# SabaPivot/ProjectionTrainer

Measured on AMD Instinct MI355X. Metric: Stage-1 images/sec/node (SigLIP-L-384 + Gemma3-1B, 576+128 tok), higher is better.
Workload: dtype bf16; 1 GPU; cfg2: SigLIP-ViT-L/16-384 frozen fwd + MLP projector fwd/bwd + Gemma3-1B frozen fwd/bwd, 575 vis + 128 text tokens; global_batch=32, per_gpu_batch=32, seq_len=703, parallelism=dp1

## Files before the change

### include/ptk.h

```cpp
#ifndef PTK_H
#define PTK_H

#include <stddef.h>
#include <stdint.h>

#ifdef __cplusplus
extern "C" {
#endif

#define PTK_ABI_VERSION 8

int ptk_abi_version(void);
const char* ptk_last_error(void);


typedef struct {
  int g;
  int skip;
  int64_t gs;
  int64_t off;
} ptk_rowmap;

enum { PTK_ACT_NONE = 0, PTK_ACT_GELU_TANH = 1, PTK_ACT_GELU_ERF = 2, PTK_ACT_GEGLU = 3,
       PTK_ACT_GELU_ERF_BWD = 4, PTK_ACT_GEGLU_BWD = 5 };
enum { PTK_OUT_BF16 = 0, PTK_OUT_F32 = 1, PTK_OUT_F32_BF16ROUND = 2 };

typedef struct {
  const void* A;
  const void* B;
  void* C;
  int M, N, K;
  int64_t lda, ldb, ldc;
  int batch;
  int batch_inner;
  int64_t sA0, sA1, sB0, sB1, sC0, sC1;
  float alpha;
  int act;
  int out;
  const float* bias;
  const float* rowadd;
  int rowadd_period;
  int64_t ld_rowadd;
  const float* resid;
  int64_t ld_resid;
  void* aux;
  void* aux2;
  int64_t ld_aux;
  const void* aux_in;
  const void* aux_in2;
  int64_t ld_aux_in;
  ptk_rowmap amap;
  ptk_rowmap cmap;
  const void* resid16;
  int64_t ld_resid16;
  int bf16_linear;
  void* tail_ws;
} ptk_gemm_desc;
int ptk_gemm(const ptk_gemm_desc* d, void* stream);
#define PTK_GEMM_TAIL_COUNTER_BYTES 16384
size_t ptk_gemm_tail_scratch_bytes(void);
int ptk_gemm_tail_split(const ptk_gemm_desc* d);
int ptk_gemm_plan(const ptk_gemm_desc* d, int ncu, int* path, int* tile_rows, int* tail_split);
int ptk_gemm_split_plan(const ptk_gemm_desc* d, int ncu, int64_t part_floats, int* slices, int* kc, int* rem,
                        int* tail_ws);

int ptk_layernorm(const float* x, const float* w, const float* b, void* y, int rows, int cols, float eps,
                  void* stream);
int ptk_rmsnorm(const float* x, const float* w, void* y, float* rstd, int rows, int cols, float eps,
                void* stream);
int ptk_rmsnorm_bwd(const float* x, const float* w, const float* rstd, const float* dn, const float* dacc,
                    float* dx, int rows, int cols, void* stream);
int ptk_qknorm_rope_fwd(const void* qkv, const float* q_norm_w, const float* k_norm_w, const float* cos_t,
                        const float* sin_t, int batch, int seq, int heads, int kv_heads, int head_dim, float eps,
                        void* Q, void* K, void* V, float* rstd_q, float* rstd_k, void* stream);
int ptk_qknorm_rope_bwd(const void* qkv, const float* q_norm_w, const float* k_norm_w, const float* cos_t,
                        const float* sin_t, int batch, int seq, int heads, int kv_heads, int head_dim,
                        const float* rstd_q, const float* rstd_k, const void* dQ, const void* dK, const void* dV,
                        void* dqkv, void* stream);
int ptk_softmax(const float* S, void* P, int nz, int rows, int cols, int64_t ld, int rows_per_batch, int qdiv,
                int zdiv, int causal, int window, const int32_t* key_valid, int key_len, void* stream);
int ptk_cross_entropy(void* logits, int64_t ld, int rows, int vocab, const int64_t* targets, float* row_loss,
                      const float* gscale, void* stream);
int ptk_transpose_bf16(const void* in, int64_t ld_in, void* out, int64_t ld_out, int nz, int64_t s_in,
                       int64_t s_out, int rows, int cols, int rows_pad, void* stream);
int ptk_transpose_rows_bf16(const void* in, int64_t ld_in, int map_g, int64_t map_gs, int64_t map_off, int rows,
                            int cols, void* out, int64_t ld_out, int rows_pad, void* stream);
int ptk_weight_grad_bf16(const void* dy, int64_t lddy, int y_map_g, int64_t y_map_gs, int64_t y_map_off, int Ny,
                         const void* x, int64_t ldx, int x_map_g, int64_t x_map_gs, int64_t x_map_off, int Nx, int rows,
                         void* grad, void* ta, void* tb, float* part, int64_t part_floats, int mode, void* stream);
int ptk_cast_f32_bf16(const float* in, void* out, int64_t n, void* stream);
int ptk_fill_normal_bf16(void* out, int64_t n, uint64_t seed, float std, float mean, void* stream);
// ... 20 lines not shown
  float scale;
} ptk_flash_desc;
int ptk_flash_attn_fwd(const ptk_flash_desc* d, void* stream);

typedef struct {
  const void* Q; const void* K; const void* V; const void* O; const void* dO;
  const float* lse; float* delta;
  void* dQ; void* dK; void* dV;
  int rows, nkeys, head_dim;
  int batch, batch_inner, zdiv;
  int64_t ldo, sO0, sO1;
  ptk_rowmap omap;
  int qdiv, causal, window;
  const int32_t* key_valid;
  float scale;
  void* workspace;
  int64_t workspace_bytes;
} ptk_flash_bwd_desc;
size_t ptk_flash_bwd_workspace_bytes(const ptk_flash_bwd_desc* d);
int ptk_flash_attn_bwd(const ptk_flash_bwd_desc* d, void* stream);

typedef struct {
  int image_size, patch_size, channels, hidden, heads, intermediate, layers;
  float eps;
} ptk_siglip_config;

typedef struct {
  const void* wqkv;  const float* bqkv;
  const void* wo;    const float* bo;
  const void* w1;    const float* b1;
  const void* w2;    const float* b2;
  const float* ln1_w; const float* ln1_b;
  const float* ln2_w; const float* ln2_b;
} ptk_siglip_layer;

typedef struct {
  const void* patch_w;
  const float* patch_b;
  const float* pos;
  const float* post_w; const float* post_b;
  const ptk_siglip_layer* layers;
} ptk_siglip_weights;

size_t ptk_siglip_workspace_bytes(const ptk_siglip_config* c, int batch);
int ptk_siglip_fwd(const ptk_siglip_config* c, const ptk_siglip_weights* w, int batch, const void* pixels,
                   void* out, void* ws, size_t ws_bytes, void* stream);

typedef struct {
  int vision_dim, inter_dim, llm_dim;
  const void* w1;   const float* b1;
  const void* w2;   const float* b2;
  const void* w2t;
  void* tail_ws;
} ptk_projector;

int ptk_projector_fwd(const ptk_projector* p, int rows, const void* x, void* a, void* h, float* out,
                      ptk_rowmap out_map, int64_t ld_out, int round_bf16, void* stream);
size_t ptk_projector_workspace_bytes(const ptk_projector* p, int rows);
int ptk_projector_bwd(const ptk_projector* p, int rows, const void* x, const void* a, const void* h,
                      const void* dy, float* dw1, float* db1, float* dw2, float* db2, void* ws, size_t ws_bytes,
                      void* stream);
int ptk_gather_vision_grad(const float* dx_llm, int batch, int num_patches, int seq_pad, int llm_dim, void* dy,
                           void* stream);

typedef struct {
  int vocab, hidden, inter, layers, heads, kv_heads, head_dim;
  int sliding_window, sliding_pattern;
  int pad_token_id;
  float query_pre_attn_scalar, eps;
} ptk_gemma3_config;

typedef struct {
  const void* wqkv;  const void* wqkv_t;
  const void* wo;    const void* wo_t;
  const void* wgu;   const void* wgu_t;
  const void* wd;    const void* wd_t;
  const float* ln_in; const float* ln_post_attn; const float* ln_pre_ff; const float* ln_post_ff;
  const float* q_norm; const float* k_norm;
} ptk_gemma3_layer;

typedef struct {
  const void* embed;
  const void* embed_t;
  const float* final_norm;
  const float* rope_cos_local; const float* rope_sin_local;
  const float* rope_cos_global; const float* rope_sin_global;
  int rope_max_pos;
  const ptk_gemma3_layer* layers;
} ptk_gemma3_weights;

typedef struct {
  int batch, text_len, num_vision, seq_pad;
  const int64_t* token_ids;
  const int64_t* labels;
  float* x;
  float* dx;
  float loss_scale;
  float* loss;
  int label_offset;
} ptk_gemma3_batch;

size_t ptk_gemma3_workspace_bytes(const ptk_gemma3_config* c, int batch, int text_len, int seq_pad);
int ptk_gemma3_loss_fwd_bwd(const ptk_gemma3_config* c, const ptk_gemma3_weights* w, const ptk_gemma3_batch* b,
                            void* ws, size_t ws_bytes, void* stream);
int ptk_gemma3_loss_fwd(const ptk_gemma3_config* c, const ptk_gemma3_weights* w, const ptk_gemma3_batch* b,
                        void* ws, size_t ws_bytes, void* stream);

typedef struct {
  void* wqkv; void* wo; void* wgu; void* wd;
  void* ln_in; void* ln_post_attn; void* ln_pre_ff; void* ln_post_ff;
  void* q_norm; void* k_norm;
// ... 96 lines not shown
```

### projectiontrainer_amd/_lib.py

```python
from __future__ import annotations

import ctypes as C
import os

_HERE = os.path.dirname(os.path.abspath(__file__))
LIB_PATH = os.path.join(_HERE, "libptk.so")
if os.environ.get("PTK_LIB"):
    LIB_PATH = os.path.join(os.path.dirname(_HERE), os.environ["PTK_LIB"])

c_void_p, c_int, c_int64, c_float, c_size_t, c_uint64 = C.c_void_p, C.c_int, C.c_int64, C.c_float, C.c_size_t, C.c_uint64
c_float_p = C.POINTER(C.c_float)

ACT_NONE, ACT_GELU_TANH, ACT_GELU_ERF, ACT_GEGLU, ACT_GELU_ERF_BWD, ACT_GEGLU_BWD = range(6)
OUT_BF16, OUT_F32, OUT_F32_BF16ROUND = range(3)


class RowMap(C.Structure):
    _fields_ = [("g", c_int), ("skip", c_int), ("gs", c_int64), ("off", c_int64)]


class GemmDesc(C.Structure):
    _fields_ = [("A", c_void_p), ("B", c_void_p), ("C", c_void_p),
                ("M", c_int), ("N", c_int), ("K", c_int),
                ("lda", c_int64), ("ldb", c_int64), ("ldc", c_int64),
                ("batch", c_int), ("batch_inner", c_int),
                ("sA0", c_int64), ("sA1", c_int64), ("sB0", c_int64), ("sB1", c_int64),
                ("sC0", c_int64), ("sC1", c_int64),
                ("alpha", c_float), ("act", c_int), ("out", c_int),
                ("bias", c_void_p), ("rowadd", c_void_p), ("rowadd_period", c_int),
                ("ld_rowadd", c_int64), ("resid", c_void_p), ("ld_resid", c_int64),
                ("aux", c_void_p), ("aux2", c_void_p), ("ld_aux", c_int64),
                ("aux_in", c_void_p), ("aux_in2", c_void_p), ("ld_aux_in", c_int64),
                ("amap", RowMap), ("cmap", RowMap), ("resid16", c_void_p), ("ld_resid16", c_int64),
                ("bf16_linear", c_int), ("tail_ws", c_void_p)]


class FlashDesc(C.Structure):
    _fields_ = [("Q", c_void_p), ("K", c_void_p), ("V", c_void_p), ("O", c_void_p), ("lse", c_void_p),
                ("rows", c_int), ("nkeys", c_int), ("head_dim", c_int),
                ("ldq", c_int64), ("ldk", c_int64), ("ldo", c_int64),
                ("batch", c_int), ("batch_inner", c_int), ("zdiv", c_int),
                ("sQ0", c_int64), ("sQ1", c_int64), ("sK0", c_int64), ("sK1", c_int64),
                ("sO0", c_int64), ("sO1", c_int64), ("qmap", RowMap), ("omap", RowMap),
                ("qdiv", c_int), ("causal", c_int), ("window", c_int), ("key_valid", c_void_p),
                ("scale", c_float)]


class FlashBwdDesc(C.Structure):
    _fields_ = [("Q", c_void_p), ("K", c_void_p), ("V", c_void_p), ("O", c_void_p), ("dO", c_void_p),
                ("lse", c_void_p), ("delta", c_void_p), ("dQ", c_void_p), ("dK", c_void_p), ("dV", c_void_p),
                ("rows", c_int), ("nkeys", c_int), ("head_dim", c_int),
                ("batch", c_int), ("batch_inner", c_int), ("zdiv", c_int),
                ("ldo", c_int64), ("sO0", c_int64), ("sO1", c_int64), ("omap", RowMap),
                ("qdiv", c_int), ("causal", c_int), ("window", c_int), ("key_valid", c_void_p),
                ("scale", c_float), ("workspace", c_void_p), ("workspace_bytes", c_int64)]


class SiglipConfigC(C.Structure):
    _fields_ = [("image_size", c_int), ("patch_size", c_int), ("channels", c_int), ("hidden", c_int),
                ("heads", c_int), ("intermediate", c_int), ("layers", c_int), ("eps", c_float)]


class SiglipLayerC(C.Structure):
    _fields_ = [("wqkv", c_void_p), ("bqkv", c_void_p), ("wo", c_void_p), ("bo", c_void_p),
                ("w1", c_void_p), ("b1", c_void_p), ("w2", c_void_p), ("b2", c_void_p),
                ("ln1_w", c_void_p), ("ln1_b", c_void_p), ("ln2_w", c_void_p), ("ln2_b", c_void_p)]


class SiglipWeightsC(C.Structure):
    _fields_ = [("patch_w", c_void_p), ("patch_b", c_void_p), ("pos", c_void_p),
                ("post_w", c_void_p), ("post_b", c_void_p), ("layers", C.POINTER(SiglipLayerC))]


class ProjectorC(C.Structure):
    _fields_ = [("vision_dim", c_int), ("inter_dim", c_int), ("llm_dim", c_int),
                ("w1", c_void_p), ("b1", c_void_p), ("w2", c_void_p), ("b2", c_void_p), ("w2t", c_void_p),
                ("tail_ws", c_void_p)]


class Gemma3ConfigC(C.Structure):
    _fields_ = [("vocab", c_int), ("hidden", c_int), ("inter", c_int), ("layers", c_int), ("heads", c_int),
                ("kv_heads", c_int), ("head_dim", c_int), ("sliding_window", c_int),
                ("sliding_pattern", c_int), ("pad_token_id", c_int),
                ("query_pre_attn_scalar", c_float), ("eps", c_float)]


class Gemma3LayerC(C.Structure):
    _fields_ = [("wqkv", c_void_p), ("wqkv_t", c_void_p), ("wo", c_void_p), ("wo_t", c_void_p),
                ("wgu", c_void_p), ("wgu_t", c_void_p), ("wd", c_void_p), ("wd_t", c_void_p),
                ("ln_in", c_void_p), ("ln_post_attn", c_void_p), ("ln_pre_ff", c_void_p),
                ("ln_post_ff", c_void_p), ("q_norm", c_void_p), ("k_norm", c_void_p)]


class Gemma3WeightsC(C.Structure):
    _fields_ = [("embed", c_void_p), ("embed_t", c_void_p), ("final_norm", c_void_p),
                ("rope_cos_local", c_void_p), ("rope_sin_local", c_void_p),
                ("rope_cos_global", c_void_p), ("rope_sin_global", c_void_p),
                ("rope_max_pos", c_int), ("layers", C.POINTER(Gemma3LayerC))]


class Gemma3BatchC(C.Structure):
    _fields_ = [("batch", c_int), ("text_len", c_int), ("num_vision", c_int), ("seq_pad", c_int),
                ("token_ids", c_void_p), ("labels", c_void_p), ("x", c_void_p), ("dx", c_void_p),
                ("loss_scale", c_float), ("loss", c_void_p), ("label_offset", c_int)]


class Gemma3GenerateC(C.Structure):
    _fields_ = [("batch", c_int), ("prompt_len", c_int), ("max_new_tokens", c_int), ("do_sample", c_int),
                ("top_k", c_int), ("temperature", c_float), ("seed", C.c_uint64), ("eos_token_id", c_int64),
                ("pad_token_id", c_int64), ("prompt_batch_stride", c_int64), ("top_p", c_float)]


class Gemma3DecodeC(C.Structure):
    _fields_ = [("rows", c_int), ("prompt_len", c_int), ("max_new_tokens", c_int), ("prompt_repeat", c_int),
                ("prompt_batch_stride", c_int64)]


class Gemma3LayerGradsC(C.Structure):
    _fields_ = [(n, c_void_p) for n in ("wqkv", "wo", "wgu", "wd", "ln_in", "ln_post_attn", "ln_pre_ff",
                                        "ln_post_ff", "q_norm", "k_norm")]


class Gemma3GradsC(C.Structure):
    _fields_ = [("embed", c_void_p), ("final_norm", c_void_p), ("layers", C.POINTER(Gemma3LayerGradsC))]
# ... 1 lines not shown

class ImageDesc(C.Structure):
    _fields_ = [("src_off", c_int64), ("h", C.c_int32), ("w", C.c_int32), ("c", C.c_int32),
                ("kh", C.c_int32), ("kv", C.c_int32), ("pad_", C.c_int32),
                ("coef_off", c_int64), ("tmp_off", c_int64)]


ABI_VERSION = 8

SIGNATURES = {
    "ptk_abi_version": (c_int, []),
    "ptk_last_error": (C.c_char_p, []),
    "ptk_gemm": (c_int, [C.POINTER(GemmDesc), c_void_p]),
    "ptk_gemm_tail_scratch_bytes": (c_size_t, []),
    "ptk_gemm_tail_split": (c_int, [C.POINTER(GemmDesc)]),
    "ptk_gemm_plan": (c_int, [C.POINTER(GemmDesc), c_int] + [C.POINTER(c_int)] * 3),
    "ptk_gemm_split_plan": (c_int, [C.POINTER(GemmDesc), c_int, c_int64] + [C.POINTER(c_int)] * 4),
    "ptk_layernorm": (c_int, [c_void_p, c_void_p, c_void_p, c_void_p, c_int, c_int, c_float, c_void_p]),
    "ptk_rmsnorm": (c_int, [c_void_p, c_void_p, c_void_p, c_void_p, c_int, c_int, c_float, c_void_p]),
    "ptk_rmsnorm_bwd": (c_int, [c_void_p] * 6 + [c_int, c_int, c_void_p]),
    "ptk_qknorm_rope_fwd": (c_int, [c_void_p] * 5 + [c_int] * 5 + [c_float] + [c_void_p] * 6),
    "ptk_qknorm_rope_bwd": (c_int, [c_void_p] * 5 + [c_int] * 5 + [c_void_p] * 7),
    "ptk_softmax": (c_int, [c_void_p, c_void_p, c_int, c_int, c_int, c_int64, c_int, c_int, c_int, c_int,
                            c_int, c_void_p, c_int, c_void_p]),
    "ptk_cross_entropy": (c_int, [c_void_p, c_int64, c_int, c_int, c_void_p, c_void_p, c_void_p, c_void_p]),
    "ptk_transpose_bf16": (c_int, [c_void_p, c_int64, c_void_p, c_int64, c_int, c_int64, c_int64, c_int,
                                   c_int, c_int, c_void_p]),
    "ptk_transpose_rows_bf16": (c_int, [c_void_p, c_int64, c_int, c_int64, c_int64, c_int, c_int, c_void_p, c_int64,
                                        c_int, c_void_p]),
    "ptk_weight_grad_bf16": (c_int, [c_void_p, c_int64, c_int, c_int64, c_int64, c_int,
                                     c_void_p, c_int64, c_int, c_int64, c_int64, c_int, c_int,
                                     c_void_p, c_void_p, c_void_p, c_void_p, c_int64, c_int, c_void_p]),
    "ptk_cast_f32_bf16": (c_int, [c_void_p, c_void_p, c_int64, c_void_p]),
    "ptk_fill_normal_bf16": (c_int, [c_void_p, c_int64, c_uint64, c_float, c_float, c_void_p]),
    "ptk_gemm_timer_enable": (c_int, [c_int]),
    "ptk_gemm_force_small_tiles": (c_int, [c_int]),
    "ptk_gemm_timer_read": (c_int, [c_int, C.POINTER(C.c_double), C.POINTER(c_int)]),
    "ptk_gemm_path_counts": (c_int, [c_void_p, c_int]),
    "ptk_stage_timers_enable": (c_int, [c_int]),
    "ptk_stage_begin": (c_int, [C.c_char_p, c_void_p]),
    "ptk_stage_end": (c_int, [c_void_p]),
    "ptk_stage_timers_read": (c_int64, [C.c_char_p, c_size_t, c_int]),
    "ptk_flash_attn_fwd": (c_int, [C.POINTER(FlashDesc), c_void_p]),
    "ptk_flash_attn_bwd": (c_int, [C.POINTER(FlashBwdDesc), c_void_p]),
    "ptk_flash_bwd_workspace_bytes": (c_size_t, [C.POINTER(FlashBwdDesc)]),
    "ptk_siglip_workspace_bytes": (c_size_t, [C.POINTER(SiglipConfigC), c_int]),
    "ptk_siglip_fwd": (c_int, [C.POINTER(SiglipConfigC), C.POINTER(SiglipWeightsC), c_int, c_void_p, c_void_p,
                               c_void_p, c_size_t, c_void_p]),
    "ptk_projector_fwd": (c_int, [C.POINTER(ProjectorC), c_int, c_void_p, c_void_p, c_void_p, c_void_p, RowMap,
                                  c_int64, c_int, c_void_p]),
    "ptk_projector_workspace_bytes": (c_size_t, [C.POINTER(ProjectorC), c_int]),
    "ptk_projector_bwd": (c_int, [C.POINTER(ProjectorC), c_int] + [c_void_p] * 8 + [c_void_p, c_size_t, c_void_p]),
    "ptk_gather_vision_grad": (c_int, [c_void_p, c_int, c_int, c_int, c_int, c_void_p, c_void_p]),
    "ptk_gemma3_workspace_bytes": (c_size_t, [C.POINTER(Gemma3ConfigC), c_int, c_int, c_int]),
    "ptk_gemma3_loss_fwd_bwd": (c_int, [C.POINTER(Gemma3ConfigC), C.POINTER(Gemma3WeightsC),
                                        C.POINTER(Gemma3BatchC), c_void_p, c_size_t, c_void_p]),
    "ptk_gemma3_loss_fwd": (c_int, [C.POINTER(Gemma3ConfigC), C.POINTER(Gemma3WeightsC),
                                    C.POINTER(Gemma3BatchC), c_void_p, c_size_t, c_void_p]),
    "ptk_gemma3_train_workspace_bytes": (c_size_t, [C.POINTER(Gemma3ConfigC), c_int, c_int, c_int]),
    "ptk_gemma3_train_fwd_bwd": (c_int, [C.POINTER(Gemma3ConfigC), C.POINTER(Gemma3WeightsC),
                                         C.POINTER(Gemma3BatchC), C.POINTER(Gemma3GradsC), c_void_p, c_size_t,
                                         c_void_p]),
    "ptk_gemma3_generate_workspace_bytes": (c_size_t, [C.POINTER(Gemma3ConfigC), c_int, c_int, c_int]),
    "ptk_gemma3_generate": (c_int, [C.POINTER(Gemma3ConfigC), C.POINTER(Gemma3WeightsC), C.POINTER(Gemma3GenerateC),
                                    c_void_p, c_void_p, c_void_p, c_void_p, c_void_p, c_size_t, c_void_p]),
    "ptk_gemma3_decode_workspace_bytes": (c_size_t, [C.POINTER(Gemma3ConfigC), C.POINTER(Gemma3DecodeC)]),
# ... 121 lines not shown
```

### projectiontrainer_amd/csrc/capi.cpp

```cpp
#include <stdarg.h>
#include <stdio.h>

#include "../../include/ptk.h"
#include "ptk_internal.h"

namespace ptk {

static thread_local char g_err[512] = "";

int set_error(const char* fmt, ...) {
  va_list ap;
  va_start(ap, fmt);
  vsnprintf(g_err, sizeof(g_err), fmt, ap);
  va_end(ap);
  return -1;
}

RowMap to_map(ptk_rowmap m) { return RowMap{m.g, m.skip, (long)m.gs, (long)m.off}; }

GemmArgs to_args(const ptk_gemm_desc* d) {
  GemmArgs a;
  a.A = (const bf16_t*)d->A; a.B = (const bf16_t*)d->B; a.C = d->C;
  a.M = d->M; a.N = d->N; a.K = d->K;
  a.lda = d->lda; a.ldb = d->ldb; a.ldc = d->ldc;
  a.zin = d->batch_inner > 0 ? d->batch_inner : 1;
  a.sA0 = d->sA0; a.sA1 = d->sA1; a.sB0 = d->sB0; a.sB1 = d->sB1; a.sC0 = d->sC0; a.sC1 = d->sC1;
  a.alpha = d->alpha;
  a.bias = d->bias; a.rowadd = d->rowadd; a.rowadd_period = d->rowadd_period > 0 ? d->rowadd_period : 1;
  a.ld_rowadd = d->ld_rowadd; a.resid = d->resid; a.ld_resid = d->ld_resid;
  a.aux = (bf16_t*)d->aux; a.aux2 = (bf16_t*)d->aux2; a.ld_aux = d->ld_aux;
  a.aux_in = (const bf16_t*)d->aux_in; a.aux_in2 = (const bf16_t*)d->aux_in2; a.ld_aux_in = d->ld_aux_in;
  a.amap = to_map(d->amap); a.cmap = to_map(d->cmap);
  a.resid16 = (const bf16_t*)d->resid16; a.ld_resid16 = d->ld_resid16; a.bf16_linear = d->bf16_linear;
  a.tail_ws = d->tail_ws;
  return a;
}

int device_cus() {
  static int n = 0;
  if (n == 0) {
    int dev = 0, v = 0;
    if (hipGetDevice(&dev) == hipSuccess &&
        hipDeviceGetAttribute(&v, hipDeviceAttributeMultiprocessorCount, dev) == hipSuccess && v > 0)
      n = v;
    else
      n = 256;
  }
  return n;
}

}

using namespace ptk;
#define ST ((hipStream_t)stream)

extern "C" {

int ptk_abi_version(void) { return PTK_ABI_VERSION; }
const char* ptk_last_error(void) { return g_err; }

int ptk_gemm(const ptk_gemm_desc* d, void* stream) {
  if (!d) return set_error("ptk_gemm: null desc");
  if (d->act == PTK_ACT_GEGLU && (d->N % 32)) return set_error("ptk_gemm: GEGLU needs N %% 32 == 0");
  return launch_gemm(to_args(d), d->act, d->out, d->batch > 0 ? d->batch : 1, ST);
}

size_t ptk_gemm_tail_scratch_bytes(void) { return p8_tail_scratch_bytes(); }
// ... 57 lines not shown
}
int ptk_qknorm_rope_bwd(const void* qkv, const float* q_norm_w, const float* k_norm_w, const float* cos_t,
                        const float* sin_t, int batch, int seq, int heads, int kv_heads, int head_dim,
                        const float* rstd_q, const float* rstd_k, const void* dQ, const void* dK, const void* dV,
                        void* dqkv, void* stream) {
  const AttnShape sh{batch, seq, heads, kv_heads, head_dim};
  return launch_qknorm_rope_bwd((const bf16_t*)qkv, q_norm_w, k_norm_w, cos_t, sin_t, sh, rstd_q, rstd_k,
                                (const bf16_t*)dQ, (const bf16_t*)dK, (const bf16_t*)dV, (bf16_t*)dqkv, ST);
}
int ptk_softmax(const float* S, void* P, int nz, int rows, int cols, int64_t ld, int rows_per_batch, int qdiv,
                int zdiv, int causal, int window, const int32_t* key_valid, int key_len, void* stream) {
  MaskSpec m{rows_per_batch > 0 ? rows_per_batch : rows, qdiv > 0 ? qdiv : 1, zdiv > 0 ? zdiv : 1, causal, window,
             key_valid, key_len};
  return launch_softmax_fwd(S, (bf16_t*)P, nz, rows, cols, ld, m, ST);
}

int ptk_cross_entropy(void* logits, int64_t ld, int rows, int vocab, const int64_t* targets, float* row_loss,
                      const float* gscale, void* stream) {
  return launch_ce_fwd_bwd((bf16_t*)logits, ld, rows, vocab, targets, row_loss, gscale, ST);
}

int ptk_transpose_bf16(const void* in, int64_t ld_in, void* out, int64_t ld_out, int nz, int64_t s_in, int64_t s_out,
                       int rows, int cols, int rows_pad, void* stream) {
  return launch_transpose((const bf16_t*)in, ld_in, s_in, 0, 1, (bf16_t*)out, ld_out, s_out, 0, nz, rows, cols,
                          rows_pad, ST);
}

int ptk_transpose_rows_bf16(const void* in, int64_t ld_in, int map_g, int64_t map_gs, int64_t map_off, int rows,
                            int cols, void* out, int64_t ld_out, int rows_pad, void* stream) {
  const RowMap m{map_g, 0, map_gs, map_off};
  return launch_transpose_rows((const bf16_t*)in, ld_in, m, rows, cols, (bf16_t*)out, ld_out, rows_pad, ST);
}

int ptk_cast_f32_bf16(const float* in, void* out, int64_t n, void* stream) {
  return launch_cast_f32_bf16(in, (bf16_t*)out, n, ST);
}

int ptk_gemm_force_small_tiles(int mode) {
  if (mode != 0 && mode != 1 && mode != 2 && mode != 4 && mode != 8 && mode != 32 && mode != 512 && mode != 1024 &&
      mode != 4096)
    return set_error("gemm tile mode %d not in {0, 1, 2, 4, 8, 32, 512, 1024, 4096}", mode);
  force_small_tiles(mode);
  return 0;
}
int ptk_gemm_timer_enable(int on) {
  timer_enable(on);
  return 0;
}
int ptk_gemm_timer_read(int act_class, double* total_ms, int* count) { return timer_read(act_class, total_ms, count); }
int ptk_gemm_path_counts(int64_t* counts, int reset) { return path_counts(counts, reset); }

int ptk_fill_normal_bf16(void* out, int64_t n, uint64_t seed, float std, float mean, void* stream) {
  return launch_fill_normal_bf16((bf16_t*)out, n, seed, std, mean, ST);
}

int ptk_flash_attn_fwd(const ptk_flash_desc* d, void* stream) {
  if (!d) return set_error("flash: null desc");
  FlashArgs a;
  a.Q = (const bf16_t*)d->Q; a.K = (const bf16_t*)d->K; a.V = (const bf16_t*)d->V; a.O = (bf16_t*)d->O;
  a.lse = d->lse; a.rows = d->rows; a.nkeys = d->nkeys; a.D = d->head_dim;
  a.ldq = d->ldq; a.ldk = d->ldk; a.ldo = d->ldo;
  a.zin = d->batch_inner > 0 ? d->batch_inner : 1; a.zdiv = d->zdiv > 0 ? d->zdiv : 1;
  a.sQ0 = d->sQ0; a.sQ1 = d->sQ1; a.sK0 = d->sK0; a.sK1 = d->sK1; a.sO0 = d->sO0; a.sO1 = d->sO1;
  a.qmap = to_map(d->qmap); a.omap = to_map(d->omap);
  a.qdiv = d->qdiv > 0 ? d->qdiv : 1; a.causal = d->causal; a.window = d->window;
  a.key_valid = d->key_valid; a.scale = d->scale;
// ... 137 lines not shown
```

### projectiontrainer_amd/csrc/gemm.hip

```cpp
#include <stdlib.h>

#include "common.h"
#include "ptk_internal.h"
#include "gemm_epi.h"

#include <algorithm>
#include <vector>

namespace ptk {

constexpr int BM = 128, BN = 128, BK = 64, GROUP_M = 8;
constexpr int STAGE_BYTES = (BM + BN) * BK * 2;
static_assert(4 * 64 * 68 * 4 >= 2 * STAGE_BYTES, "epilogue staging must cover the pipeline buffers");

typedef const __attribute__((address_space(1))) void* gptr_t;
typedef __attribute__((address_space(3))) void* lptr_t;

#ifdef PTK_NO_SRC_SWZ
#define PTK_SRC_SWZ(c, r) (c)
#else
#define PTK_SRC_SWZ(c, r) ((c) ^ (((r) >> 1) & 7))
#endif

#ifndef PTK_GLDS_AUX
// ... 651 lines not shown
    ++g_path_count[path][act & 7];
    if (g_timing && ((g_timing_mask >> act) & 1)) { e0 = next_event(act); e1 = next_event(act); }
    if (e0) (void)hipEventRecord(e0, st);
  }
  ~GemmLaunchScope() { if (e1) (void)hipEventRecord(e1, st); }
};

GemmPlanEnv gemm_plan_env() {
  GemmPlanEnv e;
  e.ncu = device_cus();
  e.force_tiles = g_force_tiles;
  e.p8_all = PTK_AB("PTK_P8", 0) == 1;
  e.tm_short = PTK_AB("PTK_TM224", 1) != 0;
  e.lean_epi = lean_epilogue_enabled();
  e.streamk = streamk_enabled();
  e.tail_scope = tail_scope();
  return e;
}

int launch_gemm(const GemmArgs& a, int act, int out, int batch, hipStream_t st, const GemmPlan* planned) {
  if (a.M <= 0 || a.N <= 0 || batch <= 0) return 0;
  if (a.K <= 0 || a.K % BK) return set_error("gemm: K=%d must be a positive multiple of 64", a.K);
  if ((a.lda % 8) || (a.ldb % 8)) return set_error("gemm: lda/ldb must be multiples of 8 (16-B rows)");
  if (((uintptr_t)a.A | (uintptr_t)a.B) & 15) return set_error("gemm: A/B must be 16-B aligned");
  if (a.zin <= 0) return set_error("gemm: zin must be >= 1");
  const long ntile = (long)((a.M + BM - 1) / BM) * ((a.N + BN - 1) / BN);
  if (ntile > 0x7fffffffL) return set_error("gemm: too many tiles");
  if (!gemm_act_out(act, out, [](auto, auto) {})) return set_error("gemm: unsupported (act=%d, out=%d)", act, out);
  const GemmPlan plan = planned ? *planned : gemm_plan(a, act, out, batch, gemm_plan_env());
  GemmLaunchScope scope(plan.path, act, st);
  const dim3 grid_big((unsigned)((long)((a.M + BIG - 1) / BIG) * ((a.N + BIG - 1) / BIG)), 1, 1);
  switch (plan.path) {
    case GEMM_PATH_P8:
    case GEMM_PATH_P8SK: return launch_gemm_p8(a, act, out, st, plan.tail, plan.tm);
    case GEMM_PATH_W4: return launch_gemm_w4(a, act, out, st, 0);
    case GEMM_PATH_BIG2:
      gemm_act_out(act, out, [&](auto A, auto O) {
        hipLaunchKernelGGL((gemm_big2_kernel<A(), O()>), grid_big, dim3(512), 0, st, a);
      });
      break;
    case GEMM_PATH_BIG:
      gemm_act_out(act, out, [&](auto A, auto O) {
        hipLaunchKernelGGL((gemm_big_kernel<A(), O()>), grid_big, dim3(512), 0, st, a);
      });
      break;
    default:
      gemm_act_out(act, out, [&](auto A, auto O) {
        hipLaunchKernelGGL((gemm_nt_kernel<A(), O()>), dim3((unsigned)ntile, 1, (unsigned)batch), dim3(256), 0, st, a);
      });
      break;
  }
  return hipGetLastError() == hipSuccess ? 0 : set_error("gemm launch failed");
}

int gemm_p8_kslices(const GemmArgs& a, int slices, hipStream_t st) {
  if (a.M <= 0 || a.N <= 0) return 0;
  GemmLaunchScope scope(GEMM_PATH_P8, ACT_NONE, st);
  return launch_gemm_p8_kslices(a, slices, st);
}

int gemm_tn(const GemmArgs& a, int out, int slices, void* slab, hipStream_t st, long k_rows) {
  if (a.M <= 0 || a.N <= 0) return 0;
  GemmLaunchScope scope(GEMM_PATH_TN, ACT_NONE, st);
  return launch_gemm_tn(a, out, slices, slab, st, k_rows);
}

}

// ... 9 lines not shown
```

### projectiontrainer_amd/csrc/gemm_plan.cpp

```cpp
#include <algorithm>

#include "ptk_internal.h"

namespace ptk {

bool w4_supported(const GemmArgs& a, int act, int out) {
  if (a.N % 8 || a.K % W4_KT) return false;
  if (a.alpha != 1.f) return false;
  if (a.row_stats) return false;
  if (a.resid16 && (out != OUT_BF16 || a.ld_resid16 % 8)) return false;
  if ((a.ldc % 8) || (a.resid && a.ld_resid % 4) || (a.rowadd && a.ld_rowadd % 4)) return false;
  if ((a.aux || a.aux2) && a.ld_aux % 8) return false;
  if ((a.aux_in || a.aux_in2) && a.ld_aux_in % 8) return false;
  if (((uintptr_t)a.C | (uintptr_t)a.bias | (uintptr_t)a.resid | (uintptr_t)a.resid16 | (uintptr_t)a.rowadd | (uintptr_t)a.aux |
       (uintptr_t)a.aux2 | (uintptr_t)a.aux_in | (uintptr_t)a.aux_in2) & 15)
    return false;
  if (act == ACT_GEGLU && (a.N % 32)) return false;
  if (act == ACT_GEGLU_BWD && (!a.aux_in || !a.aux_in2 || (a.N % 16) || (a.ldc % 8))) return false;
  if (act == ACT_GELU_ERF_BWD && !a.aux_in) return false;
  if (out != OUT_BF16 && (act != ACT_NONE)) return false;
  if (a.amap.g != 0) return false;
  const double abytes = (double)(a.M + a.amap.off) * a.lda * 2, bbytes = (double)a.N * a.ldb * 2;
  return abytes < 2147483000.0 && bbytes < 2147483000.0;
}
// ... 137 lines not shown
  return a.M >= 1024 && a.N >= 512 && (a.K >= 6144 || (a.N >= 6144 && a.K >= 1152));
}
bool staggered_big(const GemmArgs& a, const GemmPlanEnv& e) {
  return e.force_tiles == 4 || (e.force_tiles == 0 && big_shape(a) && a.K >= 4096);
}
bool big(const GemmArgs& a, const GemmPlanEnv& e) {
  return e.force_tiles != 1 && (e.force_tiles == 2 || big_shape(a));
}

}

GemmPlan gemm_plan(const GemmArgs& a, int act, int out, int batch, const GemmPlanEnv& e) {
  GemmPlan p;
  if (batch != 1) {
    p.path = GEMM_PATH_NTB;
    return p;
  }
  if (p8_supported(a, act, out)) {
    const P8Tail tl = tail(a, act, out, e);
    const int tm = tl.units ? 256 : short_tile(a, act, out, e);
    const bool single = single_round(a, act, out, e);
    if (e.force_tiles == 32 || single || tl.units || tm != 256 || p8_over_w4(a, act, out, e)) {
      p.path = tl.units ? GEMM_PATH_P8SK : GEMM_PATH_P8;
      p.tm = tm;
      p.tail = tl;
      p.single_round = single;
      return p;
    }
  }
  if ((e.force_tiles == 8 || w4_shape(a, act, out, e)) && w4_supported(a, act, out)) p.path = GEMM_PATH_W4;
  else if (staggered_big(a, e)) p.path = GEMM_PATH_BIG2;
  else if (big(a, e)) p.path = GEMM_PATH_BIG;
  return p;
}

GemmSplitPlan gemm_split_plan(const GemmArgs& a, int out, long part_floats, const GemmPlanEnv& env) {
  GemmSplitPlan sp;
  GemmPlanEnv e = env;
  e.force_tiles = 0;
  sp.direct = gemm_plan(a, ACT_NONE, out, 1, e);
  const GemmPlan& direct = sp.direct;
  if (direct.path == GEMM_PATH_P8SK) return sp;
  if (e.streamk && a.K >= 4096 && (size_t)part_floats * sizeof(float) >= P8_CNT_BYTES + p8_slab_bytes(e.ncu)) {
    GemmArgs b = a;
    b.tail_ws = reinterpret_cast<void*>((uintptr_t)256);
    const GemmPlan lent = gemm_plan(b, ACT_NONE, out, 1, e);
    if (lent.path == GEMM_PATH_P8SK) {
      sp.tail_ws = true;
      sp.direct = lent;
      return sp;
    }
  }
  if (direct.single_round) return sp;
  const long nbig = tiles256(a);
  int S = 1, kmin = 1024;
  if (a.K >= 4096 && nbig <= 64) S = 4;
  else if (a.K >= 4096 && nbig <= 300) S = 2;
  const long n128 = (long)((a.M + 127) / 128) * ((a.N + 127) / 128), cus = e.ncu;
  if (n128 * 2 <= cus) {
    kmin = 256;
    while (n128 * S * 2 <= 2 * cus && a.K / (S * 2) >= kmin) S *= 2;
  }
  while (S > 1 && ((long)S * a.M * a.N > part_floats || a.K / S < kmin || a.N % 4 || a.ldc % 4)) S /= 2;
  const bool plain = !a.rowadd && !a.resid && !a.aux && !a.aux_in && a.amap.g == 0 && a.amap.off == 0 &&
                     a.cmap.g == 0 && a.cmap.off == 0 && a.bias == nullptr && a.alpha == 1.f;
  if (S == 1 || !plain) return sp;
// ... 54 lines not shown
```

### projectiontrainer_amd/csrc/gemm_w4.hip

```cpp
#include "common.h"
#include "ptk_internal.h"
#include "gemm_epi.h"
#include "gemm_persist.h"

#include <algorithm>
#include <cstdlib>
#include <type_traits>

#ifndef PTK_W4_RDS
#define PTK_W4_RDS 0
#endif
#ifndef PTK_W4_DMS
#define PTK_W4_DMS 0
#endif
#ifndef PTK_P8_PRIO
#define PTK_P8_PRIO 1
#endif
#ifndef PTK_P8_MPRIO
#define PTK_P8_MPRIO 0
#endif

namespace ptk {

template <int ACT, int OUT, bool LEAN = false>
__global__ void __launch_bounds__(256, 1) gemm_w4_kernel(GemmArgs p, uint32_t a_bytes, uint32_t b_bytes,
                                                         uint32_t c_bytes) {
  __shared__ __attribute__((aligned(16))) char smem[W4_NSLOT * W4_SLOT];
  const int lane = threadIdx.x & 63;
  const int wave = __builtin_amdgcn_readfirstlane(threadIdx.x >> 6);
  const int wr = wave >> 1, wc = wave & 1;
  const int nbm = (p.M + W4 - 1) / W4, nbn = (p.N + W4 - 1) / W4;
  const int ntile = nbm * nbn;
  const int G = gridDim.x;
  int loc;
  {
    const int b = blockIdx.x, q = G >> 3, rr = G & 7, x = b & 7;
    loc = (x < rr ? x * (q + 1) : rr * (q + 1) + (x - rr) * q) + (b >> 3);
  }
  if (loc >= ntile) return;
  const int nt = p.K / W4_KT;
  const int nks = 2 * nt;
  const int total_ks = ((ntile - loc + G - 1) / G) * nks;

  const u32x4_t rsa = w4_rsrc(p.A, a_bytes), rsb = w4_rsrc(p.B, b_bytes);

  uint32_t offa[4], offb[4];
#pragma unroll
  for (int j = 0; j < 4; ++j) {
    const int lr = wave * 64 + 16 * j + (lane >> 2);
    const int lc = (lane & 3) ^ ((lane >> 3) & 2);
    offa[j] = (uint32_t)lr * (uint32_t)p.lda * 2u + lc * 16;
    offb[j] = (uint32_t)lr * (uint32_t)p.ldb * 2u + lc * 16;
  }
  const uint32_t lds_base = __builtin_amdgcn_readfirstlane(lds_addr(smem));
  const uint32_t lds_dma = lds_base + wave * 64 * 64;
  int dt = loc, dks = 0, dcount = 0;
  uint32_t dsa = 0, dsb = 0;
  auto dma_tile = [&](int t) {
    int bm, bn;
    w4_tile_coords(t, nbm, nbn, bm, bn);
    dsa = __builtin_amdgcn_readfirstlane((uint32_t)(bm * W4 + (int)p.amap.off) * (uint32_t)p.lda * 2u);
    dsb = __builtin_amdgcn_readfirstlane((uint32_t)(bn * W4) * (uint32_t)p.ldb * 2u);
  };
  auto dma_advance = [&]() {
    if (++dcount < total_ks) {
      if (++dks == nks) {
        dks = 0;
        dt += G;
        dma_tile(dt);
      }
    }
  };
  auto slot_next = [](uint32_t s) { s += W4_SLOT; return s == W4_NSLOT * W4_SLOT ? 0u : s; };

  const int frag_off = (lane & 15) * 64 + (((lane >> 4) ^ ((lane >> 1) & 2)) << 4);
  const uint32_t frag_a = lds_addr(smem) + wr * 128 * 64 + frag_off;
  const uint32_t frag_b = lds_addr(smem) + W4_SOPB + wc * 128 * 64 + frag_off;
  bf16x8_t fa0[8], fb0[8], fa1[8], fb1[8];
  f32x4_t acc[8][8];

#define W4_GROUP(FA, FB, Q, FIRST)                                                  \
  do {                                                                              \
    _Pragma("unroll") for (int jj = 0; jj < 4; ++jj) {                              \
      if (FIRST) W4_MFMA0(acc[(Q) >> 1][4 * ((Q) & 1) + jj], FB[4 * ((Q) & 1) + jj], FA[(Q) >> 1]); \
      else W4_MFMA(acc[(Q) >> 1][4 * ((Q) & 1) + jj], FB[4 * ((Q) & 1) + jj], FA[(Q) >> 1]);       \
    }                                                                               \
  } while (0)
#define W4_READ(FA, FB, BA, BB, Q)                                                  \
  do {                                                                              \
    if ((Q) < 8) W4_DSREAD(FA[(Q) & 7], BA, ((Q) & 7) * 1024);                      \
    else W4_DSREAD(FB[(Q) & 7], BB, ((Q) & 7) * 1024);                              \
  } while (0)
#define W4_PIN(FA, FB)                                                                              \
  do {                                                                                              \
    asm volatile("s_waitcnt lgkmcnt(0)" ::: "memory");                                              \
    asm volatile("" : "+v"(FA[0]), "+v"(FA[1]), "+v"(FA[2]), "+v"(FA[3]), "+v"(FA[4]), "+v"(FA[5]),  \
                 "+v"(FA[6]), "+v"(FA[7]));                                                         \
    asm volatile("" : "+v"(FB[0]), "+v"(FB[1]), "+v"(FB[2]), "+v"(FB[3]), "+v"(FB[4]), "+v"(FB[5]),  \
                 "+v"(FB[6]), "+v"(FB[7]));                                                         \
  } while (0)

  auto kstep = [&](auto first_c, const bf16x8_t (&FA)[8], const bf16x8_t (&FB)[8], bf16x8_t (&NA)[8],
                   bf16x8_t (&NB)[8], uint32_t rs, uint32_t ws) {
    constexpr bool first = decltype(first_c)::value;
    const uint32_t ba = frag_a + rs, bb = frag_b + rs;
    const uint32_t da = lds_dma + ws, db = da + W4_SOPB;
    const uint32_t sa = dsa + dks * (W4_KS * 2), sb = dsb + dks * (W4_KS * 2);
#pragma unroll
    for (int q = 0; q < 16; ++q) {
#if PTK_W4_RDS == 1
      if (q < 8) {
        W4_READ(NA, NB, ba, bb, 2 * q);
        W4_READ(NA, NB, ba, bb, 2 * q + 1);
      }
#else
      if (q < 8) {
        W4_READ(NA, NB, ba, bb, q);
      } else if (q < 12) {
        W4_READ(NA, NB, ba, bb, 8 + 2 * (q - 8));
        W4_READ(NA, NB, ba, bb, 9 + 2 * (q - 8));
      }
#endif
#if PTK_W4_DMS == 1
      if (q >= 8) {
        const int pc = q - 8;
#elif PTK_W4_DMS == 2
      if (q < 8) {
        const int pc = q;
#elif PTK_W4_DMS == 3
      if (q & 1) {
        const int pc = q >> 1;
#else
      if (!(q & 1)) {
        const int pc = q >> 1;
#endif
        if (pc & 1) W4_DMA(rsb, offb[pc >> 1], sb, db + (pc >> 1) * 1024);
        else W4_DMA(rsa, offa[pc >> 1], sa, da + (pc >> 1) * 1024);
      }
      W4_GROUP(FA, FB, q, first);
    }
  };

  dma_tile(dt);
#pragma unroll
  for (int b = 0; b < 4; ++b) {
    const uint32_t da = lds_dma + b * W4_SLOT, db = da + W4_SOPB;
    const uint32_t sa = dsa + dks * (W4_KS * 2), sb = dsb + dks * (W4_KS * 2);
#pragma unroll
    for (int j = 0; j < 4; ++j) {
      W4_DMA(rsa, offa[j], sa, da + j * 1024);
      W4_DMA(rsb, offb[j], sb, db + j * 1024);
    }
    dma_advance();
  }
  asm volatile("s_waitcnt vmcnt(8)" ::: "memory");
  __builtin_amdgcn_s_barrier();
#pragma unroll
  for (int q = 0; q < 16; ++q) W4_READ(fa0, fb0, frag_a, frag_b, q);
  W4_PIN(fa0, fb0);
  __builtin_amdgcn_s_barrier();

  uint32_t rs = W4_SLOT, ws = 4 * W4_SLOT;
  int t = loc, kt = 0;
#ifdef PTK_P8_STAMPS
  unsigned int stv_[4] = {0u, 0u, 0u, 0u};
  const int em_ = g_p8_epi_mode;
#endif
  for (int g = 0; g < total_ks; g += 2) {
    if (kt == 0) P8_STAMP(0, (t - loc) / G);
    if (kt == 0) kstep(std::true_type{}, fa0, fb0, fa1, fb1, rs, ws);
    else kstep(std::false_type{}, fa0, fb0, fa1, fb1, rs, ws);
    W4_PIN(fa1, fb1);
    dma_advance();
    rs = slot_next(rs);
    ws = slot_next(ws);
    kstep(std::false_type{}, fa1, fb1, fa0, fb0, rs, ws);
    W4_PIN(fa0, fb0);
    dma_advance();
    rs = slot_next(rs);
    ws = slot_next(ws);
// ... 5 lines not shown
      asm volatile("s_nop 7\n\ts_nop 7" ::: "memory");
      int bm, bn;
      w4_tile_coords(t, nbm, nbn, bm, bn);
#ifdef PTK_P8_STAMPS
      if (em_ != 1)
#endif
      {
        const long row0 = (long)bm * W4 + wr * 128, col0 = (long)bn * W4 + wc * 128;
        if constexpr (LEAN && ACT == ACT_GEGLU_BWD)
          w4_epilogue_lean_glu<ACT, 8>(kernarg_args(), acc, row0, col0, lane, c_bytes);
        else if constexpr (LEAN) w4_epilogue_lean<ACT, 8>(kernarg_args(), acc, row0, col0, lane, c_bytes);
        else w4_epilogue<ACT, OUT>(kernarg_args(), acc, row0, col0, lane);
      }
      P8_STAMP(3, (t - loc) / G);
      t += G;
      kt = 0;
    } else {
      ++kt;
    }
  }
  asm volatile("s_waitcnt vmcnt(0)" ::: "memory");
#ifdef PTK_P8_STAMPS
  if (wave == 0 && blockIdx.x < 1024)
#pragma unroll
    for (int k = 0; k < 4; ++k) g_p8_stamps[blockIdx.x][k][lane] = stv_[k];
#endif
#undef W4_GROUP
#undef W4_READ
#undef W4_PIN
}

bool lean_epilogue_enabled() { return PTK_AB("PTK_LEAN_EPI", 1) != 0; }

int launch_gemm_w4(const GemmArgs& a, int act, int out, hipStream_t st, int max_grid) {
  const long ntile = (long)((a.M + W4 - 1) / W4) * ((a.N + W4 - 1) / W4);
  long grid = std::min<long>(ntile, max_grid > 0 ? max_grid : device_cus());
#ifdef PTK_P8_STAMPS
  if (const char* e = getenv("PTK_GEMM_GRID")) grid = std::min<long>(grid, atol(e));
#endif
  const long arows = a.M + a.amap.off;
  const uint32_t ab = (uint32_t)std::min<double>((double)arows * a.lda * 2, 2147483000.0);
  const uint32_t bb = (uint32_t)std::min<double>((double)a.N * a.ldb * 2, 2147483000.0);
  uint32_t cb = 0;
  if (lean_epilogue_ok(a, act, out, cb, lean_epilogue_enabled())) {
#define PTK_W4L_CASE(ACT_)                                                                                   \
    if (act == ACT_)                                                                                         \
      hipLaunchKernelGGL((gemm_w4_kernel<ACT_, OUT_BF16, true>), dim3((unsigned)grid), dim3(256), 0, st, a, ab, bb, cb);
    PTK_W4L_CASE(ACT_NONE)
    PTK_W4L_CASE(ACT_GELU_TANH)
    PTK_W4L_CASE(ACT_GEGLU_BWD)
#undef PTK_W4L_CASE
    return hipGetLastError() == hipSuccess ? 0 : set_error("gemm_w4 launch failed");
  }
  if (!gemm_act_out(act, out, [&](auto A, auto O) {
        hipLaunchKernelGGL((gemm_w4_kernel<A(), O()>), dim3((unsigned)grid), dim3(256), 0, st, a, ab, bb, 0u);
      }))
    return set_error("gemm_w4: unsupported (act=%d, out=%d)", act, out);
  return hipGetLastError() == hipSuccess ? 0 : set_error("gemm_w4 launch failed");
}


namespace {
constexpr int P8_PIECES = 4;

}



#ifdef PTK_P8_CREAD
#define P8_DSREAD(DST, ADDR, OFF) \
  (DST) = *reinterpret_cast<const __attribute__((address_space(3))) bf16x8_t*>((uintptr_t)((ADDR) + (OFF)))
#define P8_LGKM(N) do { } while (0)
#define P8_BARRIER() do { __builtin_amdgcn_s_barrier(); asm volatile("" ::: "memory"); } while (0)
#else
#define P8_BARRIER() __builtin_amdgcn_s_barrier()
#define P8_DSREAD(DST, ADDR, OFF) W4_DSREAD(DST, ADDR, OFF)
#define P8_LGKM(N) asm volatile("s_waitcnt lgkmcnt(" #N ")" ::: "memory")
#endif
template <int ACT, int OUT, bool SK, bool LEAN = false, int TM = 256>
__global__ void __launch_bounds__(512, 1) gemm_p8_kernel(GemmArgs p, uint32_t a_bytes, uint32_t b_bytes, P8Tail tl,
                                                         uint32_t c_bytes) {
  static_assert(TM == 256 || ((TM == 224 || TM == 192 || TM == 160) && !SK), "shorter tiles: whole tiles only");
  constexpr int RB = TM / 32;
  __shared__ __attribute__((aligned(16))) char smem[W4_NSLOT * W4_SLOT];
  const int lane = threadIdx.x & 63;
  const int wave = __builtin_amdgcn_readfirstlane(threadIdx.x >> 6);
  const int hf = wave >> 2, wq = wave & 3, wr = wq >> 1, wc = wq & 1;
  const bool a_dma = TM == 256 || wave < RB;
  const int nbm = (p.M + TM - 1) / TM, nbn = (p.N + W4 - 1) / W4;
  const int ntile = nbm * nbn;
  const int G = gridDim.x;
  int loc;
  {
    const int b = blockIdx.x, q = G >> 3, rr = G & 7, x = b & 7;
    loc = (x < rr ? x * (q + 1) : rr * (q + 1) + (x - rr) * q) + (b >> 3);
  }
  const int nt = p.K / W4_KT;
  const int dp_tiles = SK ? tl.dp_tiles : ntile;
  const int n_dp = loc < dp_tiles ? (dp_tiles - loc + G - 1) / G : 0;
  const int U = SK ? tl.units : 0, Gs = SK ? tl.gsplit : 1, nu = nt >> 1;
  const int u0 = SK && loc < Gs ? p8_start(loc, Gs, U) : 0, u1 = SK && loc < Gs ? p8_start(loc + 1, Gs, U) : 0;
  const int n_tail = u1 > u0 ? (u1 - 1) / nu - u0 / nu + 1 : 0;
  const int nseg = n_dp + n_tail;
  if (nseg == 0) return;
  const int total_ks = 2 * n_dp * nt + 4 * (u1 - u0);
  uint32_t segA = 0, segB = 0, segC = 0;
  if constexpr (SK) {
    const int i = lane;
    int t, k0, k1, tt;
    if (i < n_dp) {
      t = loc + i * G; k0 = 0; k1 = nt; tt = -1;
    } else {
      tt = u0 / nu + (i - n_dp);
      k0 = 2 * (max(u0, tt * nu) - tt * nu);
      k1 = 2 * (min(u1, (tt + 1) * nu) - tt * nu);
      t = dp_tiles + tt;
    }
    int g0 = 0, np = 1, s0 = 0, myslot = 0;
    if (tt >= 0 && i < nseg) {
      g0 = p8_owner((long)tt * nu, Gs, U);
      np = p8_owner((long)(tt + 1) * nu - 1, Gs, U) - g0 + 1;
      s0 = p8_start(g0, Gs, U) < tt * nu ? 1 : 0;
      myslot = u0 < tt * nu ? 1 : 0;
      if (np == 1) tt = -1;
    }
    segA = (uint32_t)t | ((uint32_t)(tt + 1) << 16);
    segB = (uint32_t)k0 | ((uint32_t)k1 << 16);
    segC = (uint32_t)g0 | ((uint32_t)np << 10) | ((uint32_t)s0 << 20) | ((uint32_t)myslot << 21);
  }
  auto segment = [&](int s, int& t, int& k0, int& k1, int& tt) __attribute__((always_inline)) {
    if constexpr (!SK) {
      t = loc + s * G; k0 = 0; k1 = nt; tt = -1;
    } else {
      const uint32_t a = __builtin_amdgcn_readlane(segA, s), b = __builtin_amdgcn_readlane(segB, s);
      t = (int)(a & 0xffffu); tt = (int)(a >> 16) - 1;
      k0 = (int)(b & 0xffffu); k1 = (int)(b >> 16);
    }
  };
  const u32x4_t rsa = w4_rsrc(p.A, a_bytes), rsb = w4_rsrc(p.B, b_bytes);

  uint32_t offa[2], offb[2];
#pragma unroll
  for (int j = 0; j < 2; ++j) {
    const int lr = wave * 32 + 16 * j + (lane >> 2);
    const int lc = (lane & 3) ^ ((lane >> 3) & 2);
    offa[j] = (uint32_t)lr * (uint32_t)p.lda * 2u + lc * 16;
    offb[j] = (uint32_t)lr * (uint32_t)p.ldb * 2u + lc * 16;
  }
  const uint32_t lds_base = __builtin_amdgcn_readfirstlane(lds_addr(smem));
  const uint32_t lds_dma = lds_base + wave * 32 * 64;
  int dseg = 0, dks = 0, dlen = 0, dcount = 0;
  uint32_t dsa = 0, dsb = 0;
  auto dma_seg = [&](int s) {
    int t, k0, k1, tt;
    segment(s, t, k0, k1, tt);
    int bm, bn;
    w4_tile_coords(t, nbm, nbn, bm, bn);
    uint32_t kz = 0;
    if (!SK && tl.zslices > 1) {
      const int nbz = nbm / tl.zslices, z = bm / nbz;
      bm -= z * nbz;
      kz = (uint32_t)z * (uint32_t)p.K * 2u;
    }
    dsa = __builtin_amdgcn_readfirstlane((uint32_t)(bm * TM + (int)p.amap.off) * (uint32_t)p.lda * 2u + kz +
                                         (uint32_t)k0 * (W4_KT * 2));
    dsb = __builtin_amdgcn_readfirstlane((uint32_t)(bn * W4) * (uint32_t)p.ldb * 2u + kz + (uint32_t)k0 * (W4_KT * 2));
    dlen = 2 * (k1 - k0);
  };
  auto dma_advance = [&]() {
    if (++dcount < total_ks) {
      if (++dks == dlen) {
        dks = 0;
        dma_seg(++dseg);
      }
    }
  };
  auto slot_next = [](uint32_t s) { s += W4_SLOT; return s == W4_NSLOT * W4_SLOT ? 0u : s; };

  const int frag_off = (lane & 15) * 64 + (((lane >> 4) ^ ((lane >> 1) & 2)) << 4);
  const uint32_t frag_a = lds_addr(smem) + wr * (TM / 2) * 64 + frag_off;
  const uint32_t frag_b = lds_addr(smem) + W4_SOPB + (wc * 128 + hf * 64) * 64 + frag_off;
  bf16x8_t fa[8], fb0[4], fb1[4];
  f32x4_t acc[8][4];

  auto read_frags = [&](uint32_t rs) __attribute__((always_inline)) {
    const uint32_t ba = frag_a + rs, bb = frag_b + rs;
#pragma unroll
    for (int r = 0; r < RB; ++r) P8_DSREAD(fa[r], ba, r * 1024);
#pragma unroll
    for (int r = 0; r < 4; ++r) P8_DSREAD(fb0[r], bb, r * 1024);
    P8_LGKM(0);
    asm volatile("" : "+v"(fa[0]), "+v"(fa[1]), "+v"(fa[2]), "+v"(fa[3]), "+v"(fa[4]), "+v"(fa[5]),
                 "+v"(fa[6]), "+v"(fa[7]));
    asm volatile("" : "+v"(fb0[0]), "+v"(fb0[1]), "+v"(fb0[2]), "+v"(fb0[3]));
  };

  auto kstep = [&](auto first_c, auto read_c, auto half_c, bf16x8_t (&FB)[4], bf16x8_t (&NB)[4], uint32_t rs,
                   uint32_t ws) __attribute__((always_inline)) {
    constexpr bool first = decltype(first_c)::value, rd = decltype(read_c)::value;
    constexpr int half = decltype(half_c)::value;
    const uint32_t ba = frag_a + rs, bb = frag_b + rs;
    const uint32_t da = lds_dma + ws, db = da + W4_SOPB;
    const uint32_t sa = dsa + dks * (W4_KS * 2), sb = dsb + dks * (W4_KS * 2);
#pragma unroll
    for (int q = 0; q < RB; ++q) {
      if constexpr (RB == 8) {
        if (q == 0) P8_LGKM(6);
        else if (q < 3) P8_LGKM(8);
        else if (q == 3) P8_LGKM(9);
        else P8_LGKM(10);
      } else if constexpr (RB == 7) {
        if (q == 0) P8_LGKM(5);
        else if (q < 3) P8_LGKM(7);
        else if (q == 3) P8_LGKM(8);
        else P8_LGKM(9);
      } else if constexpr (RB == 6) {
        if (q == 0) P8_LGKM(4);
        else if (q < 3) P8_LGKM(6);
        else if (q == 3) P8_LGKM(7);
        else P8_LGKM(8);
      } else {
        static_assert(RB == 5, "tile heights 256, 224, 192, 160");
        if (q == 0) P8_LGKM(3);
        else if (q < 3) P8_LGKM(5);
        else if (q == 3) P8_LGKM(6);
        else P8_LGKM(7);
      }
      asm volatile("" : "+v"(fa[q]));
      if (q == 0) asm volatile("" : "+v"(FB[0]), "+v"(FB[1]), "+v"(FB[2]), "+v"(FB[3]));
      if (rd && q < 4) P8_DSREAD(NB[q], bb, q * 1024);
#pragma unroll
      for (int pc = 0; pc < 4; ++pc) {
        if (q == (2 * pc + half < RB - 1 ? 2 * pc + half : RB - 1)) {
          if (pc & 1) W4_DMA(rsb, offb[pc >> 1], sb, db + (pc >> 1) * 1024);
          else if (a_dma) W4_DMA(rsa, offa[pc >> 1], sa, da + (pc >> 1) * 1024);
        }
// ... 4 lines not shown
        if (first) W4_MFMA0(acc[q][jj], FB[jj], fa[q]);
        else W4_MFMA(acc[q][jj], FB[jj], fa[q]);
      }
      if (PTK_P8_MPRIO) asm volatile("s_setprio 0" ::: "memory");
      if (rd && q >= 1) P8_DSREAD(fa[q - 1], ba, (q - 1) * 1024);
    }
    if (rd) P8_DSREAD(fa[RB - 1], ba, (RB - 1) * 1024);
  };

  auto tail_store = [&](int slot) __attribute__((always_inline)) {
    float* mine = tl.slab + (((size_t)loc * 2 + slot) * 8 + wave) * P8_WAVE_FLOATS + lane * 4;
#pragma unroll
    for (int q = 0; q < 8; ++q)
#pragma unroll
      for (int jj = 0; jj < 4; ++jj)
        asm volatile("global_store_dwordx4 %0, %1, off" :: "v"(mine + (4 * q + jj) * 256), "a"(acc[q][jj])
                     : "memory");
  };

#ifdef PTK_P8_STAMPS
  unsigned int stv_[4] = {0u, 0u, 0u, 0u};
  const int em_ = g_p8_epi_mode;
#endif
  auto vm_wait = [&]() __attribute__((always_inline)) {
    if (TM != 256 && !a_dma) asm volatile("s_waitcnt vmcnt(2)" ::: "memory");
    else asm volatile("s_waitcnt vmcnt(4)" ::: "memory");
  };
  auto run = [&](auto half_c) __attribute__((always_inline)) {
    if (PTK_P8_PRIO && decltype(half_c)::value) __builtin_amdgcn_s_setprio(PTK_P8_PRIO);
    dma_seg(0);
#pragma unroll
    for (int b = 0; b < 4; ++b) {
      const uint32_t da = lds_dma + b * W4_SLOT, db = da + W4_SOPB;
      const uint32_t sa = dsa + dks * (W4_KS * 2), sb = dsb + dks * (W4_KS * 2);
#pragma unroll
      for (int j = 0; j < 2; ++j) {
        if (a_dma) W4_DMA(rsa, offa[j], sa, da + j * 1024);
        W4_DMA(rsb, offb[j], sb, db + j * 1024);
      }
      dma_advance();
    }
    vm_wait();
    P8_BARRIER();
    read_frags(0);
    P8_BARRIER();
    uint32_t rs = W4_SLOT, ws = 4 * W4_SLOT;
    auto pair = [&](auto first_c, auto last_c) __attribute__((always_inline)) {
      constexpr bool lst = decltype(last_c)::value;
      kstep(first_c, std::true_type{}, half_c, fb0, fb1, rs, ws);
      dma_advance();
      rs = slot_next(rs);
      ws = slot_next(ws);
      kstep(std::false_type{}, std::integral_constant<bool, !lst>{}, half_c, fb1, fb0, rs, ws);
      dma_advance();
      if (!lst) rs = slot_next(rs);
      ws = slot_next(ws);
      vm_wait();
      P8_BARRIER();
    };
    for (int s = 0; s < nseg; ++s) {
      int t, k0, k1, tt;
      segment(s, t, k0, k1, tt);
      P8_STAMP(0, s);
      pair(std::true_type{}, std::false_type{});
      P8_STAMP(1, s);
      for (int kt = k0 + 1; kt < k1 - 1; ++kt) pair(std::false_type{}, std::false_type{});
      pair(std::false_type{}, std::true_type{});
// ... 101 lines not shown
  const dim3 grid((unsigned)(ntile - tl.dp_tiles), 8);
  const int nu = a.K / W4_KT / 2;
  if (act != ACT_NONE) return set_error("p8 fixup: ACT_NONE only");
  if (out == OUT_BF16) hipLaunchKernelGGL((p8_fixup_kernel<ACT_NONE, OUT_BF16>), grid, dim3(512), 0, st, a, tl, nu);
  else if (out == OUT_F32) hipLaunchKernelGGL((p8_fixup_kernel<ACT_NONE, OUT_F32>), grid, dim3(512), 0, st, a, tl, nu);
  else hipLaunchKernelGGL((p8_fixup_kernel<ACT_NONE, OUT_F32_BFR>), grid, dim3(512), 0, st, a, tl, nu);
  return hipGetLastError() == hipSuccess ? 0 : set_error("p8 fixup launch failed");
}

size_t p8_tail_scratch_bytes() { return P8_CNT_BYTES + p8_slab_bytes(device_cus()); }

static bool streamk_models() { return PTK_AB("PTK_STREAMK", 1) != 0; }
bool streamk_enabled() { return streamk_models(); }
static thread_local void* g_tail_scope = nullptr;
void* tail_scope() { return g_tail_scope; }
TailScratchScope::TailScratchScope(void* ws, hipStream_t st) : prev(g_tail_scope) {
  if (!streamk_models()) ws = nullptr;
  g_tail_scope = ws;
  (void)st;
}
TailScratchScope::~TailScratchScope() { g_tail_scope = prev; }

size_t p8_tail_scratch_bytes_models() { return streamk_models() ? p8_tail_scratch_bytes() : 0; }

int launch_gemm_p8_kslices(const GemmArgs& a, int slices, hipStream_t st) {
  if (slices < 1 || a.M % W4 || a.K < 128 || a.K % W4_KT || a.cmap.g || a.cmap.off || a.amap.g || a.amap.off ||
      a.bias || a.rowadd || a.resid || a.resid16 || a.aux || a.row_stats)
    return set_error("gemm_p8_kslices: unsupported operands");
  if ((double)a.M * a.lda * 2 + (double)slices * a.K * 2 >= 4293918720.0 ||
      (double)a.N * a.ldb * 2 + (double)slices * a.K * 2 >= 4293918720.0)
    return set_error("gemm_p8_kslices: operands past 4 GiB");
  GemmArgs g = a;
  g.M = a.M * slices;
  P8Tail tl;
  tl.zslices = slices;
  const long ntile = (long)(g.M / W4) * ((g.N + W4 - 1) / W4);
  const long grid = std::min<long>(ntile, device_cus());
  const uint32_t ab = (uint32_t)std::min<double>((double)a.M * a.lda * 2, 4294967040.0);
  const uint32_t bb = (uint32_t)std::min<double>((double)a.N * a.ldb * 2, 4294967040.0);
  hipLaunchKernelGGL((gemm_p8_kernel<ACT_NONE, OUT_F32, false>), dim3((unsigned)grid), dim3(512), 0, st, g, ab, bb, tl,
                     0u);
  return hipGetLastError() == hipSuccess ? 0 : set_error("gemm_p8_kslices launch failed");
}

template <int TM>
static int launch_p8_short(const GemmArgs& a, int act, int out, hipStream_t st, long grid, bool lean_epi) {
  const uint32_t ab = (uint32_t)std::min<double>((double)(a.M + a.amap.off) * a.lda * 2, 2147483000.0);
  const uint32_t bb = (uint32_t)std::min<double>((double)a.N * a.ldb * 2, 2147483000.0);
  const P8Tail tl{};
  uint32_t cb = 0;
  if (lean_epilogue_ok(a, act, out, cb, lean_epi)) {
    if (act == ACT_NONE)
      hipLaunchKernelGGL((gemm_p8_kernel<ACT_NONE, OUT_BF16, false, true, TM>), dim3((unsigned)grid), dim3(512), 0,
                         st, a, ab, bb, tl, cb);
    else
      hipLaunchKernelGGL((gemm_p8_kernel<ACT_GELU_TANH, OUT_BF16, false, true, TM>), dim3((unsigned)grid),
                         dim3(512), 0, st, a, ab, bb, tl, cb);
  } else if (act == ACT_GELU_TANH) {
    hipLaunchKernelGGL((gemm_p8_kernel<ACT_GELU_TANH, OUT_BF16, false, false, TM>), dim3((unsigned)grid), dim3(512),
                       0, st, a, ab, bb, tl, 0u);
  } else if (out == OUT_BF16) {
    hipLaunchKernelGGL((gemm_p8_kernel<ACT_NONE, OUT_BF16, false, false, TM>), dim3((unsigned)grid), dim3(512), 0,
                       st, a, ab, bb, tl, 0u);
  } else if (out == OUT_F32) {
    hipLaunchKernelGGL((gemm_p8_kernel<ACT_NONE, OUT_F32, false, false, TM>), dim3((unsigned)grid), dim3(512), 0,
                       st, a, ab, bb, tl, 0u);
  } else {
    hipLaunchKernelGGL((gemm_p8_kernel<ACT_NONE, OUT_F32_BFR, false, false, TM>), dim3((unsigned)grid), dim3(512),
                       0, st, a, ab, bb, tl, 0u);
  }
  return hipGetLastError() == hipSuccess ? 0 : set_error("gemm_p8 launch failed");
}

int launch_gemm_p8(const GemmArgs& a, int act, int out, hipStream_t st, const P8Tail& tl, int tm) {
  const long ncu = device_cus();
  const bool lean_epi = lean_epilogue_enabled();
  if (tm != 256 && !tl.units) {
    if (!(act == ACT_NONE || (act == ACT_GELU_TANH && out == OUT_BF16)))
      return set_error("gemm_p8: %d-row tiles take the plain / GELU-tanh epilogues only", tm);
    if (tm != 224 && tm != 192 && tm != 160) return set_error("gemm_p8: tile height %d (256, 224, 192, 160)", tm);
    const long ntm = (long)((a.M + tm - 1) / tm) * ((a.N + W4 - 1) / W4);
    const long grid = std::min<long>(ntm, ncu);
    if (tm == 224) return launch_p8_short<224>(a, act, out, st, grid, lean_epi);
    if (tm == 192) return launch_p8_short<192>(a, act, out, st, grid, lean_epi);
    return launch_p8_short<160>(a, act, out, st, grid, lean_epi);
  }
  const long ntile = (long)((a.M + W4 - 1) / W4) * ((a.N + W4 - 1) / W4);
  long grid = tl.units ? ncu : std::min<long>(ntile, ncu);
#ifdef PTK_P8_STAMPS
  if (const char* e = getenv("PTK_GEMM_GRID")) grid = std::min<long>(grid, atol(e));
#endif
  const long arows = a.M + a.amap.off;
  const uint32_t ab = (uint32_t)std::min<double>((double)arows * a.lda * 2, 2147483000.0);
  const uint32_t bb = (uint32_t)std::min<double>((double)a.N * a.ldb * 2, 2147483000.0);
  uint32_t cb = 0;
  if (tl.units) {
    if (act != ACT_NONE) return set_error("gemm_p8: the stream-K tail takes ACT_NONE only (act=%d)", act);
    if (lean_epilogue_ok(a, act, out, cb, lean_epi)) {
      hipLaunchKernelGGL((gemm_p8_kernel<ACT_NONE, OUT_BF16, true, true>), dim3((unsigned)grid), dim3(512), 0, st, a,
                         ab, bb, tl, cb);
    } else if (!gemm_act_out(act, out, [&](auto A, auto O) {
                 if constexpr (A() == ACT_NONE)
                   hipLaunchKernelGGL((gemm_p8_kernel<ACT_NONE, O(), true>), dim3((unsigned)grid), dim3(512), 0, st, a,
                                      ab, bb, tl, 0u);
               })) {
      return set_error("gemm_p8: unsupported (act=%d, out=%d)", act, out);
    }
    if (hipGetLastError() != hipSuccess) return set_error("gemm_p8 launch failed");
    return launch_p8_fixup(a, act, out, tl, st);
  }
  if (lean_epilogue_ok(a, act, out, cb, lean_epi)) {
#define PTK_P8L_CASE(ACT_)                                                                                   \
    if (act == ACT_)                                                                                         \
      hipLaunchKernelGGL((gemm_p8_kernel<ACT_, OUT_BF16, false, true>), dim3((unsigned)grid), dim3(512), 0, st, a, ab, \
                         bb, tl, cb);
    PTK_P8L_CASE(ACT_NONE)
    PTK_P8L_CASE(ACT_GELU_TANH)
    PTK_P8L_CASE(ACT_GEGLU_BWD)
#undef PTK_P8L_CASE
    return hipGetLastError() == hipSuccess ? 0 : set_error("gemm_p8 launch failed");
  }
  if (!gemm_act_out(act, out, [&](auto A, auto O) {
        hipLaunchKernelGGL((gemm_p8_kernel<A(), O(), false>), dim3((unsigned)grid), dim3(512), 0, st, a, ab, bb, tl, 0u);
      }))
    return set_error("gemm_p8: unsupported (act=%d, out=%d)", act, out);
  return hipGetLastError() == hipSuccess ? 0 : set_error("gemm_p8 launch failed");
}

}
```

### projectiontrainer_amd/csrc/misc.hip

```cpp
#include "common.h"

#include <algorithm>
#include <cstdlib>
#include "ptk_internal.h"

namespace ptk {

#define RET_OK(name) return hipGetLastError() == hipSuccess ? 0 : set_error(name " launch failed")

__global__ void __launch_bounds__(256) transpose_kernel(const bf16_t* __restrict__ in, long ld_in, long sin0, long sin1,
                                                        int zin, bf16_t* __restrict__ out, long ld_out, long sout0,
                                                        long sout1, int rows, int cols, int rows_pad) {
  __shared__ bf16_t tile[64][66];
  const int z = blockIdx.z, z0 = z / zin, z1 = z - z0 * zin;
  const bf16_t* src = in + z0 * sin0 + z1 * sin1;
  bf16_t* dst = out + z0 * sout0 + z1 * sout1;
  const int r0 = blockIdx.y * 64, c0 = blockIdx.x * 64;
  const int tx = threadIdx.x & 15, ty = threadIdx.x >> 4;
#pragma unroll
  for (int k = 0; k < 4; ++k) {
    const int r = r0 + ty + 16 * k;
    const int c = c0 + tx * 4;
    u16x4_t v = {0, 0, 0, 0};
    if (r < rows) {
// ... 34 lines not shown
  hipLaunchKernelGGL(transpose_kernel, grid, dim3(256), 0, st, in, ld_in, sin0, sin1, zin, out, ld_out, sout0,
                     sout1, rows, cols, rows_pad);
  RET_OK("transpose");
}

__global__ void __launch_bounds__(256) im2col_kernel(const bf16_t* __restrict__ px, bf16_t* __restrict__ out, int B,
                                                     int C, int H, int W, int P) {
  const int gx = W / P, gy = H / P;
  const int oct = P / 8;
  const long total = (long)B * gy * gx * C * P * oct;
  const long i = (long)blockIdx.x * 256 + threadIdx.x;
  if (i >= total) return;
  long t = i;
  const int o = t % oct; t /= oct;
  const int ky = t % P; t /= P;
  const int c = t % C; t /= C;
  const int px_ = t % gx; t /= gx;
  const int py = t % gy; t /= gy;
  const int b = (int)t;
  const bf16_t* s = px + (((long)b * C + c) * H + (py * P + ky)) * W + px_ * P + o * 8;
  const long row = ((long)b * gy + py) * gx + px_;
  bf16_t* d = out + row * (C * P * P) + (long)c * P * P + ky * P + o * 8;
  *reinterpret_cast<u16x8_t*>(d) = *reinterpret_cast<const u16x8_t*>(s);
}

int launch_im2col(const bf16_t* px, bf16_t* out, int B, int C, int H, int W, int P, hipStream_t st) {
  if (P % 8 || H % P || W % P) return set_error("im2col: patch %d must be a multiple of 8 dividing %dx%d", P, H, W);
  const long total = (long)B * (H / P) * (W / P) * C * P * (P / 8);
  if (total <= 0) return 0;
  hipLaunchKernelGGL(im2col_kernel, dim3((unsigned)((total + 255) / 256)), dim3(256), 0, st, px, out, B, C, H, W, P);
  RET_OK("im2col");
}

__global__ void cast_f32_bf16_kernel(const float* __restrict__ in, bf16_t* __restrict__ out, long n) {
  const long i = ((long)blockIdx.x * 256 + threadIdx.x) * 4;
  if (i + 3 < n) {
    float4 v = *reinterpret_cast<const float4*>(in + i);
    u16x4_t o;
    o[0] = f2bf(v.x); o[1] = f2bf(v.y); o[2] = f2bf(v.z); o[3] = f2bf(v.w);
    *reinterpret_cast<u16x4_t*>(out + i) = o;
  } else {
    for (long j = i; j < n; ++j) out[j] = f2bf(in[j]);
  }
}
int launch_cast_f32_bf16(const float* in, bf16_t* out, long n, hipStream_t st) {
  if (n <= 0) return 0;
  hipLaunchKernelGGL(cast_f32_bf16_kernel, dim3((unsigned)((n / 4 + 256) / 256)), dim3(256), 0, st, in, out, n);
  RET_OK("cast");
}

__global__ void __launch_bounds__(256) build_llm_inputs_kernel(const bf16_t* __restrict__ E,
                                                               const int64_t* __restrict__ ids, int T, int Nv,
                                                               int S, int Spad, int H, float scale, int pad_id,
                                                               float* __restrict__ x, int32_t* __restrict__ kv) {
  const long row = blockIdx.x;
  const int b = (int)(row / Spad), s = (int)(row - (long)b * Spad);
  if (threadIdx.x == 0) {
    int valid = 0;
    if (s < Nv) valid = 1;
    else if (s < S) valid = ids[(long)b * T + (s - Nv)] != pad_id;
    kv[row] = valid;
  }
  if (s < Nv) return;
  float* xr = x + row * H;
  if (s >= S) {
    for (int c = threadIdx.x * 4; c < H; c += 1024) *reinterpret_cast<float4*>(xr + c) = make_float4(0, 0, 0, 0);
// ... 381 lines not shown
```

### projectiontrainer_amd/csrc/models.cpp

```cpp
#include <cstdlib>
#include <algorithm>
#include <math.h>
#include <string.h>

#include <vector>

#include "../../include/ptk.h"
#include "ptk_internal.h"

using namespace ptk;

namespace {

struct Bump {
  char* base;
  size_t off = 0;
  explicit Bump(void* b) : base((char*)b) {}
  template <class T>
  T* take(size_t n) {
    off = (off + 255) & ~(size_t)255;
    T* p = base ? reinterpret_cast<T*>(base + off) : nullptr;
    off += n * sizeof(T);
    return p;
  }
// ... 32 lines not shown
                                   int M, int H, bf16_t* g_pre, bf16_t* g_post, float* wpart, hipStream_t st) {
  const RowMap ident{0, 0, 0, 0};
  if (g_pre && norm_wg_fused()) {
    const int nb = residual_norm_bwd_wg_blocks(M);
    float* pq = wpart + rms_wgrad_finish_floats(nb, H);
    CK(launch_residual_norm_bwd_wg(x2, w_pre, rstd_pre, dn, dR, t, w_post, rstd_t, dt, M, H, wpart, pq, st));
    CK(launch_rms_wgrad_finish(wpart, nb, H, g_pre, st));
    return launch_rms_wgrad_finish(pq, nb, H, g_post, st);
  }
  if (g_pre) CK(launch_rms_wgrad_bdy(x2, H, ident, rstd_pre, dn, H, M, H, g_pre, wpart, st));
  CK(launch_residual_norm_bwd_bdn(x2, w_pre, rstd_pre, dn, dR, t, w_post, rstd_t, dt, M, H, st));
  if (g_pre) CK(launch_rms_wgrad_bx(t, H, ident, rstd_t, dR, H, 1, M, H, g_post, wpart, st));
  return 0;
}
static bool dkv_reduce_split() {
  static const int v = [] { const char* e = getenv("PTK_DKV_REDUCE_SPLIT"); return e && e[0] == '1' ? 1 : 0; }();
  return v != 0;
}

static bool lm_stats_only() {
#ifdef PTK_DIAG
  static const int v = [] { const char* e = getenv("PTK_LM_STATS_ONLY"); return e && e[0] == '1' ? 1 : 0; }();
  return v != 0;
#else
  return false;
#endif
}

static bool ce_two_pass() {
  static const int v = [] { const char* e = getenv("PTK_CE_TWO_PASS"); return e && e[0] == '1' ? 1 : 0; }();
  return v != 0;
}

GemmArgs gemm(const void* A, long lda, const void* B, long ldb, void* C, long ldc, int M, int N, int K) {
  GemmArgs g;
  g.A = (const bf16_t*)A; g.B = (const bf16_t*)B; g.C = C;
  g.lda = lda; g.ldb = ldb; g.ldc = ldc;
  g.M = M; g.N = N; g.K = K;
  return g;
}

struct SiglipWs {
  bf16_t *patches, *h, *a, *qkv, *o, *mlp;
  void* tail;
};

SiglipWs siglip_layout(Bump& bp, const ptk_siglip_config* c, int B) {
  const long D = c->hidden, I = c->intermediate, P = c->patch_size, Nn = (c->image_size / P) * (c->image_size / P);
  const long Np = (Nn + 63) / 64 * 64, M = B * Nn, H = c->heads, hd = D / H, Kp = (long)c->channels * P * P;
  SiglipWs w;
  w.patches = bp.take<bf16_t>(M * Kp);
  w.h = bp.take<bf16_t>(M * D);
  w.a = bp.take<bf16_t>(M * D);
  w.qkv = bp.take<bf16_t>(M * 3 * D);
  w.o = bp.take<bf16_t>(M * D);
  w.mlp = bp.take<bf16_t>(M * I);
  w.tail = bp.take<char>(p8_tail_scratch_bytes_models());
  return w;
}

struct GemmaLayerSave {
  float *x2, *rstd_in, *rstd_ao, *rstd_pre, *rstd_dn, *rstd_q, *rstd_k;
  bf16_t *qkv, *Q, *K, *V, *O, *ao, *glu_a, *glu_b, *dn;
  float* lse;
  bf16_t *xn_in = nullptr, *xn_ff = nullptr, *h = nullptr;
};
struct GemmaWs {
  std::vector<float*> x;
// ... 90 lines not shown
    const long Rp = (R + 63) / 64 * 64;
    w.TA = bp.take<bf16_t>(std::max(std::max(2 * I, Dqkv), H) * M);
    w.TB = bp.take<bf16_t>(std::max(std::max(H, Dq), I) * M);
    w.TL = bp.take<bf16_t>(V * Rp);
    w.TX = bp.take<bf16_t>(H * Rp);
    w.eg_keys = bp.take<char>((long)embed_grad_ws_bytes(B, T));
    w.wpart = bp.take<float>(std::max(std::max((long)rms_wgrad_partial_floats((int)M, (int)H),
                                               2L * rms_wgrad_finish_floats(residual_norm_bwd_wg_blocks((int)M), (int)H)),
                                      (long)qknorm_wgrad_partial_floats(M, (int)D)));
  }
  w.sk_floats = std::max(std::max(2 * M * H, 2 * 2 * I * H), 4 * std::max(Dqkv, H) * H);
  if (train) w.sk_floats = std::max(w.sk_floats, V * H);
  w.sk_floats = std::max(w.sk_floats, (long)(p8_tail_scratch_bytes() / sizeof(float)) + 64);
  if (train) w.sk_floats = std::max(w.sk_floats, (long)(tn_slab_bytes() / sizeof(float)));
  w.skpart = bp.take<float>(w.sk_floats);
  w.tail = bp.take<char>(p8_tail_scratch_bytes_models());
  return w;
}

int gemm_split(const GemmArgs& a, int out, float* part, long part_floats, hipStream_t st) {
  const GemmPlanEnv env = gemm_plan_env();
  const GemmSplitPlan sp = gemm_split_plan(a, out, part ? part_floats : 0, env);
  if (sp.kc == 0) {
    GemmArgs b = a;
    GemmPlan plan = sp.direct;
    if (sp.tail_ws) {
      b.tail_ws = part;
      plan.tail.slab = reinterpret_cast<float*>(reinterpret_cast<char*>(part) + P8_CNT_BYTES);
    }
    return launch_gemm(b, ACT_NONE, out, 1, st, env.force_tiles == 0 ? &plan : nullptr);
  }
  const int kc = sp.kc, nfull = sp.slices, rem = sp.rem;
  GemmArgs b = a;
  b.C = part; b.ldc = a.N; b.K = kc;
  b.sA0 = kc; b.sB0 = kc; b.sC0 = (long)a.M * a.N;
  b.bf16_linear = 0; b.resid16 = nullptr; b.ld_resid16 = 0;
  CK(launch_gemm(b, ACT_NONE, OUT_F32, nfull, st));
  if (rem) {
    GemmArgs r = b;
    r.A = a.A + (long)nfull * kc; r.B = a.B + (long)nfull * kc; r.K = rem;
    r.C = part + (long)nfull * a.M * a.N;
    CK(launch_gemm(r, ACT_NONE, OUT_F32, 1, st));
  }
  const bool bf = out == OUT_BF16;
  return launch_splitk_reduce(part, nfull + (rem ? 1 : 0), a.M, a.N, a.C, a.ldc, bf ? 1 : 0,
                              bf ? a.resid16 : nullptr, a.ld_resid16, st);
}

static int wgrad_tn_mode() { return PTK_AB("PTK_WGRAD_TN", 1); }
}
namespace ptk {
int wgrad_tn_enabled() { return wgrad_tn_mode() != 0; }
}
namespace {
int weight_grad(const bf16_t* dy, long lddy, RowMap ymap, int Ny, const bf16_t* x, long ldx, RowMap xmap, int Nx,
                int rows, bf16_t* TA, bf16_t* TB, void* grad, float* skpart, long sk_floats, hipStream_t st,
                int tn = -1) {
  if (!grad) return 0;
  if (tn < 0) tn = wgrad_tn_mode();
  if (tn && ymap.g == 0 && ymap.off == 0 && xmap.g == 0 && xmap.off == 0 && rows > 0) {
    const int Kp = (rows + 63) / 64 * 64;
    GemmArgs g = gemm(dy, lddy, x, ldx, grad, Nx, Ny, Nx, Kp);
    g.bf16_linear = 1;
    g.resid16 = (const bf16_t*)grad;
    g.ld_resid16 = Nx;
    const GemmPlanEnv env = gemm_plan_env();
// ... 48 lines not shown
  return bp.off + 256;
}

int ptk_siglip_fwd(const ptk_siglip_config* c, const ptk_siglip_weights* wt, int B, const void* pixels, void* out,
                   void* ws, size_t ws_bytes, void* stream) {
  hipStream_t st = (hipStream_t)stream;
  if (ws_bytes < ptk_siglip_workspace_bytes(c, B)) return set_error("siglip_fwd: workspace too small");
  if (c->hidden % c->heads) return set_error("siglip_fwd: hidden %% heads");
  const int D = c->hidden, I = c->intermediate, P = c->patch_size, Hh = c->heads, hd = D / Hh;
  const int Nn = (c->image_size / P) * (c->image_size / P), Np = (Nn + 63) / 64 * 64, M = B * Nn;
  const int Kp = c->channels * P * P;
  if (Kp % 64 || hd % 64) return set_error("siglip_fwd: patch dim %d and head dim %d must be multiples of 64", Kp, hd);
  Bump bp(ws);
  SiglipWs w = siglip_layout(bp, c, B);
  TailScratchScope tail(w.tail, st);
  CK(tail.status);
  StageScope stage_all("siglip.fwd", st);
  StageSeq sq(st);
  sq.next("siglip.embed");

  CK(launch_im2col((const bf16_t*)pixels, w.patches, B, c->channels, c->image_size, c->image_size, P, st));
  {
    GemmArgs g = gemm(w.patches, Kp, wt->patch_w, Kp, w.h, D, M, D, Kp);
    g.bias = wt->patch_b;
    g.bf16_linear = 1;
    g.rowadd = wt->pos; g.rowadd_period = Nn; g.ld_rowadd = D;
    CK(launch_gemm(g, ACT_NONE, OUT_BF16, 1, st));
  }
  for (int l = 0; l < c->layers; ++l) {
    const ptk_siglip_layer& L = wt->layers[l];
    sq.next("siglip.attn");
    CK(launch_layernorm_bf16(w.h, L.ln1_w, L.ln1_b, w.a, M, D, c->eps, st));
    {
      GemmArgs g = gemm(w.a, D, L.wqkv, D, w.qkv, 3 * D, M, 3 * D, D);
      g.bias = L.bqkv;
      CK(launch_gemm(g, ACT_NONE, OUT_BF16, 1, st));
    }
    {
      FlashArgs fa;
      fa.Q = w.qkv; fa.K = w.qkv + D; fa.V = w.qkv + 2 * D; fa.O = w.o;
      fa.rows = Nn; fa.nkeys = Nn; fa.D = hd;
      fa.ldq = fa.ldk = 3 * D; fa.ldo = D;
      fa.zin = Hh; fa.zdiv = Hh;
      fa.sQ0 = fa.sK0 = (long)Nn * 3 * D; fa.sQ1 = fa.sK1 = hd;
      fa.sO0 = (long)Nn * D; fa.sO1 = hd;
      fa.scale = 1.0f / sqrtf((float)hd);
      StageScope sf("siglip.flash", st);
      CK(launch_attn_fwd(fa, B * Hh, st));
    }
    {
      GemmArgs g = gemm(w.o, D, L.wo, D, w.h, D, M, D, D);
      g.bias = L.bo; g.bf16_linear = 1; g.resid16 = w.h; g.ld_resid16 = D;
      CK(launch_gemm(g, ACT_NONE, OUT_BF16, 1, st));
    }
    sq.next("siglip.mlp");
    CK(launch_layernorm_bf16(w.h, L.ln2_w, L.ln2_b, w.a, M, D, c->eps, st));
    {
      GemmArgs g = gemm(w.a, D, L.w1, D, w.mlp, I, M, I, D);
      g.bias = L.b1;
      CK(launch_gemm(g, ACT_GELU_TANH, OUT_BF16, 1, st));
    }
    {
      GemmArgs g = gemm(w.mlp, I, L.w2, I, w.h, D, M, D, I);
      g.bias = L.b2; g.bf16_linear = 1; g.resid16 = w.h; g.ld_resid16 = D;
      CK(launch_gemm(g, ACT_NONE, OUT_BF16, 1, st));
    }
  }
  sq.next("siglip.post_norm");
  CK(launch_layernorm_bf16(w.h, wt->post_w, wt->post_b, (bf16_t*)out, M, D, c->eps, st));
  return 0;
}

size_t ptk_gemma3_workspace_bytes(const ptk_gemma3_config* c, int batch, int text_len, int seq_pad) {
  Bump bp(nullptr);
  gemma_layout(bp, c, batch, text_len, seq_pad);
  return bp.off + 256;
}

size_t ptk_gemma3_train_workspace_bytes(const ptk_gemma3_config* c, int batch, int text_len, int seq_pad) {
  Bump bp(nullptr);
  gemma_layout(bp, c, batch, text_len, seq_pad, true);
  return bp.off + 256;
}

}

namespace {

int gemma_run(const ptk_gemma3_config* c, const ptk_gemma3_weights* wt, const ptk_gemma3_batch* bt,
              const ptk_gemma3_grads* gr, void* ws, size_t ws_bytes, hipStream_t st, bool fwd_only = false) {
  const bool train = gr != nullptr;
  const int B = bt->batch, T = bt->text_len, Nv = bt->num_vision, Sp = bt->seq_pad, S = Nv + T;
  const int lo = bt->label_offset;
  if (Sp % 64 || S > Sp) return set_error("gemma3: seq_pad %d must be a multiple of 64 and >= %d", Sp, S);
  if (Sp > wt->rope_max_pos) return set_error("gemma3: seq_pad %d exceeds rope table (%d)", Sp, wt->rope_max_pos);
  if (c->heads % c->kv_heads) return set_error("gemma3: heads %% kv_heads");
// ... 6 lines not shown
  const int H = c->hidden, I = c->inter, D = c->head_dim, Hq = c->heads, Hkv = c->kv_heads, G = Hq / Hkv;
  const int M = B * Sp, Dq = Hq * D, Dqkv = (Hq + 2 * Hkv) * D, Tl = T - lo, R = B * Tl, V = c->vocab;
  const int Z = B * Hkv, SG = Sp * G, nl = c->layers;
  const float eps = c->eps, scale = 1.0f / sqrtf(c->query_pre_attn_scalar);
  Bump bp(ws);
  GemmaWs w = gemma_layout(bp, c, B, T, Sp, train);
  TailScratchScope tail(w.tail, st);
  CK(tail.status);
  AttnShape ash{B, Sp, Hq, Hkv, D};
  const RowMap ident{0, 0, 0, 0};
  const int Rp = (R + 63) / 64 * 64;
  StageSeq sq(st);
  sq.next("gemma.embed");

  const float escale = bfround_host(sqrtf((float)H));
  CK(launch_build_llm_inputs((const bf16_t*)wt->embed, bt->token_ids, B, T, Nv, S, Sp, H, escale, c->pad_token_id,
                             bt->x, w.key_valid, st));
  w.x[0] = bt->x;
  CK(launch_rmsnorm_fwd(w.x[0], H, ident, wt->layers[0].ln_in, train ? w.L[0].xn_in : w.xn, w.L[0].rstd_in, M, H,
                        eps, st));

  const RowMap lossmap{Tl, 0, Sp, Nv - 1 + lo};

  for (int l = 0; l < nl; ++l) {
    const ptk_gemma3_layer& L = wt->layers[l];
    GemmaLayerSave& sv = w.L[l];
    const bool sliding = (l + 1) % c->sliding_pattern != 0;
    const float* cs = sliding ? wt->rope_cos_local : wt->rope_cos_global;
    const float* sn = sliding ? wt->rope_sin_local : wt->rope_sin_global;
    bf16_t* xin = train ? sv.xn_in : w.xn;
    bf16_t* xff = train ? sv.xn_ff : w.xn;
    bf16_t* hh = train ? sv.h : w.h;
    sq.next("gemma.fwd.attn");
    CK(gemm_split(gemm(xin, H, L.wqkv, H, sv.qkv, Dqkv, M, Dqkv, H), OUT_BF16, w.skpart, w.sk_floats, st));
    CK(launch_qknorm_rope_fwd(sv.qkv, L.q_norm, L.k_norm, cs, sn, ash, eps, sv.Q, sv.K, sv.V, sv.rstd_q, sv.rstd_k,
                              st));
    {
      FlashArgs fa;
      fa.Q = sv.Q; fa.K = sv.K; fa.V = sv.V; fa.O = sv.O; fa.lse = sv.lse;
      fa.rows = SG; fa.nkeys = Sp; fa.D = D;
      fa.ldq = D; fa.ldk = D; fa.ldo = D;
      fa.zin = Hkv; fa.zdiv = Hkv;
      fa.sQ0 = (long)Hkv * SG * D; fa.sQ1 = (long)SG * D;
      fa.sK0 = (long)Hkv * Sp * D; fa.sK1 = (long)Sp * D;
      fa.sO0 = (long)Sp * Hq * D; fa.sO1 = (long)G * D;
      fa.omap = RowMap{G, 0, Hq, 0};
      fa.qdiv = G; fa.causal = 1; fa.window = sliding ? c->sliding_window : 0;
      fa.key_valid = w.key_valid;
      fa.scale = scale;
      StageScope sf("gemma.fwd.flash", st);
      CK(launch_attn_fwd(fa, Z, st));
    }
    CK(gemm_split(gemm(sv.O, Dq, L.wo, Dq, sv.ao, H, M, H, Dq), OUT_BF16, w.skpart, w.sk_floats, st));
    CK(launch_residual_norm_fwd(sv.ao, w.x[l], L.ln_post_attn, L.ln_pre_ff, sv.x2, xff, sv.rstd_ao, sv.rstd_pre, M,
                                H, eps, st));
    sq.next("gemma.fwd.mlp");
    if (l + 1 < nl) {
      GemmArgs g = gemm(xff, H, L.wgu, H, hh, I, M, 2 * I, H);
      g.aux = sv.glu_a; g.aux2 = sv.glu_b; g.ld_aux = I;
      CK(launch_gemm(g, ACT_GEGLU, OUT_BF16, 1, st));
      CK(gemm_split(gemm(hh, I, L.wd, I, sv.dn, H, M, H, I), OUT_BF16, w.skpart, w.sk_floats, st));
    } else {
      GemmArgs g = gemm(xff, H, L.wgu, H, hh, I, R, 2 * I, H);
      g.amap = lossmap;
      g.aux = sv.glu_a; g.aux2 = sv.glu_b; g.ld_aux = I;
      CK(launch_gemm(g, ACT_GEGLU, OUT_BF16, 1, st));
      CK(launch_zero(sv.dn, (size_t)M * H * sizeof(bf16_t), st));
      GemmArgs g2 = gemm(hh, I, L.wd, I, sv.dn, H, R, H, I);
      g2.cmap = lossmap;
      CK(launch_gemm(g2, ACT_NONE, OUT_BF16, 1, st));
    }
    const float* wnext = (l + 1 < nl) ? wt->layers[l + 1].ln_in : nullptr;
    float* rnext = (l + 1 < nl) ? w.L[l + 1].rstd_in : nullptr;
    bf16_t* xnext = (train && l + 1 < nl) ? w.L[l + 1].xn_in : w.xn;
    CK(launch_residual_norm_fwd(sv.dn, sv.x2, L.ln_post_ff, wnext, w.x[l + 1], xnext, sv.rstd_dn, rnext, M, H, eps,
                                st));
  }

  sq.next("gemma.lm_head_ce");
  CK(launch_rmsnorm_fwd(w.x[nl], H, lossmap, wt->final_norm, w.xf, w.rstd_f, R, H, eps, st));
  {
    GemmArgs g = gemm(w.xf, H, wt->embed, H, w.logits, V, R, V, H);
    if (w.ce_stats && !ce_two_pass()) {
      g.row_stats = w.ce_stats;
      g.ld_stats = (V / 64) * 2;
      g.stats_only = lm_stats_only() ? 1 : 0;
    }
    CK(launch_gemm(g, ACT_NONE, OUT_BF16, 1, st));
    CK(launch_count_valid(bt->labels, R, bt->loss_scale, w.gscale, w.count, st));
    if (g.row_stats)
      CK(launch_ce_stats_fwd_bwd(w.logits, V, R, V, w.ce_stats, g.ld_stats, bt->labels, w.row_loss, w.gscale, st));
    else
      CK(launch_ce_fwd_bwd(w.logits, V, R, V, bt->labels, w.row_loss, w.gscale, st));
  }
  CK(launch_loss_reduce(w.row_loss, R, w.count, bt->loss, st));
  if (fwd_only) return 0;
  sq.next("gemma.lm_head_bwd");
  if (train) CK(weight_grad(w.logits, V, ident, V, w.xf, H, ident, H, R, w.TL, w.TX, gr->embed, w.skpart, w.sk_floats, st));
  const bool ks_fits = (double)R * V * 2 + (double)LM_KSLICES * (V / LM_KSLICES) * 2 < 4293918720.0;
  if (R % 256 == 0 && V % (64 * LM_KSLICES) == 0 && ks_fits) {
    GemmArgs g = gemm(w.logits, V, wt->embed_t, V, w.dxf_part, H, R, H, V / LM_KSLICES);
// ... 6 lines not shown
    CK(launch_gemm(g, ACT_NONE, OUT_F32, LM_SPLITK, st));
    if (rem) {
      const long o = (long)LM_SPLITK * kc;
      CK(launch_gemm(gemm(w.logits + o, V, (const bf16_t*)wt->embed_t + o, V, w.dxf_part + (long)LM_SPLITK * R * H, H, R, H, rem),
                     ACT_NONE, OUT_F32, 1, st));
    }
    CK(launch_sum_partials(w.dxf_part, LM_SPLITK + (rem ? 1 : 0), (long)R * H, w.dxf, st));
  }
  float* dR = bt->dx;
  CK(launch_zero(dR, (size_t)M * H * 4, st));
  CK(launch_rmsnorm_bwd_scatter(w.x[nl], lossmap, wt->final_norm, w.rstd_f, w.dxf, dR, R, H, st));
  if (train)
    CK(launch_rms_wgrad(w.x[nl], H, lossmap, w.rstd_f, w.dxf, H, 1, R, H, (bf16_t*)gr->final_norm, w.wpart, st));

  for (int l = nl - 1; l >= 0; --l) {
    const ptk_gemma3_layer& L = wt->layers[l];
    const ptk_gemma3_layer_grads* GL = train ? &gr->layers[l] : nullptr;
    GemmaLayerSave& sv = w.L[l];
    const bool sliding = (l + 1) % c->sliding_pattern != 0;
    const float* cs = sliding ? wt->rope_cos_local : wt->rope_cos_global;
    const float* sn = sliding ? wt->rope_sin_local : wt->rope_sin_global;
    const bool last = l == nl - 1;
    sq.next("gemma.bwd.mlp");
    if (last) {
      CK(launch_post_norm_bwd(dR, sv.dn, L.ln_post_ff, sv.rstd_dn, w.dao, M, H, st));
      if (train)
        CK(launch_rms_wgrad_bx(sv.dn, H, ident, sv.rstd_dn, dR, H, 1, M, H, (bf16_t*)GL->ln_post_ff, w.wpart, st));
    }
    if (train)
      CK(last ? weight_grad(w.dao, H, lossmap, H, sv.h, I, ident, I, R, w.TA, w.TB, GL->wd, w.skpart, w.sk_floats, st)
              : weight_grad(w.dao, H, ident, H, sv.h, I, ident, I, M, w.TA, w.TB, GL->wd, w.skpart, w.sk_floats, st));
    if (!last) {
      if (geglu_split()) {
        CK(launch_gemm(gemm(w.dao, H, L.wd_t, H, w.h, I, M, I, H), ACT_NONE, OUT_BF16, 1, st));
        CK(launch_geglu_bwd(w.h, sv.glu_a, sv.glu_b, w.dgu, M, I, st));
      } else {
        GemmArgs g = gemm(w.dao, H, L.wd_t, H, w.dgu, 2 * I, M, I, H);
        g.aux_in = sv.glu_a;
        g.aux_in2 = sv.glu_b;
        g.ld_aux_in = I;
        CK(launch_gemm(g, ACT_GEGLU_BWD, OUT_BF16, 1, st));
      }
      if (train) CK(weight_grad(w.dgu, 2 * I, ident, 2 * I, sv.xn_ff, H, ident, H, M, w.TA, w.TB, GL->wgu, w.skpart, w.sk_floats, st));
      CK(gemm_split(gemm(w.dgu, 2 * I, L.wgu_t, 2 * I, w.dtmp, H, M, H, 2 * I), OUT_BF16, w.skpart, w.sk_floats, st));
    } else {
      GemmArgs g = gemm(w.dao, H, L.wd_t, H, w.h, I, R, I, H);
      g.amap = lossmap;
      CK(launch_gemm(g, ACT_NONE, OUT_BF16, 1, st));
      CK(launch_geglu_bwd(w.h, sv.glu_a, sv.glu_b, w.dgu, R, I, st));
      if (train) CK(weight_grad(w.dgu, 2 * I, ident, 2 * I, sv.xn_ff, H, lossmap, H, R, w.TA, w.TB, GL->wgu, w.skpart, w.sk_floats, st));
      CK(launch_zero(w.dtmp, (size_t)M * H * sizeof(bf16_t), st));
      GemmArgs g2 = gemm(w.dgu, 2 * I, L.wgu_t, 2 * I, w.dtmp, H, R, H, 2 * I);
      g2.cmap = lossmap;
      CK(launch_gemm(g2, ACT_NONE, OUT_BF16, 1, st));
    }
    sq.next("gemma.bwd.attn");
    CK(residual_norm_bwd_grads(sv.x2, L.ln_pre_ff, sv.rstd_pre, w.dtmp, dR, sv.ao, L.ln_post_attn, sv.rstd_ao, w.dao,
                               M, H, train ? (bf16_t*)GL->ln_pre_ff : nullptr,
                               train ? (bf16_t*)GL->ln_post_attn : nullptr, w.wpart, st));
    if (train)
      CK(weight_grad(w.dao, H, ident, H, sv.O, Dq, ident, Dq, M, w.TA, w.TB, GL->wo, w.skpart, w.sk_floats, st));
    {
      GemmArgs g = gemm(w.dao, H, L.wo_t, H, w.dO, (long)G * D, M, G * D, H);
      g.sB0 = (long)G * D * H; g.sC0 = (long)Sp * G * D;
      g.cmap = RowMap{Sp, 0, (long)Hkv * Sp, 0};
      CK(launch_gemm(g, ACT_NONE, OUT_BF16, Hkv, st));
    }
    FlashBwdArgs dkv_plan;
    dkv_plan.dkv_deferred = 0;
    {
      FlashBwdArgs fb;
      fb.Q = sv.Q; fb.K = sv.K; fb.V = sv.V; fb.O = sv.O; fb.dO = w.dO; fb.lse = sv.lse; fb.delta = w.delta;
      fb.dQ = w.dQ; fb.dK = w.dK; fb.dV = w.dV;
      fb.rows = SG; fb.nkeys = Sp; fb.D = D;
      fb.zin = Hkv; fb.zdiv = Hkv;
      fb.ldo = D; fb.sO0 = (long)Sp * Hq * D; fb.sO1 = (long)G * D;
      fb.omap = RowMap{G, 0, Hq, 0};
      fb.qdiv = G; fb.causal = 1; fb.window = sliding ? c->sliding_window : 0;
      fb.key_valid = w.key_valid;
      fb.scale = scale;
      fb.dkv_part = w.dkv_part; fb.dkv_part_bytes = w.dkv_part_bytes;
      StageScope sf("gemma.bwd.flash", st);
      CK(launch_attn_bwd(fb, Z, st, (dkv_reduce_split() || train) ? nullptr : &dkv_plan));
    }
    CK(launch_qknorm_rope_bwd(sv.qkv, L.q_norm, L.k_norm, cs, sn, ash, sv.rstd_q, sv.rstd_k, w.dQ, w.dK, w.dV, w.dqkv,
                              st, &dkv_plan));
    if (train) {
      CK(launch_qknorm_wgrad(sv.qkv, cs, sn, ash, sv.rstd_q, sv.rstd_k, w.dQ, w.dK, (bf16_t*)GL->q_norm,
                             (bf16_t*)GL->k_norm, w.wpart, st));
      CK(weight_grad(w.dqkv, Dqkv, ident, Dqkv, sv.xn_in, H, ident, H, M, w.TA, w.TB, GL->wqkv, w.skpart, w.sk_floats, st));
    }
    CK(gemm_split(gemm(w.dqkv, Dqkv, L.wqkv_t, Dqkv, w.dtmp, H, M, H, Dqkv), OUT_BF16, w.skpart, w.sk_floats, st));
    if (l > 0) {
      const ptk_gemma3_layer& Lp = wt->layers[l - 1];
      const GemmaLayerSave& sp = w.L[l - 1];
      CK(residual_norm_bwd_grads(w.x[l], L.ln_in, sv.rstd_in, w.dtmp, dR, sp.dn, Lp.ln_post_ff, sp.rstd_dn, w.dao,
                                 M, H, train ? (bf16_t*)GL->ln_in : nullptr,
                                 train ? (bf16_t*)gr->layers[l - 1].ln_post_ff : nullptr, w.wpart, st));
    } else {
      if (train)
        CK(launch_rms_wgrad_bdy(w.x[l], H, ident, sv.rstd_in, w.dtmp, H, M, H, (bf16_t*)GL->ln_in, w.wpart, st));
      CK(launch_rmsnorm_bwd_bdn(w.x[l], L.ln_in, sv.rstd_in, w.dtmp, dR, dR, M, H, st));
    }
  }
  if (train) sq.next("gemma.embed_grad");
  if (train) CK(launch_embed_grad(bt->token_ids, B, T, Nv, Sp, H, escale, dR, (bf16_t*)gr->embed, w.eg_keys, st));
  return 0;
}

}

namespace {

struct GenPass {
  float *xa, *xb, *x2, *rs1, *rs2, *rq, *rk;
  bf16_t *xn, *qkv, *Q, *K, *V, *O, *ao, *h, *dn;
  int32_t* kv;
  float* skp = nullptr;
  size_t skp_bytes = 0;
};
size_t gen_skinny_bytes(const ptk_gemma3_config* c, long rows) {
  if (rows > 256) return 0;
  rows = std::min<long>(rows, 64);
  const int H = c->hidden, I = c->inter, D = c->head_dim, Dq = c->heads * D, Dqkv = (c->heads + 2 * c->kv_heads) * D;
  const int M = (int)rows;
// ... 411 lines not shown
```

### projectiontrainer_amd/csrc/ptk_internal.h

```cpp
#pragma once
#include <hip/hip_runtime.h>
#include <stddef.h>
#include <stdint.h>

#include <type_traits>

#include "common.h"

namespace ptk {

int set_error(const char* fmt, ...);

#ifdef PTK_AB_ENV
}
#include <cstdlib>
namespace ptk {
inline int ab_env(const char* name, int dflt) { const char* e = getenv(name); return e && *e ? atoi(e) : dflt; }
#define PTK_AB(NAME, DFLT) ([] { static const int v_ = ::ptk::ab_env(NAME, DFLT); return v_; }())
#else
#define PTK_AB(NAME, DFLT) (DFLT)
#endif

enum Act { ACT_NONE = 0, ACT_GELU_TANH = 1, ACT_GELU_ERF = 2, ACT_GEGLU = 3,
           ACT_GELU_ERF_BWD = 4, ACT_GEGLU_BWD = 5 };
enum Out { OUT_BF16 = 0, OUT_F32 = 1, OUT_F32_BFR = 2 };

struct GemmArgs {
  const bf16_t* A = nullptr;
  const bf16_t* B = nullptr;
  void* C = nullptr;
  int M = 0, N = 0, K = 0;
  long lda = 0, ldb = 0, ldc = 0;
  int zin = 1;
  long sA0 = 0, sA1 = 0, sB0 = 0, sB1 = 0, sC0 = 0, sC1 = 0;
  float alpha = 1.f;
  const float* bias = nullptr;
  const float* rowadd = nullptr;
  int rowadd_period = 1;
  long ld_rowadd = 0;
  const float* resid = nullptr;
  long ld_resid = 0;
  const bf16_t* resid16 = nullptr;
  long ld_resid16 = 0;
  int bf16_linear = 0;
  bf16_t* aux = nullptr;
  bf16_t* aux2 = nullptr;
  long ld_aux = 0;
  const bf16_t* aux_in = nullptr;
  const bf16_t* aux_in2 = nullptr;
  long ld_aux_in = 0;
  RowMap amap{0, 0, 0, 0};
  RowMap cmap{0, 0, 0, 0};
  float* row_stats = nullptr;
  long ld_stats = 0;
  int stats_only = 0;
  void* tail_ws = nullptr;
};

enum GemmPath { GEMM_PATH_NT = 0, GEMM_PATH_BIG = 1, GEMM_PATH_BIG2 = 2, GEMM_PATH_W4 = 3, GEMM_PATH_NTB = 4,
                GEMM_PATH_P8SK = 5, GEMM_PATH_P8 = 6, GEMM_PATH_TN = 7, GEMM_NPATH = 9 };
int path_counts(int64_t* out, int reset);
int device_cus();

template <class F>
inline bool gemm_act_out(int act, int out, F&& f) {
#define PTK_ACT_OUT(ACT_, OUT_)                                                          \
  if (act == ACT_ && out == OUT_) {                                                      \
    f(std::integral_constant<int, ACT_>{}, std::integral_constant<int, OUT_>{});         \
    return true;                                                                         \
  }
  PTK_ACT_OUT(ACT_NONE, OUT_BF16)
  PTK_ACT_OUT(ACT_NONE, OUT_F32)
  PTK_ACT_OUT(ACT_NONE, OUT_F32_BFR)
  PTK_ACT_OUT(ACT_GELU_TANH, OUT_BF16)
  PTK_ACT_OUT(ACT_GELU_ERF, OUT_BF16)
  PTK_ACT_OUT(ACT_GEGLU, OUT_BF16)
  PTK_ACT_OUT(ACT_GELU_ERF_BWD, OUT_BF16)
  PTK_ACT_OUT(ACT_GEGLU_BWD, OUT_BF16)
#undef PTK_ACT_OUT
  return false;
}

constexpr int W4 = 256;
constexpr int W4_KT = 64;
struct P8Tail {
  int dp_tiles = 0;
  int units = 0;
  int gsplit = 0;
  float* slab = nullptr;
  int zslices = 1;
};
constexpr size_t P8_WAVE_FLOATS = 128 * 64;
constexpr size_t P8_CNT_BYTES = 16384;
struct GemmPlanEnv {
  int ncu = 256;
  int force_tiles = 0;
  bool p8_all = false;
  bool tm_short = true;
  bool lean_epi = true;
  bool streamk = true;
  void* tail_scope = nullptr;
};
GemmPlanEnv gemm_plan_env();
struct GemmPlan {
  int path = GEMM_PATH_NT;
  int tm = 256;
  P8Tail tail;
  bool single_round = false;
};
GemmPlan gemm_plan(const GemmArgs& a, int act, int out, int batch, const GemmPlanEnv& env);
int launch_gemm(const GemmArgs& a, int act, int out, int batch, hipStream_t st, const GemmPlan* planned = nullptr);
struct GemmSplitPlan {
  int slices = 1, kc = 0, rem = 0;
  bool tail_ws = false;
  GemmPlan direct;
};
GemmSplitPlan gemm_split_plan(const GemmArgs& a, int out, long part_floats, const GemmPlanEnv& env);
bool w4_supported(const GemmArgs& a, int act, int out);
int launch_gemm_w4(const GemmArgs& a, int act, int out, hipStream_t st, int max_grid);
double w4_round_fill(long M, long N, int ncu);
bool p8_supported(const GemmArgs& a, int act, int out);
int launch_gemm_p8(const GemmArgs& a, int act, int out, hipStream_t st, const P8Tail& tail, int tm = 256);
int p8_tile_height(const GemmArgs& a, int act, int out, int ncu);
int launch_gemm_p8_kslices(const GemmArgs& a, int slices, hipStream_t st);
int gemm_p8_kslices(const GemmArgs& a, int slices, hipStream_t st);
bool lean_epilogue_candidate(const GemmArgs& a, bool lean_epi);
bool lean_epilogue_ok(const GemmArgs& a, int act, int out, uint32_t& c_bytes, bool lean_epi);
bool lean_epilogue_enabled();
bool tn_supported(const GemmArgs& a, int out, int slices, bool lean_epi);
int tn_slices(const GemmArgs& a, long part_floats, const GemmPlanEnv& env);
P8Tail tn_tail_plan(const GemmArgs& a, void* slab, int ncu);
size_t tn_slab_bytes();
int launch_gemm_tn(const GemmArgs& a, int out, int slices, void* slab, hipStream_t st, long k_rows = -1);
int gemm_tn(const GemmArgs& a, int out, int slices, void* slab, hipStream_t st, long k_rows = -1);
int wgrad_tn_enabled();
size_t p8_tail_scratch_bytes();
size_t p8_tail_scratch_bytes_models();
size_t p8_slab_bytes(long G);
bool streamk_enabled();
P8Tail p8_tail_plan_ws(const GemmArgs& a, long ntile, long G, void* slab, long max_t0, long max_t1);
P8Tail p8_tail_plan(const GemmArgs& a, int act, int out, const GemmPlanEnv& env);
void* tail_scope();
struct TailScratchScope {
// ... 123 lines not shown
  int dkv_deferred = 0;
};

constexpr int DKV_KEYS = 128, DKV_CH = 32;
__host__ __device__ inline void dkv_slab_chunks(const FlashBwdArgs& a, int s, int& c_lo, int& c_hi) {
  int r_lo = 0, r_hi = a.rows;
  if (a.causal) {
    r_lo = min(a.rows, s * DKV_KEYS * a.qdiv);
    if (a.window > 0) r_hi = min(a.rows, (s * DKV_KEYS + DKV_KEYS + a.window - 1) * a.qdiv);
  }
  c_lo = r_lo / DKV_CH;
  c_hi = max(c_lo, (r_hi + DKV_CH - 1) / DKV_CH);
}
__host__ __device__ inline int dkv_pieces(const FlashBwdArgs& a, int s) {
  int lo, hi;
  dkv_slab_chunks(a, s, lo, hi);
  const int n = hi - lo;
  return (a.dkv_target <= 0 || n <= a.dkv_target) ? 1 : (n + a.dkv_target - 1) / a.dkv_target;
}
__host__ __device__ inline int dkv_part_base(const FlashBwdArgs& a, int s) {
  int base = 0;
  for (int t = 0; t < s; ++t) {
    const int pt = dkv_pieces(a, t);
    if (pt > 1) base += pt;
  }
  return base;
}

int launch_attn_bwd(const FlashBwdArgs& a, int nz, hipStream_t st, FlashBwdArgs* defer = nullptr);
size_t attn_bwd_workspace_bytes(const FlashBwdArgs& a, int nz);

int launch_transpose(const bf16_t* in, long ld_in, long sin0, long sin1, int zin, bf16_t* out, long ld_out,
                     long sout0, long sout1, int nz, int rows, int cols, int rows_pad, hipStream_t st);
int launch_im2col(const bf16_t* px, bf16_t* out, int B, int C, int H, int W, int P, hipStream_t st);
int launch_cast_f32_bf16(const float* in, bf16_t* out, long n, hipStream_t st);
int launch_build_llm_inputs(const bf16_t* embed, const int64_t* ids, int B, int T, int Nv, int S, int Spad,
                            int H, float scale_bf16, int pad_id, float* x, int32_t* key_valid,
                            hipStream_t st);
int launch_ce_fwd_bwd(bf16_t* logits, long ld, int R, int V, const int64_t* targets, float* row_loss,
                      const float* gscale, hipStream_t st);
int launch_ce_stats_fwd_bwd(bf16_t* logits, long ld, int R, int V, const float* stats, long ld_stats,
                            const int64_t* targets, float* row_loss, const float* gscale, hipStream_t st);
int launch_count_valid(const int64_t* labels, int n, float loss_scale, float* gscale, float* count,
                       hipStream_t st);
int launch_loss_reduce(const float* row_loss, int R, const float* count, float* loss, hipStream_t st);
int launch_gather_dy(const float* dx, int B, int N, int Spad, int H, bf16_t* dy, hipStream_t st);
int launch_colsum_bf16(const bf16_t* x, int rows, int cols, float* out, float* partial, long part_floats,
                       hipStream_t st);
int launch_sumsq_partial(const float* x, long n, float* partial, int nparts, hipStream_t st);
int launch_clip_adamw(float* p, const float* g, float* m, float* v, long n, const float* partial,
                      int nparts, float grad_scale, float max_norm, float lr, float b1, float b2,
                      float eps, float wd, int step, float* norm_out, hipStream_t st);
int launch_sum_partials(const float* part, int nsplit, long n, float* out, hipStream_t st);
int launch_zero(void* p, size_t bytes, hipStream_t st);
int launch_geglu_bwd(const bf16_t* dh, const bf16_t* g, const bf16_t* u, bf16_t* dgu, long M, int I, hipStream_t st);
int launch_fill_normal_bf16(bf16_t* out, long n, uint64_t seed, float std, float mean, hipStream_t st);

int launch_gen_prompt(const float* src, long ld_b, int B, int P, int Pp, int H, float* x, int32_t* kv, hipStream_t st);
int launch_kv_append(const bf16_t* src, long src_z, bf16_t* dst, long dst_z, int Z, int p0, int n, int D,
                     hipStream_t st);
int launch_gen_sample(const bf16_t* logits, long ld, int B, int V, int do_sample, int top_k, float temperature,
                      float top_p, uint64_t seed, int step, long eos_id, long pad_id, int32_t* finished, int64_t* out,
                      long ld_out, int64_t* next, hipStream_t st);
bool skinny_supported(int M, int N, int K, long lda, long ldb, long ldc, int act);
size_t skinny_part_bytes(int M, int N, int K);
int launch_gemm_skinny(const bf16_t* A, long lda, const bf16_t* B, long ldb, bf16_t* C, long ldc, int M, int N,
// ... 50 lines not shown
```

### projectiontrainer_amd/gemma3.py

```python
from __future__ import annotations

import ctypes as C

import numpy as np
import torch

from . import _lib as L
from . import kernels as K
from .config import Gemma3TextConfig


def _dev(a, dtype, device):
    t = torch.from_numpy(a) if isinstance(a, np.ndarray) else a
    return t.to(device=device, dtype=dtype).contiguous()


def interleave_gate_up(gate, up):
    I, H = gate.shape
    return torch.stack([gate.view(I // 16, 16, H), up.view(I // 16, 16, H)], dim=1).reshape(2 * I, H).contiguous()


def rope_tables(cfg: Gemma3TextConfig, max_pos: int, sliding: bool):
    d = cfg.head_dim
    theta = cfg.rope_local_base_freq if sliding else cfg.rope_theta
    inv = 1.0 / (theta ** (torch.arange(0, d, 2, dtype=torch.int64).float() / d))
    if not sliding and cfg.rope_linear_factor != 1.0:
        inv = inv / cfg.rope_linear_factor
    f = torch.arange(max_pos, dtype=torch.float32)[:, None] * inv[None, :]
    return f.cos().contiguous(), f.sin().contiguous()


class Gemma3CausalLM:
    def __init__(self, cfg: Gemma3TextConfig, params: dict | None, device="cuda", max_pos: int = 2048):
        self.cfg, self.device, self.max_pos = cfg, torch.device(device), max_pos
        self._ws = None
        if params is not None:
            self._load(params)
            self._build_c()

    def _load(self, params):
        cfg, dev = self.cfg, self.device
        bf, f32 = torch.bfloat16, torch.float32
        g = lambda n, dt: _dev(params[n], dt, dev)
        self.embed = g("model.embed_tokens.weight", bf)
        self.final_norm = g("model.norm.weight", f32)
        self.layers = []
        for i in range(cfg.num_hidden_layers):
            p = f"model.layers.{i}."
            wqkv = torch.cat([g(p + f"self_attn.{n}_proj.weight", bf) for n in "qkv"]).contiguous()
            wgu = interleave_gate_up(g(p + "mlp.gate_proj.weight", bf), g(p + "mlp.up_proj.weight", bf))
            lay = dict(wqkv=wqkv, wo=g(p + "self_attn.o_proj.weight", bf), wgu=wgu,
                       wd=g(p + "mlp.down_proj.weight", bf),
                       ln_in=g(p + "input_layernorm.weight", f32),
                       ln_post_attn=g(p + "post_attention_layernorm.weight", f32),
                       ln_pre_ff=g(p + "pre_feedforward_layernorm.weight", f32),
                       ln_post_ff=g(p + "post_feedforward_layernorm.weight", f32),
                       q_norm=g(p + "self_attn.q_norm.weight", f32), k_norm=g(p + "self_attn.k_norm.weight", f32))
            self.layers.append(lay)
        self._derive()

    def _derive(self):
        for lay in self.layers:
            for k in ("wqkv", "wo", "wgu", "wd"):
                lay[k + "_t"] = K.transpose(lay[k])
        self.embed_t = K.transpose(self.embed)
        tabs = [rope_tables(self.cfg, self.max_pos, s) for s in (True, False)]
        (self.cos_l, self.sin_l), (self.cos_g, self.sin_g) = [(c.to(self.device), s.to(self.device))
                                                              for c, s in tabs]

    @staticmethod
    def config_from_hf(c) -> Gemma3TextConfig:
        lt = getattr(c, "layer_types", None)
        rp = getattr(c, "rope_parameters", None)
        if lt is not None and isinstance(rp, dict) and "full_attention" in rp:
            lt = list(lt)
            pattern = lt.index("full_attention") + 1 if "full_attention" in lt else len(lt) + 1
            want = ["sliding_attention" if (i + 1) % pattern else "full_attention" for i in range(len(lt))]
            if lt != want:
                raise ValueError(f"Gemma3 layer_types {lt} are not a periodic sliding/full pattern")
            theta, local = rp["full_attention"]["rope_theta"], rp["sliding_attention"]["rope_theta"]
            factor = float(rp["full_attention"].get("factor", 1.0))
        else:
            pattern = int(c.sliding_window_pattern)
            theta, local = float(c.rope_theta), float(c.rope_local_base_freq)
            rs = getattr(c, "rope_scaling", None) or {}
            kind = rs.get("rope_type", rs.get("type", "default"))
            if kind not in ("default", "linear"):
                raise ValueError(f"Gemma3 rope_scaling type {kind!r} is not supported (default / linear only)")
            factor = float(rs.get("factor", 1.0)) if kind == "linear" else 1.0
        return Gemma3TextConfig(vocab_size=c.vocab_size, hidden_size=c.hidden_size,
                                intermediate_size=c.intermediate_size, num_hidden_layers=c.num_hidden_layers,
                                num_attention_heads=c.num_attention_heads, num_key_value_heads=c.num_key_value_heads,
                                head_dim=c.head_dim, sliding_window=c.sliding_window, sliding_window_pattern=pattern,
                                rope_theta=theta, rope_local_base_freq=local, rope_linear_factor=factor,
                                query_pre_attn_scalar=c.query_pre_attn_scalar, rms_norm_eps=c.rms_norm_eps,
                                pad_token_id=c.pad_token_id if c.pad_token_id is not None else 0)

    @staticmethod
    def check_not_quantized(model):
        qc = getattr(getattr(model, "config", None), "quantization_config", None)
        if (getattr(model, "is_loaded_in_4bit", False) or getattr(model, "is_loaded_in_8bit", False)
                or getattr(model, "is_quantized", False) or qc is not None or hasattr(model, "peft_config")):
            raise ValueError("Gemma3CausalLM.from_hf: quantised / QLoRA (peft) language models are not supported "
                             "by the HIP Stage-1 path; pass the dense bf16 or fp32 Gemma3ForCausalLM "
                             "(run without --enable_qlora)")

    @classmethod
    def from_hf(cls, model, device="cuda", max_pos=2048):
        cls.check_not_quantized(model)
        cfg = cls.config_from_hf(model.config)
        sd = {k: v.detach().float() for k, v in model.state_dict().items()}
        lm = cls(cfg, sd, device, max_pos)
        gc = getattr(model, "generation_config", None)
        if gc is not None:
            lm.generation_defaults = {k: getattr(gc, k) for k in ("top_k", "top_p", "temperature")
                                      if getattr(gc, k, None) is not None}
        return lm

    @classmethod
    def random_init(cls, cfg: Gemma3TextConfig, device="cuda", seed=1, max_pos=2048):
        self = cls(cfg, None, device, max_pos)
        dev = self.device
        H, I = cfg.hidden_size, cfg.intermediate_size
        s = [seed * 100000]

        def nb(*shape, std=0.02):
            s[0] += 1
            return K.fill_normal_(torch.empty(shape, dtype=torch.bfloat16, device=dev), s[0], std)
        z = lambda n: torch.zeros(n, dtype=torch.float32, device=dev)
        self.embed = nb(cfg.vocab_size, H)
        self.final_norm = z(H)
        self.layers = [dict(wqkv=nb(cfg.q_dim + 2 * cfg.kv_dim, H), wo=nb(H, cfg.q_dim), wgu=nb(2 * I, H),
                            wd=nb(H, I), ln_in=z(H), ln_post_attn=z(H), ln_pre_ff=z(H), ln_post_ff=z(H),
                            q_norm=z(cfg.head_dim), k_norm=z(cfg.head_dim))
                       for _ in range(cfg.num_hidden_layers)]
        self._derive()
        self._build_c()
        return self

    def _build_c(self):
        c = self.cfg
        self.c_cfg = L.Gemma3ConfigC(c.vocab_size, c.hidden_size, c.intermediate_size, c.num_hidden_layers,
                                     c.num_attention_heads, c.num_key_value_heads, c.head_dim, c.sliding_window,
                                     c.sliding_window_pattern, c.pad_token_id, float(c.query_pre_attn_scalar),
                                     c.rms_norm_eps)
        keys = ("wqkv", "wqkv_t", "wo", "wo_t", "wgu", "wgu_t", "wd", "wd_t", "ln_in", "ln_post_attn", "ln_pre_ff",
                "ln_post_ff", "q_norm", "k_norm")
        arr = (L.Gemma3LayerC * len(self.layers))()
        for i, lay in enumerate(self.layers):
            arr[i] = L.Gemma3LayerC(*[lay[k].data_ptr() for k in keys])
        self._c_layers = arr
        self.c_w = L.Gemma3WeightsC(self.embed.data_ptr(), self.embed_t.data_ptr(), self.final_norm.data_ptr(),
                                    self.cos_l.data_ptr(), self.sin_l.data_ptr(), self.cos_g.data_ptr(),
                                    self.sin_g.data_ptr(), self.max_pos, C.cast(arr, C.POINTER(L.Gemma3LayerC)))

    @staticmethod
    def seq_pad(seq_len: int) -> int:
        return (seq_len + 63) // 64 * 64

    def workspace(self, batch, text_len, seq_pad):
        n = L.lib().ptk_gemma3_workspace_bytes(self.c_cfg, batch, text_len, seq_pad)
        if self._ws is None or self._ws.numel() < n:
            self._ws = None
            self._ws = torch.empty(n, dtype=torch.uint8, device=self.device)
        return self._ws

    def loss_and_input_grad(self, x, dx, token_ids, labels, num_vision, loss_scale, loss, pad_token_id=None):
        B, T = token_ids.shape
        Sp = x.shape[0] // B
        ws = self.workspace(B, T, Sp)
        bt = L.Gemma3BatchC(B, T, num_vision, Sp, token_ids.data_ptr(), labels.data_ptr(), x.data_ptr(),
                            0 if dx is None else dx.data_ptr(), loss_scale, loss.data_ptr())
        cfg = self.c_cfg
        if pad_token_id is not None and pad_token_id != cfg.pad_token_id:
            cfg = L.Gemma3ConfigC.from_buffer_copy(cfg)
            cfg.pad_token_id = int(pad_token_id)
        fn = "ptk_gemma3_loss_fwd" if dx is None else "ptk_gemma3_loss_fwd_bwd"
        L.check(getattr(L.lib(), fn)(cfg, self.c_w, bt, ws.data_ptr(), ws.numel(), L.stream_ptr(self.device)), fn)

    def get_input_embeddings(self):
        return self.embed

    generation_defaults: dict = {}
# ... 128 lines not shown
```

### projectiontrainer_amd/kernels.py

```python
from __future__ import annotations

import torch

from . import _lib as L
from ._lib import check, ptr


def _require_cuda(*ts):
    for t in ts:
        if t is not None and not t.is_cuda:
            raise L.PtkError("libptk ops need HIP device tensors (no CPU fallback)")


def _bits(t):
    return ptr(t)


def gemm(A, B, *, C=None, out_dtype=torch.bfloat16, act=L.ACT_NONE, alpha=1.0, bias=None, rowadd=None,
         resid=None, aux=None, aux2=None, aux_in=None, aux_in2=None, M=None, N=None, K=None,
         lda=None, ldb=None, ldc=None, batch=1, batch_inner=1, strides=(0, 0, 0, 0, 0, 0),
         amap=(0, 0, 0, 0), cmap=(0, 0, 0, 0), out_mode=None, resid16=None, bf16_linear=False, tail_ws=None):
    _require_cuda(A, B)
    M = A.shape[-2] if M is None else M
    K = A.shape[-1] if K is None else K
    N = B.shape[-2] if N is None else N
    n_out = N // 2 if act == L.ACT_GEGLU else (2 * N if act == L.ACT_GEGLU_BWD else N)
    if C is None:
        C = torch.empty((M, n_out), dtype=out_dtype, device=A.device)
    if out_mode is None:
        out_mode = L.OUT_BF16 if C.dtype == torch.bfloat16 else L.OUT_F32
    d = L.GemmDesc()
    d.A, d.B, d.C = ptr(A), ptr(B), ptr(C)
    d.M, d.N, d.K = M, N, K
    d.lda = A.stride(-2) if lda is None else lda
    d.ldb = B.stride(-2) if ldb is None else ldb
    d.ldc = C.stride(-2) if ldc is None else ldc
    d.batch, d.batch_inner = batch, batch_inner
    d.sA0, d.sA1, d.sB0, d.sB1, d.sC0, d.sC1 = strides
    d.alpha, d.act, d.out = alpha, act, out_mode
    d.bias = ptr(bias)
    if rowadd is not None:
        d.rowadd, d.rowadd_period, d.ld_rowadd = ptr(rowadd), rowadd.shape[0], rowadd.stride(0)
    if resid is not None:
        d.resid, d.ld_resid = ptr(resid), resid.stride(-2)
    if aux is not None:
        d.aux, d.ld_aux = ptr(aux), aux.stride(-2)
    d.aux2 = ptr(aux2)
    if aux_in is not None:
        d.aux_in, d.ld_aux_in = ptr(aux_in), aux_in.stride(-2)
    d.aux_in2 = ptr(aux_in2)
    d.amap = L.RowMap(*amap)
    d.cmap = L.RowMap(*cmap)
    if resid16 is not None:
        d.resid16, d.ld_resid16 = ptr(resid16), resid16.stride(-2)
    d.bf16_linear = int(bool(bf16_linear))
    d.tail_ws = ptr(tail_ws)
    check(L.lib().ptk_gemm(d, L.stream_ptr(A.device)), "ptk_gemm")
    return C


def layernorm(x, w, b, eps):
    _require_cuda(x)
    y = torch.empty(x.shape, dtype=torch.bfloat16, device=x.device)
    rows, cols = x.numel() // x.shape[-1], x.shape[-1]
    check(L.lib().ptk_layernorm(ptr(x), ptr(w), ptr(b), ptr(y), rows, cols, eps, L.stream_ptr(x.device)), "layernorm")
    return y


def rmsnorm(x, w, eps):
    _require_cuda(x)
    rows, cols = x.numel() // x.shape[-1], x.shape[-1]
    y = torch.empty(x.shape, dtype=torch.bfloat16, device=x.device)
    rstd = torch.empty(rows, dtype=torch.float32, device=x.device)
    check(L.lib().ptk_rmsnorm(ptr(x), ptr(w), ptr(y), ptr(rstd), rows, cols, eps, L.stream_ptr(x.device)), "rmsnorm")
    return y, rstd


def rmsnorm_bwd(x, w, rstd, dn, dacc=None):
    rows, cols = x.numel() // x.shape[-1], x.shape[-1]
    dx = torch.empty_like(x)
    check(L.lib().ptk_rmsnorm_bwd(ptr(x), ptr(w), ptr(rstd), ptr(dn), ptr(dacc), ptr(dx), rows, cols,
                                  L.stream_ptr(x.device)), "rmsnorm_bwd")
    return dx


def qknorm_rope(qkv, q_w, k_w, cos_t, sin_t, *, batch, seq, heads, kv_heads, head_dim, eps):
    _require_cuda(qkv)
    dev, G = qkv.device, heads // kv_heads
    Q = torch.empty(batch, kv_heads, seq, G, head_dim, dtype=torch.bfloat16, device=dev)
# ... 48 lines not shown
    for t in (dy, x, grad):
        if t.dtype != torch.bfloat16 or t.dim() != 2 or t.stride(1) != 1:
            raise L.PtkError("weight_grad: dy, x, grad must be 2-D bf16 tensors with unit column stride")
    Ny, Nx = dy.shape[1], x.shape[1]
    if tuple(grad.shape) != (Ny, Nx) or grad.stride(0) != Nx:
        raise L.PtkError("weight_grad: grad must be a contiguous [Ny, Nx] tensor")
    rows = dy.shape[0] if rows is None else rows
    kp = (rows + 63) // 64 * 64
    ta = tb = None
    if mode != 2:
        ta = torch.empty((Ny, kp), dtype=torch.bfloat16, device=dy.device)
        tb = torch.empty((Nx, kp), dtype=torch.bfloat16, device=dy.device)
    pf = 0 if part is None else part.numel()
    check(L.lib().ptk_weight_grad_bf16(ptr(dy), dy.stride(0), ymap[0], ymap[1], ymap[2], Ny, ptr(x), x.stride(0),
                                       xmap[0], xmap[1], xmap[2], Nx, rows, ptr(grad), ptr(ta), ptr(tb), ptr(part),
                                       pf, mode, L.stream_ptr(dy.device)), "weight_grad")
    return grad


def transpose(x, rows_pad=None, out=None):
    squeeze = x.dim() == 2
    x3 = x.unsqueeze(0) if squeeze else x
    Z, rows, cols = x3.shape
    rp = rows if rows_pad is None else rows_pad
    if out is None:
        out = torch.empty((Z, cols, rp), dtype=x.dtype, device=x.device)
    else:
        if tuple(out.shape[-2:]) != (cols, rp) or out.numel() != Z * cols * rp or not out.is_contiguous():
            raise L.PtkError(f"transpose: out {tuple(out.shape)} does not hold [{Z}, {cols}, {rp}]")
        out = out.view(Z, cols, rp)
    check(L.lib().ptk_transpose_bf16(ptr(x3), x3.stride(1), ptr(out), rp, Z, x3.stride(0), cols * rp, rows, cols, rp,
                                     L.stream_ptr(x.device)), "transpose")
    return out[0] if squeeze else out


def cast_bf16(x, out=None):
    out = torch.empty(x.shape, dtype=torch.bfloat16, device=x.device) if out is None else out
    check(L.lib().ptk_cast_f32_bf16(ptr(x), ptr(out), x.numel(), L.stream_ptr(x.device)), "cast")
    return out


def fill_normal_(t, seed, std=0.02, mean=0.0):
    assert t.dtype == torch.bfloat16 and t.is_contiguous()
    check(L.lib().ptk_fill_normal_bf16(ptr(t), t.numel(), seed & (2**64 - 1), std, mean, L.stream_ptr(t.device)),
          "fill_normal")
    return t


def flash_attn(Q, K, V, O, *, rows, nkeys, head_dim, ldq, ldk, ldo, batch, batch_inner=1, zdiv=1,
               strides=(0, 0, 0, 0, 0, 0), qmap=(0, 0, 0, 0), omap=(0, 0, 0, 0), qdiv=1, causal=False,
               window=0, key_valid=None, scale=1.0, lse=None):
    _require_cuda(Q, K, V, O)
    d = L.FlashDesc()
    d.Q, d.K, d.V, d.O, d.lse = ptr(Q), ptr(K), ptr(V), ptr(O), ptr(lse)
    d.rows, d.nkeys, d.head_dim = rows, nkeys, head_dim
    d.ldq, d.ldk, d.ldo = ldq, ldk, ldo
    d.batch, d.batch_inner, d.zdiv = batch, batch_inner, zdiv
    d.sQ0, d.sQ1, d.sK0, d.sK1, d.sO0, d.sO1 = strides
    d.qmap, d.omap = L.RowMap(*qmap), L.RowMap(*omap)
    d.qdiv, d.causal, d.window = qdiv, int(causal), window
    d.key_valid, d.scale = ptr(key_valid), scale
    check(L.lib().ptk_flash_attn_fwd(d, L.stream_ptr(Q.device)), "flash_attn_fwd")
    return O


def flash_attn_bwd(Q, K, V, O, dO, lse, *, rows, nkeys, head_dim, batch, batch_inner=1, zdiv=1, ldo=None,
# ... 24 lines not shown
```

### projectiontrainer_amd/siglip.py

```python
from __future__ import annotations

import ctypes as C

import numpy as np
import torch

from . import _lib as L
from . import kernels as K
from .config import SiglipVisionConfig


def _dev(a, dtype, device):
    t = torch.from_numpy(a) if isinstance(a, np.ndarray) else a
    return t.to(device=device, dtype=dtype).contiguous()


class SiglipVisionTower:
    def __init__(self, cfg: SiglipVisionConfig, params: dict, device="cuda", prefix="vision_model."):
        self.cfg, self.device = cfg, torch.device(device)
        bf, f32 = torch.bfloat16, torch.float32
        g = lambda n, dt: _dev(params[prefix + n], dt, self.device)
        D = cfg.hidden_size
        self.patch_w = g("embeddings.patch_embedding.weight", bf).reshape(D, -1).contiguous()
        self.patch_b = g("embeddings.patch_embedding.bias", f32)
# ... 24 lines not shown
                                 layer_norm_eps=vc.layer_norm_eps)
        sd = {"vision_model." + k: v.detach().float() for k, v in vm.state_dict().items()}
        return cls(cfg, sd, device)

    @classmethod
    def random_init(cls, cfg: SiglipVisionConfig, device="cuda", seed=0):
        dev = torch.device(device)
        self = cls.__new__(cls)
        self.cfg, self.device = cfg, dev
        D, I = cfg.hidden_size, cfg.intermediate_size
        s = [seed * 1000]

        def nb(*shape, std=0.02):
            s[0] += 1
            return K.fill_normal_(torch.empty(shape, dtype=torch.bfloat16, device=dev), s[0], std)
        f = lambda n, v=0.0: torch.full((n,), v, dtype=torch.float32, device=dev)
        self.patch_w = nb(D, cfg.patch_dim)
        self.patch_b = f(D)
        self.pos = nb(cfg.num_patches, D).float()
        self.post_w, self.post_b = f(D, 1.0), f(D)
        self.layers = [dict(wqkv=nb(3 * D, D), bqkv=f(3 * D), wo=nb(D, D), bo=f(D), w1=nb(I, D), b1=f(I),
                            w2=nb(D, I), b2=f(D), ln1_w=f(D, 1.0), ln1_b=f(D), ln2_w=f(D, 1.0), ln2_b=f(D))
                       for _ in range(cfg.num_hidden_layers)]
        self._build_c()
        self._ws = None
        return self

    def _build_c(self):
        c = self.cfg
        self.c_cfg = L.SiglipConfigC(c.image_size, c.patch_size, c.num_channels, c.hidden_size,
                                     c.num_attention_heads, c.intermediate_size, c.num_hidden_layers,
                                     c.layer_norm_eps)
        arr = (L.SiglipLayerC * len(self.layers))()
        for i, lay in enumerate(self.layers):
            arr[i] = L.SiglipLayerC(*[lay[k].data_ptr() for k in ("wqkv", "bqkv", "wo", "bo", "w1", "b1", "w2", "b2",
                                                                   "ln1_w", "ln1_b", "ln2_w", "ln2_b")])
        self._c_layers = arr
        self.c_w = L.SiglipWeightsC(self.patch_w.data_ptr(), self.patch_b.data_ptr(), self.pos.data_ptr(),
                                    self.post_w.data_ptr(), self.post_b.data_ptr(),
                                    C.cast(arr, C.POINTER(L.SiglipLayerC)))

    def workspace(self, batch):
        n = L.lib().ptk_siglip_workspace_bytes(self.c_cfg, batch)
        if self._ws is None or self._ws.numel() < n:
            self._ws = torch.empty(n, dtype=torch.uint8, device=self.device)
        return self._ws

    def forward_into(self, pixels_bf16, out):
        B = pixels_bf16.shape[0]
        ws = self.workspace(B)
        L.check(L.lib().ptk_siglip_fwd(self.c_cfg, self.c_w, B, pixels_bf16.data_ptr(), out.data_ptr(),
                                       ws.data_ptr(), ws.numel(), L.stream_ptr(self.device)), "ptk_siglip_fwd")
        return out

    def __call__(self, pixel_values):
        if not pixel_values.is_cuda:
            raise L.PtkError("SiglipVisionTower runs on the HIP device only")
        px = pixel_values.to(torch.bfloat16).contiguous()
        B = px.shape[0]
        out = torch.empty((B * self.cfg.num_patches, self.cfg.hidden_size), dtype=torch.bfloat16, device=self.device)
        self.forward_into(px, out)
        return out.view(B, self.cfg.num_patches, self.cfg.hidden_size)
```

### projectiontrainer_amd/stage2.py

```python
from __future__ import annotations

import math

import torch
import torch.distributed as dist

from . import _lib as L
from . import kernels as K
from .gemma3 import Gemma3CausalLM
from .projectors import MLPProjector
from .siglip import SiglipVisionTower
from .stage1 import cosine_lambda

LAYER_KEYS = ("wqkv", "wo", "wgu", "wd", "ln_in", "ln_post_attn", "ln_pre_ff", "ln_post_ff", "q_norm", "k_norm")
NORM_KEYS = ("ln_in", "ln_post_attn", "ln_pre_ff", "ln_post_ff", "q_norm", "k_norm")
HF_NORM = {"ln_in": "input_layernorm", "ln_post_attn": "post_attention_layernorm",
           "ln_pre_ff": "pre_feedforward_layernorm", "ln_post_ff": "post_feedforward_layernorm",
           "q_norm": "self_attn.q_norm", "k_norm": "self_attn.k_norm"}


def deinterleave_gate_up(wgu):
    I2, H = wgu.shape
    v = wgu.view(I2 // 32, 2, 16, H)
    return v[:, 0].reshape(I2 // 2, H), v[:, 1].reshape(I2 // 2, H)
# ... 8 lines not shown
        cfg, dev = llm.cfg, llm.device
        segs = [("embed", tuple(llm.embed.shape))]
        for i, lay in enumerate(llm.layers):
            segs += [(f"{i}.{k}", tuple(lay[k].shape)) for k in ("wqkv", "wo", "wgu", "wd")]
        norm_segs = [("final_norm", (cfg.hidden_size,))]
        for i, lay in enumerate(llm.layers):
            norm_segs += [(f"{i}.{k}", tuple(lay[k].shape)) for k in NORM_KEYS]
        off, self.offsets = 0, {}
        for j, (name, shape) in enumerate(segs + norm_segs):
            if j == len(segs):
                self.norm_lo = off
            self.offsets[name] = (off, shape)
            n = math.prod(shape)
            off += (n + self.ALIGN - 1) // self.ALIGN * self.ALIGN
        self.norm_hi = off
        unit = self.ALIGN * world_size
        self.numel = (off + unit - 1) // unit * unit
        self.flat = torch.zeros(self.numel, dtype=torch.bfloat16, device=dev)
        self.grad = torch.zeros(self.numel, dtype=torch.bfloat16, device=dev)
        self.view("embed").copy_(llm.embed)
        self.view("final_norm").copy_(llm.final_norm)
        for i, lay in enumerate(llm.layers):
            for k in LAYER_KEYS:
                self.view(f"{i}.{k}").copy_(lay[k])
        llm.embed = self.view("embed")
        self.norm32 = torch.zeros(self.norm_hi - self.norm_lo, dtype=torch.float32, device=dev)
        n32 = lambda name: self.norm32[self.offsets[name][0] - self.norm_lo:][:math.prod(self.offsets[name][1])]
        llm.final_norm = n32("final_norm")
        for i, lay in enumerate(llm.layers):
            for k in ("wqkv", "wo", "wgu", "wd"):
                lay[k] = self.view(f"{i}.{k}")
            for k in NORM_KEYS:
                lay[k] = n32(f"{i}.{k}").view(self.offsets[f"{i}.{k}"][1])
        self.refresh()
        llm._build_c()
        self._build_grads_c()

    def view(self, name, buf=None):
        off, shape = self.offsets[name]
        return (self.flat if buf is None else buf)[off:off + math.prod(shape)].view(shape)

    def grad_view(self, name):
        return self.view(name, self.grad)

    def _build_grads_c(self):
        arr = (L.Gemma3LayerGradsC * len(self.llm.layers))()
        for i in range(len(self.llm.layers)):
            arr[i] = L.Gemma3LayerGradsC(*[self.grad_view(f"{i}.{k}").data_ptr() for k in LAYER_KEYS])
        self._c_layer_grads = arr
        self.c_grads = L.Gemma3GradsC(self.grad_view("embed").data_ptr(), self.grad_view("final_norm").data_ptr(),
                                      arr)

    def refresh(self):
        llm = self.llm
        self.norm32.copy_(self.flat[self.norm_lo:self.norm_hi])
        for lay in llm.layers:
            for k in ("wqkv", "wo", "wgu", "wd"):
                K.transpose(lay[k], out=lay[k + "_t"])
        K.transpose(llm.embed, out=llm.embed_t)

    def zero_grad(self):
        self.grad.zero_()

    def shard(self, rank):
        n = self.numel // self.world
        return rank * n, n
# ... 128 lines not shown
        L.check(L.lib().ptk_adamw_bf16(p.data_ptr(), g.data_ptr(), self.exp_avg.data_ptr(),
                                       self.exp_avg_sq.data_ptr(), n, self.sumsq.data_ptr(), self.max_norm, lr, b1,
                                       b2, self.eps, self.wd, self.opt_step, self.grad_norm.data_ptr(), stream),
                "adamw_bf16")
        if self.zero1:
            self._shard_param.copy_(p)
            all_gather_(st.flat, self._shard_param, self.world, self.pg)
        st.refresh()
        st.zero_grad()
        self.sched_step += self.world
        self.last_lr = lr
        return lr

    @property
    def scheduler_lr(self):
        return self.lr0 * cosine_lambda(self.sched_step, self.warmup, self.total)

    def optimizer_state(self):
        return {"exp_avg": self.exp_avg.cpu(), "exp_avg_sq": self.exp_avg_sq.cpu(), "step": self.opt_step,
                "sched_step": self.sched_step, "shard": (self.shard_lo, self.shard_n), "world": self.world,
                "rank": self.rank, "numel": self.state.numel}

    def load_optimizer_state(self, sd):
        if (sd["world"], sd["rank"], sd["numel"]) != (self.world, self.rank, self.state.numel):
            raise ValueError(f"optimizer shard of world {sd['world']} rank {sd['rank']} (store {sd['numel']}) does "
                             f"not match this engine (world {self.world} rank {self.rank} store {self.state.numel})")
        self.exp_avg.copy_(sd["exp_avg"])
        self.exp_avg_sq.copy_(sd["exp_avg_sq"])
        self.opt_step, self.sched_step = int(sd["step"]), int(sd["sched_step"])


def synthetic_engine(cfg, device="cuda", seed=0, **kw):
    vision = SiglipVisionTower.random_init(cfg.vision, device, seed)
    llm = Gemma3CausalLM.random_init(cfg.text, device, seed + 1, max_pos=Gemma3CausalLM.seq_pad(cfg.seq_len))
    torch.manual_seed(seed + 2)
    proj = MLPProjector(cfg.vision.hidden_size, cfg.text.hidden_size, cfg.expansion_factor, device=device)
    return Stage2Engine(vision, llm, proj, **kw)


def reduce_scatter_(out_shard, flat, world, rank, group=None):
    if dist.get_backend(group) == "gloo":
        t = flat.float()
        dist.all_reduce(t, op=dist.ReduceOp.SUM, group=group)
        n = out_shard.numel()
        out_shard.copy_(t[rank * n:(rank + 1) * n])
    else:
        dist.reduce_scatter_tensor(out_shard, flat, op=dist.ReduceOp.SUM, group=group)
    return out_shard


def all_gather_(flat, shard, world, group=None):
    if dist.get_backend(group) == "gloo":
        parts = [torch.empty(shard.shape, dtype=torch.float32, device=shard.device) for _ in range(world)]
        dist.all_gather(parts, shard.float(), group=group)
        flat.copy_(torch.cat(parts))
    else:
        dist.all_gather_into_tensor(flat, shard, group=group)
    return flat
```

### projectiontrainer_amd/vqa_trainer.py

```python
from __future__ import annotations

import logging
import math
import os

import torch

from . import dist as D
from .gemma3 import Gemma3CausalLM
from .projectors import MLPProjector
from .siglip import SiglipVisionTower
from .stage2 import Stage2Engine

logger = logging.getLogger(__name__)


def vqa_collate_fn(batch, tokenizer):
    pad_id, side = tokenizer.pad_token_id, getattr(tokenizer, "padding_side", "right")

    def pad(seqs):
        n = max(s.shape[0] for s in seqs)
        out = []
        for s in seqs:
            p = torch.full((n - s.shape[0],), pad_id, dtype=s.dtype)
# ... 9 lines not shown
                 val_dataset, output_dir: str, batch_size: int, learning_rate: float, weight_decay: float,
                 num_epochs: int, gradient_accumulation_steps: int, warmup_ratio: float, freeze_vision_encoder: bool,
                 freeze_projection_layer: bool, freeze_llm: bool, enable_qlora: bool, train_ve_first_epoch: bool,
                 wandb_project: str, log_fn=None, seed: int = 0, generate_max_new_tokens: int = 512,
                 generate_num_beams: int = 3, generate_do_sample: bool = True, generate_top_k: int = 50,
                 generate_top_p: float = 0.9, generate_seed: int = 0):
        if enable_qlora:
            raise NotImplementedError("VQATrainerStage2 (HIP): QLoRA / 4-bit LLMs are not supported; run with the "
                                      "dense bf16 LLM and --unfreeze_llm")
        if freeze_llm or not freeze_projection_layer or not freeze_vision_encoder or train_ve_first_epoch:
            raise NotImplementedError("VQATrainerStage2 (HIP) supports the BASELINE cfg4 setting: LLM unfrozen, "
                                      "projector and vision encoder frozen")
        if accelerator is None:
            accelerator = D.DistState(gradient_accumulation_steps)
        elif not isinstance(accelerator, D.DistState):
            accelerator = D.from_accelerator(accelerator)
        self.accelerator = acc = accelerator
        self.device = acc.device
        self.tokenizer = tokenizer
        self.output_dir, self.num_epochs, self.batch_size = output_dir, num_epochs, batch_size
        self.train_dataset, self.val_dataset = train_dataset, val_dataset
        self.wandb_project, self.log_fn, self.seed = wandb_project, log_fn, seed
        self.gas = gradient_accumulation_steps
        self.gen_kwargs = dict(max_new_tokens=generate_max_new_tokens, num_beams=generate_num_beams,
                               do_sample=generate_do_sample, top_k=generate_top_k, top_p=generate_top_p)
        self.generate_seed = generate_seed
        self.validation_dir = os.path.join(output_dir, "validation_examples")
        if acc.is_main_process:
            os.makedirs(self.validation_dir, exist_ok=True)

        self.vision_encoder = vision_encoder if isinstance(vision_encoder, SiglipVisionTower) \
            else SiglipVisionTower.from_hf(vision_encoder, self.device)
        self.language_model = language_model if isinstance(language_model, Gemma3CausalLM) \
            else Gemma3CausalLM.from_hf(language_model, self.device, max_pos=4096)
        if not isinstance(projection_layer, MLPProjector):
            sd = projection_layer.state_dict()
            p = MLPProjector(sd["model.0.weight"].shape[1], sd["model.2.weight"].shape[0])
            p.load_state_dict({k: v.detach().float().cpu() for k, v in sd.items()})
            projection_layer = p
        self.projection_layer = projection_layer.to(self.device)

        n_batches = math.ceil(len(train_dataset) / batch_size)
        self.max_train_steps = num_epochs * math.ceil(n_batches / gradient_accumulation_steps)
        self.num_warmup_steps = math.ceil(warmup_ratio * self.max_train_steps)
        pad = getattr(tokenizer, "pad_token_id", None)
        self.engine = Stage2Engine(self.vision_encoder, self.language_model, self.projection_layer,
                                   learning_rate=learning_rate, weight_decay=weight_decay,
                                   gradient_accumulation_steps=gradient_accumulation_steps,
                                   warmup_steps=self.num_warmup_steps, total_steps=self.max_train_steps,
                                   world_size=acc.num_processes, rank=acc.process_index,
                                   pad_token_id=-1 if pad is None else int(pad))
        self.global_step = 0

    def _batches(self, dataset, epoch, shuffle=True):
        acc = self.accelerator
        for idx in D.shard_batches(len(dataset), self.batch_size, acc.process_index, acc.num_processes, epoch,
                                   self.seed, shuffle):
            b = vqa_collate_fn([dataset[int(i)] for i in idx], self.tokenizer)
            yield {k: v.to(self.device, non_blocking=True) for k, v in b.items()}

    def _log(self, d, step):
        if self.accelerator.is_main_process:
            if self.log_fn is not None:
                self.log_fn(d, step)
            else:
                logger.info("step %d %s", step, d)

# ... 118 lines not shown
```

Baseline: 316.2 images/sec.

## Pre-pack frozen weights into k-step tiles for contiguous GEMM B loads

Adds a packed k-step tiled, swizzled copy of frozen bf16 weight matrices (SigLIP layers and frozen Gemma3 layers). The W4 and P8 GEMM kernels gain a template variant that DMAs B from this packed layout, so each wave reads one contiguous 1 KiB block per k-step instead of strided rows. The aim is better memory coalescing and fewer address computations on B loads. It costs extra weight memory and a packing pass at load time, and it falls back to the old path for batched or k-sliced calls and for trainable LLM weights.

```diff
diff --git a/include/ptk.h b/include/ptk.h
--- a/include/ptk.h
+++ b/include/ptk.h
@@ -55,8 +55,11 @@
   int64_t ld_resid16;
   int bf16_linear;
   void* tail_ws;
+  const void* B_kt;
 } ptk_gemm_desc;
 int ptk_gemm(const ptk_gemm_desc* d, void* stream);
+int64_t ptk_kstep_tile_offset(int64_t row, int64_t k, int64_t K);
+int ptk_pack_kstep_tiles_bf16(const void* src, void* dst, int N, int K, void* stream);
 #define PTK_GEMM_TAIL_COUNTER_BYTES 16384
 size_t ptk_gemm_tail_scratch_bytes(void);
 int ptk_gemm_tail_split(const ptk_gemm_desc* d);
@@ -143,6 +146,7 @@
   const void* w2;    const float* b2;
   const float* ln1_w; const float* ln1_b;
   const float* ln2_w; const float* ln2_b;
+  const void* wqkv_kt; const void* wo_kt; const void* w1_kt; const void* w2_kt;
 } ptk_siglip_layer;
 
 typedef struct {
@@ -188,6 +192,10 @@
   const void* wd;    const void* wd_t;
   const float* ln_in; const float* ln_post_attn; const float* ln_pre_ff; const float* ln_post_ff;
   const float* q_norm; const float* k_norm;
+  const void* wqkv_kt; const void* wqkv_t_kt;
+  const void* wo_kt;   const void* wo_t_kt;
+  const void* wgu_kt;  const void* wgu_t_kt;
+  const void* wd_kt;   const void* wd_t_kt;
 } ptk_gemma3_layer;
 
 typedef struct {
diff --git a/projectiontrainer_amd/_lib.py b/projectiontrainer_amd/_lib.py
--- a/projectiontrainer_amd/_lib.py
+++ b/projectiontrainer_amd/_lib.py
@@ -32,7 +32,7 @@
                 ("aux", c_void_p), ("aux2", c_void_p), ("ld_aux", c_int64),
                 ("aux_in", c_void_p), ("aux_in2", c_void_p), ("ld_aux_in", c_int64),
                 ("amap", RowMap), ("cmap", RowMap), ("resid16", c_void_p), ("ld_resid16", c_int64),
-                ("bf16_linear", c_int), ("tail_ws", c_void_p)]
+                ("bf16_linear", c_int), ("tail_ws", c_void_p), ("B_kt", c_void_p)]
 
 
 class FlashDesc(C.Structure):
@@ -64,7 +64,8 @@
 class SiglipLayerC(C.Structure):
     _fields_ = [("wqkv", c_void_p), ("bqkv", c_void_p), ("wo", c_void_p), ("bo", c_void_p),
                 ("w1", c_void_p), ("b1", c_void_p), ("w2", c_void_p), ("b2", c_void_p),
-                ("ln1_w", c_void_p), ("ln1_b", c_void_p), ("ln2_w", c_void_p), ("ln2_b", c_void_p)]
+                ("ln1_w", c_void_p), ("ln1_b", c_void_p), ("ln2_w", c_void_p), ("ln2_b", c_void_p),
+                ("wqkv_kt", c_void_p), ("wo_kt", c_void_p), ("w1_kt", c_void_p), ("w2_kt", c_void_p)]
 
 
 class SiglipWeightsC(C.Structure):
@@ -89,7 +90,9 @@
     _fields_ = [("wqkv", c_void_p), ("wqkv_t", c_void_p), ("wo", c_void_p), ("wo_t", c_void_p),
                 ("wgu", c_void_p), ("wgu_t", c_void_p), ("wd", c_void_p), ("wd_t", c_void_p),
                 ("ln_in", c_void_p), ("ln_post_attn", c_void_p), ("ln_pre_ff", c_void_p),
-                ("ln_post_ff", c_void_p), ("q_norm", c_void_p), ("k_norm", c_void_p)]
+                ("ln_post_ff", c_void_p), ("q_norm", c_void_p), ("k_norm", c_void_p),
+                ("wqkv_kt", c_void_p), ("wqkv_t_kt", c_void_p), ("wo_kt", c_void_p), ("wo_t_kt", c_void_p),
+                ("wgu_kt", c_void_p), ("wgu_t_kt", c_void_p), ("wd_kt", c_void_p), ("wd_t_kt", c_void_p)]
 
 
 class Gemma3WeightsC(C.Structure):
@@ -157,6 +160,8 @@
                                      c_void_p, c_int64, c_int, c_int64, c_int64, c_int, c_int,
                                      c_void_p, c_void_p, c_void_p, c_void_p, c_int64, c_int, c_void_p]),
     "ptk_cast_f32_bf16": (c_int, [c_void_p, c_void_p, c_int64, c_void_p]),
+    "ptk_kstep_tile_offset": (c_int64, [c_int64, c_int64, c_int64]),
+    "ptk_pack_kstep_tiles_bf16": (c_int, [c_void_p, c_void_p, c_int, c_int, c_void_p]),
     "ptk_fill_normal_bf16": (c_int, [c_void_p, c_int64, c_uint64, c_float, c_float, c_void_p]),
     "ptk_gemm_timer_enable": (c_int, [c_int]),
     "ptk_gemm_force_small_tiles": (c_int, [c_int]),
diff --git a/projectiontrainer_amd/csrc/capi.cpp b/projectiontrainer_amd/csrc/capi.cpp
--- a/projectiontrainer_amd/csrc/capi.cpp
+++ b/projectiontrainer_amd/csrc/capi.cpp
@@ -33,6 +33,7 @@
   a.amap = to_map(d->amap); a.cmap = to_map(d->cmap);
   a.resid16 = (const bf16_t*)d->resid16; a.ld_resid16 = d->ld_resid16; a.bf16_linear = d->bf16_linear;
   a.tail_ws = d->tail_ws;
+  a.B_kt = (const bf16_t*)d->B_kt;
   return a;
 }
 
@@ -156,6 +157,10 @@
   return launch_transpose_rows((const bf16_t*)in, ld_in, m, rows, cols, (bf16_t*)out, ld_out, rows_pad, ST);
 }
 
+int64_t ptk_kstep_tile_offset(int64_t row, int64_t k, int64_t K) { return kstep_tile_offset(row, k, K); }
+int ptk_pack_kstep_tiles_bf16(const void* src, void* dst, int N, int K, void* stream) {
+  return launch_pack_kstep_tiles((const bf16_t*)src, (bf16_t*)dst, N, K, ST);
+}
 int ptk_cast_f32_bf16(const float* in, void* out, int64_t n, void* stream) {
   return launch_cast_f32_bf16(in, (bf16_t*)out, n, ST);
 }
diff --git a/projectiontrainer_amd/csrc/gemm.hip b/projectiontrainer_amd/csrc/gemm.hip
--- a/projectiontrainer_amd/csrc/gemm.hip
+++ b/projectiontrainer_amd/csrc/gemm.hip
@@ -707,8 +707,13 @@
   const dim3 grid_big((unsigned)((long)((a.M + BIG - 1) / BIG) * ((a.N + BIG - 1) / BIG)), 1, 1);
   switch (plan.path) {
     case GEMM_PATH_P8:
-    case GEMM_PATH_P8SK: return launch_gemm_p8(a, act, out, st, plan.tail, plan.tm);
-    case GEMM_PATH_W4: return launch_gemm_w4(a, act, out, st, 0);
+    case GEMM_PATH_P8SK:
+    case GEMM_PATH_W4: {
+      GemmArgs b = a;
+      if (!b_ktiled_ok(a, plan, act, batch)) b.B_kt = nullptr;
+      if (plan.path == GEMM_PATH_W4) return launch_gemm_w4(b, act, out, st, 0);
+      return launch_gemm_p8(b, act, out, st, plan.tail, plan.tm);
+    }
     case GEMM_PATH_BIG2:
       gemm_act_out(act, out, [&](auto A, auto O) {
         hipLaunchKernelGGL((gemm_big2_kernel<A(), O()>), grid_big, dim3(512), 0, st, a);
diff --git a/projectiontrainer_amd/csrc/gemm_plan.cpp b/projectiontrainer_amd/csrc/gemm_plan.cpp
--- a/projectiontrainer_amd/csrc/gemm_plan.cpp
+++ b/projectiontrainer_amd/csrc/gemm_plan.cpp
@@ -193,6 +193,18 @@
   else if (staggered_big(a, e)) p.path = GEMM_PATH_BIG2;
   else if (big(a, e)) p.path = GEMM_PATH_BIG;
   return p;
+}
+
+long kstep_tile_offset(long row, long k, long K) {
+  const long rr = row & 15, chunk = (k >> 3) & 3;
+  const long unit = 4 * rr + (chunk ^ ((rr >> 1) & 2));
+  return ((row >> 4) * (K / 32) + (k >> 5)) * 1024 + unit * 16 + (k & 7) * 2;
+}
+
+bool b_ktiled_ok(const GemmArgs& a, const GemmPlan& plan, int act, int batch) {
+  if (!a.B_kt || batch != 1 || !bkt_act(act)) return false;
+  if (plan.path != GEMM_PATH_W4 && plan.path != GEMM_PATH_P8 && plan.path != GEMM_PATH_P8SK) return false;
+  return a.ldb == a.K && a.K % 32 == 0 && a.N % 16 == 0 && !((uintptr_t)a.B_kt & 15);
 }
 
 GemmSplitPlan gemm_split_plan(const GemmArgs& a, int out, long part_floats, const GemmPlanEnv& env) {
diff --git a/projectiontrainer_amd/csrc/gemm_w4.hip b/projectiontrainer_amd/csrc/gemm_w4.hip
--- a/projectiontrainer_amd/csrc/gemm_w4.hip
+++ b/projectiontrainer_amd/csrc/gemm_w4.hip
@@ -22,7 +22,7 @@
 
 namespace ptk {
 
-template <int ACT, int OUT, bool LEAN = false>
+template <int ACT, int OUT, bool LEAN = false, bool BKT = false>
 __global__ void __launch_bounds__(256, 1) gemm_w4_kernel(GemmArgs p, uint32_t a_bytes, uint32_t b_bytes,
                                                          uint32_t c_bytes) {
   __shared__ __attribute__((aligned(16))) char smem[W4_NSLOT * W4_SLOT];
@@ -42,7 +42,9 @@
   const int nks = 2 * nt;
   const int total_ks = ((ntile - loc + G - 1) / G) * nks;
 
-  const u32x4_t rsa = w4_rsrc(p.A, a_bytes), rsb = w4_rsrc(p.B, b_bytes);
+  constexpr bool bkt = BKT;
+  constexpr uint32_t bks = BKT ? 1024u : (uint32_t)(W4_KS * 2);
+  const u32x4_t rsa = w4_rsrc(p.A, a_bytes), rsb = w4_rsrc(bkt ? p.B_kt : p.B, b_bytes);
 
   uint32_t offa[4], offb[4];
 #pragma unroll
@@ -50,7 +52,8 @@
     const int lr = wave * 64 + 16 * j + (lane >> 2);
     const int lc = (lane & 3) ^ ((lane >> 3) & 2);
     offa[j] = (uint32_t)lr * (uint32_t)p.lda * 2u + lc * 16;
-    offb[j] = (uint32_t)lr * (uint32_t)p.ldb * 2u + lc * 16;
+    offb[j] = bkt ? (uint32_t)(wave * 4 + j) * (uint32_t)p.K * 32u + lane * 16
+                  : (uint32_t)lr * (uint32_t)p.ldb * 2u + lc * 16;
   }
   const uint32_t lds_base = __builtin_amdgcn_readfirstlane(lds_addr(smem));
   const uint32_t lds_dma = lds_base + wave * 64 * 64;
@@ -105,7 +108,7 @@
     constexpr bool first = decltype(first_c)::value;
     const uint32_t ba = frag_a + rs, bb = frag_b + rs;
     const uint32_t da = lds_dma + ws, db = da + W4_SOPB;
-    const uint32_t sa = dsa + dks * (W4_KS * 2), sb = dsb + dks * (W4_KS * 2);
+    const uint32_t sa = dsa + dks * (W4_KS * 2), sb = dsb + dks * bks;
 #pragma unroll
     for (int q = 0; q < 16; ++q) {
 #if PTK_W4_RDS == 1
@@ -145,7 +148,7 @@
 #pragma unroll
   for (int b = 0; b < 4; ++b) {
     const uint32_t da = lds_dma + b * W4_SLOT, db = da + W4_SOPB;
-    const uint32_t sa = dsa + dks * (W4_KS * 2), sb = dsb + dks * (W4_KS * 2);
+    const uint32_t sa = dsa + dks * (W4_KS * 2), sb = dsb + dks * bks;
 #pragma unroll
     for (int j = 0; j < 4; ++j) {
       W4_DMA(rsa, offa[j], sa, da + j * 1024);
@@ -217,6 +220,17 @@
 
 bool lean_epilogue_enabled() { return PTK_AB("PTK_LEAN_EPI", 1) != 0; }
 
+template <int ACT, int OUT, bool LEAN>
+static void w4_launch(const GemmArgs& a, long grid, hipStream_t st, uint32_t ab, uint32_t bb, uint32_t cb) {
+  if constexpr (bkt_act(ACT)) {
+    if (a.B_kt) {
+      hipLaunchKernelGGL((gemm_w4_kernel<ACT, OUT, LEAN, true>), dim3((unsigned)grid), dim3(256), 0, st, a, ab, bb, cb);
+      return;
+    }
+  }
+  hipLaunchKernelGGL((gemm_w4_kernel<ACT, OUT, LEAN, false>), dim3((unsigned)grid), dim3(256), 0, st, a, ab, bb, cb);
+}
+
 int launch_gemm_w4(const GemmArgs& a, int act, int out, hipStream_t st, int max_grid) {
   const long ntile = (long)((a.M + W4 - 1) / W4) * ((a.N + W4 - 1) / W4);
   long grid = std::min<long>(ntile, max_grid > 0 ? max_grid : device_cus());
@@ -228,9 +242,9 @@
   const uint32_t bb = (uint32_t)std::min<double>((double)a.N * a.ldb * 2, 2147483000.0);
   uint32_t cb = 0;
   if (lean_epilogue_ok(a, act, out, cb, lean_epilogue_enabled())) {
-#define PTK_W4L_CASE(ACT_)                                                                                   \
-    if (act == ACT_)                                                                                         \
-      hipLaunchKernelGGL((gemm_w4_kernel<ACT_, OUT_BF16, true>), dim3((unsigned)grid), dim3(256), 0, st, a, ab, bb, cb);
+#define PTK_W4L_CASE(ACT_) \
+    if (act == ACT_)       \
+      w4_launch<ACT_, OUT_BF16, true>(a, grid, st, ab, bb, cb);
     PTK_W4L_CASE(ACT_NONE)
     PTK_W4L_CASE(ACT_GELU_TANH)
     PTK_W4L_CASE(ACT_GEGLU_BWD)
@@ -238,7 +252,7 @@
     return hipGetLastError() == hipSuccess ? 0 : set_error("gemm_w4 launch failed");
   }
   if (!gemm_act_out(act, out, [&](auto A, auto O) {
-        hipLaunchKernelGGL((gemm_w4_kernel<A(), O()>), dim3((unsigned)grid), dim3(256), 0, st, a, ab, bb, 0u);
+        w4_launch<A(), O(), false>(a, grid, st, ab, bb, 0u);
       }))
     return set_error("gemm_w4: unsupported (act=%d, out=%d)", act, out);
   return hipGetLastError() == hipSuccess ? 0 : set_error("gemm_w4 launch failed");
@@ -262,7 +276,7 @@
 #define P8_DSREAD(DST, ADDR, OFF) W4_DSREAD(DST, ADDR, OFF)
 #define P8_LGKM(N) asm volatile("s_waitcnt lgkmcnt(" #N ")" ::: "memory")
 #endif
-template <int ACT, int OUT, bool SK, bool LEAN = false, int TM = 256>
+template <int ACT, int OUT, bool SK, bool LEAN = false, int TM = 256, bool BKT = false>
 __global__ void __launch_bounds__(512, 1) gemm_p8_kernel(GemmArgs p, uint32_t a_bytes, uint32_t b_bytes, P8Tail tl,
                                                          uint32_t c_bytes) {
   static_assert(TM == 256 || ((TM == 224 || TM == 192 || TM == 160) && !SK), "shorter tiles: whole tiles only");
@@ -322,7 +336,9 @@
       k0 = (int)(b & 0xffffu); k1 = (int)(b >> 16);
     }
   };
-  const u32x4_t rsa = w4_rsrc(p.A, a_bytes), rsb = w4_rsrc(p.B, b_bytes);
+  constexpr bool bkt = BKT;
+  constexpr uint32_t bks = BKT ? 1024u : (uint32_t)(W4_KS * 2);
+  const u32x4_t rsa = w4_rsrc(p.A, a_bytes), rsb = w4_rsrc(bkt ? p.B_kt : p.B, b_bytes);
 
   uint32_t offa[2], offb[2];
 #pragma unroll
@@ -330,7 +346,8 @@
     const int lr = wave * 32 + 16 * j + (lane >> 2);
     const int lc = (lane & 3) ^ ((lane >> 3) & 2);
     offa[j] = (uint32_t)lr * (uint32_t)p.lda * 2u + lc * 16;
-    offb[j] = (uint32_t)lr * (uint32_t)p.ldb * 2u + lc * 16;
+    offb[j] = bkt ? (uint32_t)(wave * 2 + j) * (uint32_t)p.K * 32u + lane * 16
+                  : (uint32_t)lr * (uint32_t)p.ldb * 2u + lc * 16;
   }
   const uint32_t lds_base = __builtin_amdgcn_readfirstlane(lds_addr(smem));
   const uint32_t lds_dma = lds_base + wave * 32 * 64;
@@ -349,7 +366,7 @@
     }
     dsa = __builtin_amdgcn_readfirstlane((uint32_t)(bm * TM + (int)p.amap.off) * (uint32_t)p.lda * 2u + kz +
                                          (uint32_t)k0 * (W4_KT * 2));
-    dsb = __builtin_amdgcn_readfirstlane((uint32_t)(bn * W4) * (uint32_t)p.ldb * 2u + kz + (uint32_t)k0 * (W4_KT * 2));
+    dsb = __builtin_amdgcn_readfirstlane((uint32_t)(bn * W4) * (uint32_t)p.ldb * 2u + kz + (uint32_t)k0 * (2u * bks));
     dlen = 2 * (k1 - k0);
   };
   auto dma_advance = [&]() {
@@ -386,7 +403,7 @@
     constexpr int half = decltype(half_c)::value;
     const uint32_t ba = frag_a + rs, bb = frag_b + rs;
     const uint32_t da = lds_dma + ws, db = da + W4_SOPB;
-    const uint32_t sa = dsa + dks * (W4_KS * 2), sb = dsb + dks * (W4_KS * 2);
+    const uint32_t sa = dsa + dks * (W4_KS * 2), sb = dsb + dks * bks;
 #pragma unroll
     for (int q = 0; q < RB; ++q) {
       if constexpr (RB == 8) {
@@ -457,7 +474,7 @@
 #pragma unroll
     for (int b = 0; b < 4; ++b) {
       const uint32_t da = lds_dma + b * W4_SLOT, db = da + W4_SOPB;
-      const uint32_t sa = dsa + dks * (W4_KS * 2), sb = dsb + dks * (W4_KS * 2);
+      const uint32_t sa = dsa + dks * (W4_KS * 2), sb = dsb + dks * bks;
 #pragma unroll
       for (int j = 0; j < 2; ++j) {
         if (a_dma) W4_DMA(rsa, offa[j], sa, da + j * 1024);
@@ -625,6 +642,7 @@
     return set_error("gemm_p8_kslices: operands past 4 GiB");
   GemmArgs g = a;
   g.M = a.M * slices;
+  g.B_kt = nullptr;
   P8Tail tl;
   tl.zslices = slices;
   const long ntile = (long)(g.M / W4) * ((g.N + W4 - 1) / W4);
@@ -636,6 +654,20 @@
   return hipGetLastError() == hipSuccess ? 0 : set_error("gemm_p8_kslices launch failed");
 }
 
+template <int ACT, int OUT, bool SK, bool LEAN, int TM>
+static void p8_launch(const GemmArgs& a, long grid, hipStream_t st, uint32_t ab, uint32_t bb, const P8Tail& tl,
+                      uint32_t cb) {
+  if constexpr (bkt_act(ACT)) {
+    if (a.B_kt) {
+      hipLaunchKernelGGL((gemm_p8_kernel<ACT, OUT, SK, LEAN, TM, true>), dim3((unsigned)grid), dim3(512), 0, st, a, ab,
+                         bb, tl, cb);
+      return;
+    }
+  }
+  hipLaunchKernelGGL((gemm_p8_kernel<ACT, OUT, SK, LEAN, TM, false>), dim3((unsigned)grid), dim3(512), 0, st, a, ab, bb,
+                     tl, cb);
+}
+
 template <int TM>
 static int launch_p8_short(const GemmArgs& a, int act, int out, hipStream_t st, long grid, bool lean_epi) {
   const uint32_t ab = (uint32_t)std::min<double>((double)(a.M + a.amap.off) * a.lda * 2, 2147483000.0);
@@ -644,23 +676,17 @@
   uint32_t cb = 0;
   if (lean_epilogue_ok(a, act, out, cb, lean_epi)) {
     if (act == ACT_NONE)
-      hipLaunchKernelGGL((gemm_p8_kernel<ACT_NONE, OUT_BF16, false, true, TM>), dim3((unsigned)grid), dim3(512), 0,
-                         st, a, ab, bb, tl, cb);
+      p8_launch<ACT_NONE, OUT_BF16, false, true, TM>(a, grid, st, ab, bb, tl, cb);
     else
-      hipLaunchKernelGGL((gemm_p8_kernel<ACT_GELU_TANH, OUT_BF16, false, true, TM>), dim3((unsigned)grid),
-                         dim3(512), 0, st, a, ab, bb, tl, cb);
+      p8_launch<ACT_GELU_TANH, OUT_BF16, false, true, TM>(a, grid, st, ab, bb, tl, cb);
   } else if (act == ACT_GELU_TANH) {
-    hipLaunchKernelGGL((gemm_p8_kernel<ACT_GELU_TANH, OUT_BF16, false, false, TM>), dim3((unsigned)grid), dim3(512),
-                       0, st, a, ab, bb, tl, 0u);
+    p8_launch<ACT_GELU_TANH, OUT_BF16, false, false, TM>(a, grid, st, ab, bb, tl, 0u);
   } else if (out == OUT_BF16) {
-    hipLaunchKernelGGL((gemm_p8_kernel<ACT_NONE, OUT_BF16, false, false, TM>), dim3((unsigned)grid), dim3(512), 0,
-                       st, a, ab, bb, tl, 0u);
+    p8_launch<ACT_NONE, OUT_BF16, false, false, TM>(a, grid, st, ab, bb, tl, 0u);
   } else if (out == OUT_F32) {
-    hipLaunchKernelGGL((gemm_p8_kernel<ACT_NONE, OUT_F32, false, false, TM>), dim3((unsigned)grid), dim3(512), 0,
-                       st, a, ab, bb, tl, 0u);
+    p8_launch<ACT_NONE, OUT_F32, false, false, TM>(a, grid, st, ab, bb, tl, 0u);
   } else {
-    hipLaunchKernelGGL((gemm_p8_kernel<ACT_NONE, OUT_F32_BFR, false, false, TM>), dim3((unsigned)grid), dim3(512),
-                       0, st, a, ab, bb, tl, 0u);
+    p8_launch<ACT_NONE, OUT_F32_BFR, false, false, TM>(a, grid, st, ab, bb, tl, 0u);
   }
   return hipGetLastError() == hipSuccess ? 0 : set_error("gemm_p8 launch failed");
 }
@@ -690,12 +716,10 @@
   if (tl.units) {
     if (act != ACT_NONE) return set_error("gemm_p8: the stream-K tail takes ACT_NONE only (act=%d)", act);
     if (lean_epilogue_ok(a, act, out, cb, lean_epi)) {
-      hipLaunchKernelGGL((gemm_p8_kernel<ACT_NONE, OUT_BF16, true, true>), dim3((unsigned)grid), dim3(512), 0, st, a,
-                         ab, bb, tl, cb);
+      p8_launch<ACT_NONE, OUT_BF16, true, true, 256>(a, grid, st, ab, bb, tl, cb);
     } else if (!gemm_act_out(act, out, [&](auto A, auto O) {
                  if constexpr (A() == ACT_NONE)
-                   hipLaunchKernelGGL((gemm_p8_kernel<ACT_NONE, O(), true>), dim3((unsigned)grid), dim3(512), 0, st, a,
-                                      ab, bb, tl, 0u);
+                   p8_launch<ACT_NONE, O(), true, false, 256>(a, grid, st, ab, bb, tl, 0u);
                })) {
       return set_error("gemm_p8: unsupported (act=%d, out=%d)", act, out);
     }
@@ -705,8 +729,7 @@
   if (lean_epilogue_ok(a, act, out, cb, lean_epi)) {
 #define PTK_P8L_CASE(ACT_)                                                                                   \
     if (act == ACT_)                                                                                         \
-      hipLaunchKernelGGL((gemm_p8_kernel<ACT_, OUT_BF16, false, true>), dim3((unsigned)grid), dim3(512), 0, st, a, ab, \
-                         bb, tl, cb);
+      p8_launch<ACT_, OUT_BF16, false, true, 256>(a, grid, st, ab, bb, tl, cb);
     PTK_P8L_CASE(ACT_NONE)
     PTK_P8L_CASE(ACT_GELU_TANH)
     PTK_P8L_CASE(ACT_GEGLU_BWD)
@@ -714,7 +737,7 @@
     return hipGetLastError() == hipSuccess ? 0 : set_error("gemm_p8 launch failed");
   }
   if (!gemm_act_out(act, out, [&](auto A, auto O) {
-        hipLaunchKernelGGL((gemm_p8_kernel<A(), O(), false>), dim3((unsigned)grid), dim3(512), 0, st, a, ab, bb, tl, 0u);
+        p8_launch<A(), O(), false, false, 256>(a, grid, st, ab, bb, tl, 0u);
       }))
     return set_error("gemm_p8: unsupported (act=%d, out=%d)", act, out);
   return hipGetLastError() == hipSuccess ? 0 : set_error("gemm_p8 launch failed");
diff --git a/projectiontrainer_amd/csrc/misc.hip b/projectiontrainer_amd/csrc/misc.hip
--- a/projectiontrainer_amd/csrc/misc.hip
+++ b/projectiontrainer_amd/csrc/misc.hip
@@ -90,6 +90,26 @@
   RET_OK("im2col");
 }
 
+__global__ void __launch_bounds__(256) pack_kstep_tiles_kernel(const bf16_t* __restrict__ src, bf16_t* __restrict__ dst,
+                                                               long units, int ksteps) {
+  const long u = (long)blockIdx.x * 256 + threadIdx.x;
+  if (u >= units) return;
+  const int i = (int)(u & 63);
+  const long blk = u >> 6, g = blk / ksteps, s = blk - g * ksteps;
+  const long row = 16 * g + (i >> 2);
+  const int chunk = (i & 3) ^ ((i >> 3) & 2);
+  const uint4 v = *reinterpret_cast<const uint4*>(src + (row * ksteps + s) * 32 + chunk * 8);
+  *reinterpret_cast<uint4*>(dst + u * 8) = v;
+}
+int launch_pack_kstep_tiles(const bf16_t* src, bf16_t* dst, int N, int K, hipStream_t st) {
+  if (N <= 0 || K <= 0 || N % 16 || K % 32) return set_error("pack_kstep_tiles: N %d %% 16, K %d %% 32", N, K);
+  if (!src || !dst || (((uintptr_t)src | (uintptr_t)dst) & 15)) return set_error("pack_kstep_tiles: 16-B aligned src / dst");
+  const long units = (long)N * K / 8;
+  hipLaunchKernelGGL(pack_kstep_tiles_kernel, dim3((unsigned)((units + 255) / 256)), dim3(256), 0, st, src, dst, units,
+                     K / 32);
+  RET_OK("pack_kstep_tiles");
+}
+
 __global__ void cast_f32_bf16_kernel(const float* __restrict__ in, bf16_t* __restrict__ out, long n) {
   const long i = ((long)blockIdx.x * 256 + threadIdx.x) * 4;
   if (i + 3 < n) {
diff --git a/projectiontrainer_amd/csrc/models.cpp b/projectiontrainer_amd/csrc/models.cpp
--- a/projectiontrainer_amd/csrc/models.cpp
+++ b/projectiontrainer_amd/csrc/models.cpp
@@ -88,8 +88,10 @@
   return v != 0;
 }
 
-GemmArgs gemm(const void* A, long lda, const void* B, long ldb, void* C, long ldc, int M, int N, int K) {
+GemmArgs gemm(const void* A, long lda, const void* B, long ldb, void* C, long ldc, int M, int N, int K,
+              const void* B_kt = nullptr) {
   GemmArgs g;
+  g.B_kt = (const bf16_t*)B_kt;
   g.A = (const bf16_t*)A; g.B = (const bf16_t*)B; g.C = C;
   g.lda = lda; g.ldb = ldb; g.ldc = ldc;
   g.M = M; g.N = N; g.K = K;
@@ -246,6 +248,7 @@
   }
   const int kc = sp.kc, nfull = sp.slices, rem = sp.rem;
   GemmArgs b = a;
+  b.B_kt = nullptr;
   b.C = part; b.ldc = a.N; b.K = kc;
   b.sA0 = kc; b.sB0 = kc; b.sC0 = (long)a.M * a.N;
   b.bf16_linear = 0; b.resid16 = nullptr; b.ld_resid16 = 0;
@@ -360,7 +363,7 @@
     sq.next("siglip.attn");
     CK(launch_layernorm_bf16(w.h, L.ln1_w, L.ln1_b, w.a, M, D, c->eps, st));
     {
-      GemmArgs g = gemm(w.a, D, L.wqkv, D, w.qkv, 3 * D, M, 3 * D, D);
+      GemmArgs g = gemm(w.a, D, L.wqkv, D, w.qkv, 3 * D, M, 3 * D, D, L.wqkv_kt);
       g.bias = L.bqkv;
       CK(launch_gemm(g, ACT_NONE, OUT_BF16, 1, st));
     }
@@ -377,19 +380,19 @@
       CK(launch_attn_fwd(fa, B * Hh, st));
     }
     {
-      GemmArgs g = gemm(w.o, D, L.wo, D, w.h, D, M, D, D);
+      GemmArgs g = gemm(w.o, D, L.wo, D, w.h, D, M, D, D, L.wo_kt);
       g.bias = L.bo; g.bf16_linear = 1; g.resid16 = w.h; g.ld_resid16 = D;
       CK(launch_gemm(g, ACT_NONE, OUT_BF16, 1, st));
     }
     sq.next("siglip.mlp");
     CK(launch_layernorm_bf16(w.h, L.ln2_w, L.ln2_b, w.a, M, D, c->eps, st));
     {
-      GemmArgs g = gemm(w.a, D, L.w1, D, w.mlp, I, M, I, D);
+      GemmArgs g = gemm(w.a, D, L.w1, D, w.mlp, I, M, I, D, L.w1_kt);
       g.bias = L.b1;
       CK(launch_gemm(g, ACT_GELU_TANH, OUT_BF16, 1, st));
     }
     {
-      GemmArgs g = gemm(w.mlp, I, L.w2, I, w.h, D, M, D, I);
+      GemmArgs g = gemm(w.mlp, I, L.w2, I, w.h, D, M, D, I, L.w2_kt);
       g.bias = L.b2; g.bf16_linear = 1; g.resid16 = w.h; g.ld_resid16 = D;
       CK(launch_gemm(g, ACT_NONE, OUT_BF16, 1, st));
     }
@@ -462,7 +465,7 @@
     bf16_t* xff = train ? sv.xn_ff : w.xn;
     bf16_t* hh = train ? sv.h : w.h;
     sq.next("gemma.fwd.attn");
-    CK(gemm_split(gemm(xin, H, L.wqkv, H, sv.qkv, Dqkv, M, Dqkv, H), OUT_BF16, w.skpart, w.sk_floats, st));
+    CK(gemm_split(gemm(xin, H, L.wqkv, H, sv.qkv, Dqkv, M, Dqkv, H, L.wqkv_kt), OUT_BF16, w.skpart, w.sk_floats, st));
     CK(launch_qknorm_rope_fwd(sv.qkv, L.q_norm, L.k_norm, cs, sn, ash, eps, sv.Q, sv.K, sv.V, sv.rstd_q, sv.rstd_k,
                               st));
     {
@@ -481,22 +484,22 @@
       StageScope sf("gemma.fwd.flash", st);
       CK(launch_attn_fwd(fa, Z, st));
     }
-    CK(gemm_split(gemm(sv.O, Dq, L.wo, Dq, sv.ao, H, M, H, Dq), OUT_BF16, w.skpart, w.sk_floats, st));
+    CK(gemm_split(gemm(sv.O, Dq, L.wo, Dq, sv.ao, H, M, H, Dq, L.wo_kt), OUT_BF16, w.skpart, w.sk_floats, st));
     CK(launch_residual_norm_fwd(sv.ao, w.x[l], L.ln_post_attn, L.ln_pre_ff, sv.x2, xff, sv.rstd_ao, sv.rstd_pre, M,
                                 H, eps, st));
     sq.next("gemma.fwd.mlp");
     if (l + 1 < nl) {
-      GemmArgs g = gemm(xff, H, L.wgu, H, hh, I, M, 2 * I, H);
+      GemmArgs g = gemm(xff, H, L.wgu, H, hh, I, M, 2 * I, H, L.wgu_kt);
       g.aux = sv.glu_a; g.aux2 = sv.glu_b; g.ld_aux = I;
       CK(launch_gemm(g, ACT_GEGLU, OUT_BF16, 1, st));
-      CK(gemm_split(gemm(hh, I, L.wd, I, sv.dn, H, M, H, I), OUT_BF16, w.skpart, w.sk_floats, st));
+      CK(gemm_split(gemm(hh, I, L.wd, I, sv.dn, H, M, H, I, L.wd_kt), OUT_BF16, w.skpart, w.sk_floats, st));
     } else {
-      GemmArgs g = gemm(xff, H, L.wgu, H, hh, I, R, 2 * I, H);
+      GemmArgs g = gemm(xff, H, L.wgu, H, hh, I, R, 2 * I, H, L.wgu_kt);
       g.amap = lossmap;
       g.aux = sv.glu_a; g.aux2 = sv.glu_b; g.ld_aux = I;
       CK(launch_gemm(g, ACT_GEGLU, OUT_BF16, 1, st));
       CK(launch_zero(sv.dn, (size_t)M * H * sizeof(bf16_t), st));
-      GemmArgs g2 = gemm(hh, I, L.wd, I, sv.dn, H, R, H, I);
+      GemmArgs g2 = gemm(hh, I, L.wd, I, sv.dn, H, R, H, I, L.wd_kt);
       g2.cmap = lossmap;
       CK(launch_gemm(g2, ACT_NONE, OUT_BF16, 1, st));
     }
@@ -569,25 +572,25 @@
               : weight_grad(w.dao, H, ident, H, sv.h, I, ident, I, M, w.TA, w.TB, GL->wd, w.skpart, w.sk_floats, st));
     if (!last) {
       if (geglu_split()) {
-        CK(launch_gemm(gemm(w.dao, H, L.wd_t, H, w.h, I, M, I, H), ACT_NONE, OUT_BF16, 1, st));
+        CK(launch_gemm(gemm(w.dao, H, L.wd_t, H, w.h, I, M, I, H, L.wd_t_kt), ACT_NONE, OUT_BF16, 1, st));
         CK(launch_geglu_bwd(w.h, sv.glu_a, sv.glu_b, w.dgu, M, I, st));
       } else {
-        GemmArgs g = gemm(w.dao, H, L.wd_t, H, w.dgu, 2 * I, M, I, H);
+        GemmArgs g = gemm(w.dao, H, L.wd_t, H, w.dgu, 2 * I, M, I, H, L.wd_t_kt);
         g.aux_in = sv.glu_a;
         g.aux_in2 = sv.glu_b;
         g.ld_aux_in = I;
         CK(launch_gemm(g, ACT_GEGLU_BWD, OUT_BF16, 1, st));
       }
       if (train) CK(weight_grad(w.dgu, 2 * I, ident, 2 * I, sv.xn_ff, H, ident, H, M, w.TA, w.TB, GL->wgu, w.skpart, w.sk_floats, st));
-      CK(gemm_split(gemm(w.dgu, 2 * I, L.wgu_t, 2 * I, w.dtmp, H, M, H, 2 * I), OUT_BF16, w.skpart, w.sk_floats, st));
+      CK(gemm_split(gemm(w.dgu, 2 * I, L.wgu_t, 2 * I, w.dtmp, H, M, H, 2 * I, L.wgu_t_kt), OUT_BF16, w.skpart, w.sk_floats, st));
     } else {
-      GemmArgs g = gemm(w.dao, H, L.wd_t, H, w.h, I, R, I, H);
+      GemmArgs g = gemm(w.dao, H, L.wd_t, H, w.h, I, R, I, H, L.wd_t_kt);
       g.amap = lossmap;
       CK(launch_gemm(g, ACT_NONE, OUT_BF16, 1, st));
       CK(launch_geglu_bwd(w.h, sv.glu_a, sv.glu_b, w.dgu, R, I, st));
       if (train) CK(weight_grad(w.dgu, 2 * I, ident, 2 * I, sv.xn_ff, H, lossmap, H, R, w.TA, w.TB, GL->wgu, w.skpart, w.sk_floats, st));
       CK(launch_zero(w.dtmp, (size_t)M * H * sizeof(bf16_t), st));
-      GemmArgs g2 = gemm(w.dgu, 2 * I, L.wgu_t, 2 * I, w.dtmp, H, R, H, 2 * I);
+      GemmArgs g2 = gemm(w.dgu, 2 * I, L.wgu_t, 2 * I, w.dtmp, H, R, H, 2 * I, L.wgu_t_kt);
       g2.cmap = lossmap;
       CK(launch_gemm(g2, ACT_NONE, OUT_BF16, 1, st));
     }
@@ -598,7 +601,7 @@
     if (train)
       CK(weight_grad(w.dao, H, ident, H, sv.O, Dq, ident, Dq, M, w.TA, w.TB, GL->wo, w.skpart, w.sk_floats, st));
     {
-      GemmArgs g = gemm(w.dao, H, L.wo_t, H, w.dO, (long)G * D, M, G * D, H);
+      GemmArgs g = gemm(w.dao, H, L.wo_t, H, w.dO, (long)G * D, M, G * D, H, L.wo_t_kt);
       g.sB0 = (long)G * D * H; g.sC0 = (long)Sp * G * D;
       g.cmap = RowMap{Sp, 0, (long)Hkv * Sp, 0};
       CK(launch_gemm(g, ACT_NONE, OUT_BF16, Hkv, st));
@@ -627,7 +630,7 @@
                              (bf16_t*)GL->k_norm, w.wpart, st));
       CK(weight_grad(w.dqkv, Dqkv, ident, Dqkv, sv.xn_in, H, ident, H, M, w.TA, w.TB, GL->wqkv, w.skpart, w.sk_floats, st));
     }
-    CK(gemm_split(gemm(w.dqkv, Dqkv, L.wqkv_t, Dqkv, w.dtmp, H, M, H, Dqkv), OUT_BF16, w.skpart, w.sk_floats, st));
+    CK(gemm_split(gemm(w.dqkv, Dqkv, L.wqkv_t, Dqkv, w.dtmp, H, M, H, Dqkv, L.wqkv_t_kt), OUT_BF16, w.skpart, w.sk_floats, st));
     if (l > 0) {
       const ptk_gemma3_layer& Lp = wt->layers[l - 1];
       const GemmaLayerSave& sp = w.L[l - 1];
diff --git a/projectiontrainer_amd/csrc/ptk_internal.h b/projectiontrainer_amd/csrc/ptk_internal.h
--- a/projectiontrainer_amd/csrc/ptk_internal.h
+++ b/projectiontrainer_amd/csrc/ptk_internal.h
@@ -55,6 +55,7 @@
   long ld_stats = 0;
   int stats_only = 0;
   void* tail_ws = nullptr;
+  const bf16_t* B_kt = nullptr;
 };
 
 enum GemmPath { GEMM_PATH_NT = 0, GEMM_PATH_BIG = 1, GEMM_PATH_BIG2 = 2, GEMM_PATH_W4 = 3, GEMM_PATH_NTB = 4,
@@ -109,6 +110,9 @@
   bool single_round = false;
 };
 GemmPlan gemm_plan(const GemmArgs& a, int act, int out, int batch, const GemmPlanEnv& env);
+constexpr bool bkt_act(int act) { return act != ACT_GELU_ERF && act != ACT_GELU_ERF_BWD; }
+long kstep_tile_offset(long row, long k, long K);
+bool b_ktiled_ok(const GemmArgs& a, const GemmPlan& plan, int act, int batch);
 int launch_gemm(const GemmArgs& a, int act, int out, int batch, hipStream_t st, const GemmPlan* planned = nullptr);
 struct GemmSplitPlan {
   int slices = 1, kc = 0, rem = 0;
@@ -298,6 +302,7 @@
 
 int launch_transpose(const bf16_t* in, long ld_in, long sin0, long sin1, int zin, bf16_t* out, long ld_out,
                      long sout0, long sout1, int nz, int rows, int cols, int rows_pad, hipStream_t st);
+int launch_pack_kstep_tiles(const bf16_t* src, bf16_t* dst, int N, int K, hipStream_t st);
 int launch_im2col(const bf16_t* px, bf16_t* out, int B, int C, int H, int W, int P, hipStream_t st);
 int launch_cast_f32_bf16(const float* in, bf16_t* out, long n, hipStream_t st);
 int launch_build_llm_inputs(const bf16_t* embed, const int64_t* ids, int B, int T, int Nv, int S, int Spad,
diff --git a/projectiontrainer_amd/gemma3.py b/projectiontrainer_amd/gemma3.py
--- a/projectiontrainer_amd/gemma3.py
+++ b/projectiontrainer_amd/gemma3.py
@@ -30,9 +30,14 @@
     return f.cos().contiguous(), f.sin().contiguous()
 
 
+KT_KEYS = ("wqkv", "wqkv_t", "wo", "wo_t", "wgu", "wgu_t", "wd", "wd_t")
+
+
 class Gemma3CausalLM:
-    def __init__(self, cfg: Gemma3TextConfig, params: dict | None, device="cuda", max_pos: int = 2048):
+    def __init__(self, cfg: Gemma3TextConfig, params: dict | None, device="cuda", max_pos: int = 2048,
+                 frozen: bool = True):
         self.cfg, self.device, self.max_pos = cfg, torch.device(device), max_pos
+        self.frozen = frozen
         self._ws = None
         if params is not None:
             self._load(params)
@@ -63,10 +68,18 @@
         for lay in self.layers:
             for k in ("wqkv", "wo", "wgu", "wd"):
                 lay[k + "_t"] = K.transpose(lay[k])
+            for k in KT_KEYS:
+                lay[k + "_kt"] = K.frozen_kstep_tiles(lay[k]) if self.frozen else None
         self.embed_t = K.transpose(self.embed)
         tabs = [rope_tables(self.cfg, self.max_pos, s) for s in (True, False)]
         (self.cos_l, self.sin_l), (self.cos_g, self.sin_g) = [(c.to(self.device), s.to(self.device))
                                                               for c, s in tabs]
+
+    def drop_ktiled(self):
+        self.frozen = False
+        for lay in self.layers:
+            for k in KT_KEYS:
+                lay[k + "_kt"] = None
 
     @staticmethod
     def config_from_hf(c) -> Gemma3TextConfig:
@@ -106,11 +119,11 @@
                              "(run without --enable_qlora)")
 
     @classmethod
-    def from_hf(cls, model, device="cuda", max_pos=2048):
+    def from_hf(cls, model, device="cuda", max_pos=2048, frozen=True):
         cls.check_not_quantized(model)
         cfg = cls.config_from_hf(model.config)
         sd = {k: v.detach().float() for k, v in model.state_dict().items()}
-        lm = cls(cfg, sd, device, max_pos)
+        lm = cls(cfg, sd, device, max_pos, frozen)
         gc = getattr(model, "generation_config", None)
         if gc is not None:
             lm.generation_defaults = {k: getattr(gc, k) for k in ("top_k", "top_p", "temperature")
@@ -118,8 +131,8 @@
         return lm
 
     @classmethod
-    def random_init(cls, cfg: Gemma3TextConfig, device="cuda", seed=1, max_pos=2048):
-        self = cls(cfg, None, device, max_pos)
+    def random_init(cls, cfg: Gemma3TextConfig, device="cuda", seed=1, max_pos=2048, frozen=True):
+        self = cls(cfg, None, device, max_pos, frozen)
         dev = self.device
         H, I = cfg.hidden_size, cfg.intermediate_size
         s = [seed * 100000]
@@ -148,7 +161,7 @@
                 "ln_post_ff", "q_norm", "k_norm")
         arr = (L.Gemma3LayerC * len(self.layers))()
         for i, lay in enumerate(self.layers):
-            arr[i] = L.Gemma3LayerC(*[lay[k].data_ptr() for k in keys])
+            arr[i] = L.Gemma3LayerC(*[lay[k].data_ptr() for k in keys], *[L.ptr(lay.get(k + "_kt")) for k in KT_KEYS])
         self._c_layers = arr
         self.c_w = L.Gemma3WeightsC(self.embed.data_ptr(), self.embed_t.data_ptr(), self.final_norm.data_ptr(),
                                     self.cos_l.data_ptr(), self.sin_l.data_ptr(), self.cos_g.data_ptr(),
diff --git a/projectiontrainer_amd/kernels.py b/projectiontrainer_amd/kernels.py
--- a/projectiontrainer_amd/kernels.py
+++ b/projectiontrainer_amd/kernels.py
@@ -1,4 +1,6 @@
 from __future__ import annotations
+
+import os
 
 import torch
 
@@ -19,7 +21,8 @@
 def gemm(A, B, *, C=None, out_dtype=torch.bfloat16, act=L.ACT_NONE, alpha=1.0, bias=None, rowadd=None,
          resid=None, aux=None, aux2=None, aux_in=None, aux_in2=None, M=None, N=None, K=None,
          lda=None, ldb=None, ldc=None, batch=1, batch_inner=1, strides=(0, 0, 0, 0, 0, 0),
-         amap=(0, 0, 0, 0), cmap=(0, 0, 0, 0), out_mode=None, resid16=None, bf16_linear=False, tail_ws=None):
+         amap=(0, 0, 0, 0), cmap=(0, 0, 0, 0), out_mode=None, resid16=None, bf16_linear=False, tail_ws=None,
+         B_kt=None):
     _require_cuda(A, B)
     M = A.shape[-2] if M is None else M
     K = A.shape[-1] if K is None else K
@@ -55,6 +58,7 @@
         d.resid16, d.ld_resid16 = ptr(resid16), resid16.stride(-2)
     d.bf16_linear = int(bool(bf16_linear))
     d.tail_ws = ptr(tail_ws)
+    d.B_kt = ptr(B_kt)
     check(L.lib().ptk_gemm(d, L.stream_ptr(A.device)), "ptk_gemm")
     return C
 
@@ -169,6 +173,22 @@
     check(L.lib().ptk_transpose_bf16(ptr(x3), x3.stride(1), ptr(out), rp, Z, x3.stride(0), cols * rp, rows, cols, rp,
                                      L.stream_ptr(x.device)), "transpose")
     return out[0] if squeeze else out
+
+
+def pack_kstep_tiles(w):
+    _require_cuda(w)
+    if w.dim() != 2 or w.dtype != torch.bfloat16 or not w.is_contiguous():
+        raise L.PtkError("pack_kstep_tiles: a contiguous bf16 [N, K] matrix")
+    out = torch.empty_like(w)
+    check(L.lib().ptk_pack_kstep_tiles_bf16(ptr(w), ptr(out), w.shape[0], w.shape[1], L.stream_ptr(w.device)),
+          "pack_kstep_tiles")
+    return out
+
+
+def frozen_kstep_tiles(w):
+    if os.environ.get("PTK_B_KTILED", "1") == "0" or w.shape[0] % 16 or w.shape[1] % 32:
+        return None
+    return pack_kstep_tiles(w)
 
 
 def cast_bf16(x, out=None):
diff --git a/projectiontrainer_amd/siglip.py b/projectiontrainer_amd/siglip.py
--- a/projectiontrainer_amd/siglip.py
+++ b/projectiontrainer_amd/siglip.py
@@ -80,9 +80,12 @@
                                      c.num_attention_heads, c.intermediate_size, c.num_hidden_layers,
                                      c.layer_norm_eps)
         arr = (L.SiglipLayerC * len(self.layers))()
+        for lay in self.layers:
+            lay["kt"] = {k: K.frozen_kstep_tiles(lay[k]) for k in ("wqkv", "wo", "w1", "w2")}
         for i, lay in enumerate(self.layers):
             arr[i] = L.SiglipLayerC(*[lay[k].data_ptr() for k in ("wqkv", "bqkv", "wo", "bo", "w1", "b1", "w2", "b2",
-                                                                   "ln1_w", "ln1_b", "ln2_w", "ln2_b")])
+                                                                   "ln1_w", "ln1_b", "ln2_w", "ln2_b")],
+                                    *[L.ptr(lay["kt"][k]) for k in ("wqkv", "wo", "w1", "w2")])
         self._c_layers = arr
         self.c_w = L.SiglipWeightsC(self.patch_w.data_ptr(), self.patch_b.data_ptr(), self.pos.data_ptr(),
                                     self.post_w.data_ptr(), self.post_b.data_ptr(),
diff --git a/projectiontrainer_amd/stage2.py b/projectiontrainer_amd/stage2.py
--- a/projectiontrainer_amd/stage2.py
+++ b/projectiontrainer_amd/stage2.py
@@ -64,6 +64,7 @@
                 lay[k] = self.view(f"{i}.{k}")
             for k in NORM_KEYS:
                 lay[k] = n32(f"{i}.{k}").view(self.offsets[f"{i}.{k}"][1])
+        llm.drop_ktiled()
         self.refresh()
         llm._build_c()
         self._build_grads_c()
@@ -258,7 +259,8 @@
 
 def synthetic_engine(cfg, device="cuda", seed=0, **kw):
     vision = SiglipVisionTower.random_init(cfg.vision, device, seed)
-    llm = Gemma3CausalLM.random_init(cfg.text, device, seed + 1, max_pos=Gemma3CausalLM.seq_pad(cfg.seq_len))
+    llm = Gemma3CausalLM.random_init(cfg.text, device, seed + 1, max_pos=Gemma3CausalLM.seq_pad(cfg.seq_len),
+                                     frozen=False)
     torch.manual_seed(seed + 2)
     proj = MLPProjector(cfg.vision.hidden_size, cfg.text.hidden_size, cfg.expansion_factor, device=device)
     return Stage2Engine(vision, llm, proj, **kw)
diff --git a/projectiontrainer_amd/vqa_trainer.py b/projectiontrainer_amd/vqa_trainer.py
--- a/projectiontrainer_amd/vqa_trainer.py
+++ b/projectiontrainer_amd/vqa_trainer.py
@@ -65,7 +65,7 @@
         self.vision_encoder = vision_encoder if isinstance(vision_encoder, SiglipVisionTower) \
             else SiglipVisionTower.from_hf(vision_encoder, self.device)
         self.language_model = language_model if isinstance(language_model, Gemma3CausalLM) \
-            else Gemma3CausalLM.from_hf(language_model, self.device, max_pos=4096)
+            else Gemma3CausalLM.from_hf(language_model, self.device, max_pos=4096, frozen=False)
         if not isinstance(projection_layer, MLPProjector):
             sd = projection_layer.state_dict()
             p = MLPProjector(sd["model.0.weight"].shape[1], sd["model.2.weight"].shape[0])
```

Result: faster. 326.9 images/sec (median of 6 runs) (+3.4%).
